# JoshFCooper415/differential_transformer_replication

Hardware: AMD Instinct MI355X
Metric: diff-attn fwd+bwd TFLOP/s (% MFMA peak); train tokens/sec at 1/2/4/8 GPUs (higher is better)
Workload: dtype bf16; 1 GPU; cfg2: fused N=2 diff-attention core fwd+bwd (BASELINE configs[1]); batch_per_gpu=8, global_batch=8, heads=16, head_size=64, dv=128, seq_len=4096, n_terms=2, causal=True, parallelism=batch-sharded replicas x1 (no data-path collective)

## Files before the change

### differential_transformer_replication_amd/_lib.py

```python
from __future__ import annotations

import ctypes
import os
import threading
from typing import Optional

import torch

_HERE = os.path.dirname(os.path.abspath(__file__))
LIB_PATH = os.environ.get("DTA_LIB", os.path.join(_HERE, "lib", "libdiffattn.so"))

DTA_BF16, DTA_F16, DTA_F32 = 0, 1, 2
_DTYPES = {torch.bfloat16: DTA_BF16, torch.float16: DTA_F16, torch.float32: DTA_F32}

ABI_VERSION = 9

EXPORTS = ("dta_attn_fwd", "dta_attn_bwd", "dta_attn_bwd_workspace_bytes", "dta_attn_bwd_dcoef_partial_bytes",
           "dta_ln_fwd", "dta_ln_bwd", "dta_ln_bwd_workspace_bytes",
           "dta_rope", "dta_cast_f32", "dta_error_string", "dta_abi_version", "dta_supported",
           "dta_attn_decode", "dta_attn_decode_workspace_bytes", "dta_swiglu_fwd", "dta_swiglu_bwd",
           "dta_accumulate_f32", "dta_swiglu_bwd_workspace_bytes", "dta_attn_bwd_dkdv_groups",
           "dta_attn_extend", "dta_extend_supported",
           "dta_attn_decode_ragged", "dta_attn_extend_ragged",
           "dta_attn_decode_paged", "dta_attn_extend_paged",
           "dta_attn_decode_paged_fp8", "dta_kv_quant_rows",
           "dta_attn_extend_paged_fp8", "dta_extend_fp8_supported")
FP8_EXPORTS = ("dta_attn_decode_paged_fp8", "dta_kv_quant_rows")
FP8_EXTEND_EXPORTS = ("dta_attn_extend_paged_fp8", "dta_extend_fp8_supported")


class DtaTensor(ctypes.Structure):
    _fields_ = [("ptr", ctypes.c_void_p), ("sb", ctypes.c_int64), ("st", ctypes.c_int64),
                ("sh", ctypes.c_int64), ("si", ctypes.c_int64)]


class SwigluArgs(ctypes.Structure):
    _fields_ = [("dtype", ctypes.c_int32), ("rows", ctypes.c_int64), ("n", ctypes.c_int64),
                ("a", ctypes.c_void_p), ("a_stride", ctypes.c_int64),
                ("b", ctypes.c_void_p), ("b_stride", ctypes.c_int64),
                ("out", ctypes.c_void_p), ("out_stride", ctypes.c_int64),
                ("dout", ctypes.c_void_p), ("dout_stride", ctypes.c_int64),
                ("da", ctypes.c_void_p), ("da_stride", ctypes.c_int64),
                ("db", ctypes.c_void_p), ("db_stride", ctypes.c_int64),
                ("dbias", ctypes.c_void_p), ("dbias_work", ctypes.c_void_p)]


class AttnFwdArgs(ctypes.Structure):
    _fields_ = [("dtype", ctypes.c_int32), ("B", ctypes.c_int32), ("T", ctypes.c_int32),
                ("H", ctypes.c_int32), ("n_terms", ctypes.c_int32), ("head_size", ctypes.c_int32),
                ("dv", ctypes.c_int32), ("scale", ctypes.c_float), ("dropout_p", ctypes.c_float),
                ("q", DtaTensor), ("k", DtaTensor), ("v", DtaTensor), ("o", DtaTensor),
                ("obr", DtaTensor), ("lse", ctypes.c_void_p), ("coef", ctypes.c_void_p),
                ("dropout_seed", ctypes.c_uint64), ("rope_freqs", ctypes.c_void_p), ("q_rot", DtaTensor),
                ("obr_dtype", ctypes.c_int32)]


class AttnBwdArgs(ctypes.Structure):
    _fields_ = [("dtype", ctypes.c_int32), ("B", ctypes.c_int32), ("T", ctypes.c_int32),
                ("H", ctypes.c_int32), ("n_terms", ctypes.c_int32), ("head_size", ctypes.c_int32),
                ("dv", ctypes.c_int32), ("scale", ctypes.c_float), ("dropout_p", ctypes.c_float),
                ("q", DtaTensor), ("k", DtaTensor), ("v", DtaTensor), ("obr", DtaTensor),
                ("lse", ctypes.c_void_p), ("coef", ctypes.c_void_p), ("dout", DtaTensor),
                ("dq", DtaTensor), ("dk", DtaTensor), ("dv_out", DtaTensor),
                ("dcoef", ctypes.c_void_p), ("delta", ctypes.c_void_p), ("dq_f32", ctypes.c_void_p),
                ("stages", ctypes.c_int32), ("rope_freqs", ctypes.c_void_p), ("dcoef_partial", ctypes.c_void_p),
                ("dropout_seed", ctypes.c_uint64), ("obr_dtype", ctypes.c_int32),
                ("group_max_dq", ctypes.c_int32), ("group_max_dkdv", ctypes.c_int32),
                ("dv_f32", ctypes.c_void_p), ("lse_c", ctypes.c_void_p)]


BWD_PRE, BWD_DQ, BWD_DKDV = 1, 2, 4


class LnArgs(ctypes.Structure):
    _fields_ = [("dtype", ctypes.c_int32), ("rows", ctypes.c_int64), ("C", ctypes.c_int64),
                ("eps", ctypes.c_float), ("out_scale", ctypes.c_float),
                ("x", ctypes.c_void_p), ("x_stride", ctypes.c_int64),
                ("y", ctypes.c_void_p), ("y_stride", ctypes.c_int64),
                ("w", ctypes.c_void_p), ("b", ctypes.c_void_p),
                ("mean", ctypes.c_void_p), ("rstd", ctypes.c_void_p),
                ("dy", ctypes.c_void_p), ("dy_stride", ctypes.c_int64),
                ("dx", ctypes.c_void_p), ("dx_stride", ctypes.c_int64),
                ("dw", ctypes.c_void_p), ("db", ctypes.c_void_p), ("partial", ctypes.c_void_p), ("io_dtype", ctypes.c_int32),
                ("res", ctypes.c_void_p), ("res_stride", ctypes.c_int64), ("xo", ctypes.c_void_p),
                ("xo_stride", ctypes.c_int64), ("dres", ctypes.c_void_p), ("dres_stride", ctypes.c_int64),
                ("dx16", ctypes.c_void_p), ("dx16_stride", ctypes.c_int64)]


class RopeArgs(ctypes.Structure):
    _fields_ = [("dtype", ctypes.c_int32), ("B", ctypes.c_int32), ("T", ctypes.c_int32),
                ("H", ctypes.c_int32), ("n_terms", ctypes.c_int32), ("head_size", ctypes.c_int32),
                ("inverse", ctypes.c_int32), ("src_f32", ctypes.c_int32),
                ("src", DtaTensor), ("dst", DtaTensor), ("freqs", ctypes.c_void_p)]


def _cache_op_fields(sizes, k: str, v: str, pointers):
    i32 = ("dtype", "B", "H", "n_terms", "head_size", "dv") + sizes
    return ([(n, ctypes.c_int32) for n in i32] + [("scale", ctypes.c_float)]
            + [(n, DtaTensor) for n in ("q", k, v, "o")]
            + [(n, ctypes.c_void_p) for n in ("coef",) + pointers])


_PAGED_FIELDS = [("page_size", ctypes.c_int32), ("max_pages", ctypes.c_int32), ("n_pages", ctypes.c_int32),
                 ("block_table_dev", ctypes.c_void_p)]
_DECODE_SIZES = ("length", "t_cap")


class DecodeArgs(ctypes.Structure):
    _fields_ = _cache_op_fields(_DECODE_SIZES, "k_cache", "v_cache", ("workspace", "length_dev"))


class ExtendArgs(ctypes.Structure):
    _fields_ = _cache_op_fields(("Tq", "pos", "t_cap"), "k_cache", "v_cache", ())


class DecodeRaggedArgs(ctypes.Structure):
    _fields_ = _cache_op_fields(_DECODE_SIZES, "k_cache", "v_cache", ("workspace", "lengths_dev"))


class ExtendRaggedArgs(ctypes.Structure):
    _fields_ = _cache_op_fields(("Tq", "t_cap"), "k_cache", "v_cache", ("pos_dev", "count_dev"))


class DecodePagedArgs(ctypes.Structure):
    _fields_ = _cache_op_fields(_DECODE_SIZES, "k_pool", "v_pool", ("workspace", "lengths_dev")) + _PAGED_FIELDS


class ExtendPagedArgs(ctypes.Structure):
    _fields_ = _cache_op_fields(("Tq", "t_cap"), "k_pool", "v_pool", ("pos_dev", "count_dev")) + _PAGED_FIELDS


class DecodePagedFp8Args(ctypes.Structure):
    _fields_ = DecodePagedArgs._fields_ + [("scale_pool_dev", ctypes.c_void_p), ("scale_page_stride", ctypes.c_int64)]


class ExtendPagedFp8Args(ctypes.Structure):
    _fields_ = ExtendPagedArgs._fields_ + [("scale_pool_dev", ctypes.c_void_p), ("scale_page_stride", ctypes.c_int64)]


class KvQuantRowsArgs(ctypes.Structure):
    _fields_ = [("dtype", ctypes.c_int32), ("B", ctypes.c_int32), ("Tn", ctypes.c_int32), ("H", ctypes.c_int32),
                ("n_terms", ctypes.c_int32), ("head_size", ctypes.c_int32), ("dv", ctypes.c_int32),
                ("page_size", ctypes.c_int32), ("n_pages", ctypes.c_int32),
                ("k_new", DtaTensor), ("v_new", DtaTensor), ("k_pool", DtaTensor), ("v_pool", DtaTensor),
                ("scale_pool_dev", ctypes.c_void_p), ("scale_page_stride", ctypes.c_int64),
                ("slot_dev", ctypes.c_void_p)]


_lock = threading.Lock()
_lib: Optional[ctypes.CDLL] = None


def load(path: str = LIB_PATH) -> ctypes.CDLL:
    global _lib
    with _lock:
        if _lib is not None:
            return _lib
        if not os.path.exists(path):
            raise RuntimeError(f"libdiffattn.so not found at {path}: run __graft_entry__.build() "
                               "(hipcc --offload-arch=gfx950); there is no CPU fallback")
        lib = ctypes.CDLL(path)
        P = ctypes.POINTER
        lib.dta_attn_fwd.argtypes = [P(AttnFwdArgs), ctypes.c_void_p]
        lib.dta_attn_bwd.argtypes = [P(AttnBwdArgs), ctypes.c_void_p]
        lib.dta_ln_fwd.argtypes = [P(LnArgs), ctypes.c_void_p]
        lib.dta_ln_bwd.argtypes = [P(LnArgs), ctypes.c_void_p]
        lib.dta_rope.argtypes = [P(RopeArgs), ctypes.c_void_p]
        lib.dta_swiglu_fwd.argtypes = [P(SwigluArgs), ctypes.c_void_p]
        lib.dta_swiglu_bwd.argtypes = [P(SwigluArgs), ctypes.c_void_p]
        lib.dta_cast_f32.argtypes = [ctypes.c_int32] * 6 + [ctypes.c_void_p, DtaTensor, ctypes.c_void_p]
        lib.dta_swiglu_bwd_workspace_bytes.argtypes = [ctypes.c_int64, ctypes.c_int64]
        lib.dta_swiglu_bwd_workspace_bytes.restype = ctypes.c_size_t
        lib.dta_accumulate_f32.argtypes = [ctypes.c_int32, ctypes.c_int64, ctypes.c_void_p, ctypes.c_void_p,
                                           ctypes.c_void_p]
        lib.dta_attn_decode.argtypes = [P(DecodeArgs), ctypes.c_void_p]
        lib.dta_attn_decode_workspace_bytes.argtypes = [ctypes.c_int32] * 6
        lib.dta_attn_extend.argtypes = [P(ExtendArgs), ctypes.c_void_p]
        lib.dta_extend_supported.argtypes = [ctypes.c_int32] * 4
        lib.dta_attn_decode_ragged.argtypes = [P(DecodeRaggedArgs), ctypes.c_void_p]
        lib.dta_attn_extend_ragged.argtypes = [P(ExtendRaggedArgs), ctypes.c_void_p]
        lib.dta_attn_decode_paged.argtypes = [P(DecodePagedArgs), ctypes.c_void_p]
        lib.dta_attn_extend_paged.argtypes = [P(ExtendPagedArgs), ctypes.c_void_p]
        lib.dta_attn_decode_workspace_bytes.restype = ctypes.c_size_t
        lib.dta_attn_bwd_workspace_bytes.argtypes = [ctypes.c_int32] * 5
        lib.dta_attn_bwd_workspace_bytes.restype = ctypes.c_size_t
        lib.dta_attn_bwd_dcoef_partial_bytes.argtypes = [ctypes.c_int32] * 4
        lib.dta_attn_bwd_dcoef_partial_bytes.restype = ctypes.c_size_t
        lib.dta_ln_bwd_workspace_bytes.argtypes = [ctypes.c_int64] * 2
        lib.dta_ln_bwd_workspace_bytes.restype = ctypes.c_size_t
        lib.dta_error_string.argtypes = [ctypes.c_int]
        lib.dta_error_string.restype = ctypes.c_char_p
        lib.dta_supported.argtypes = [ctypes.c_int32] * 4
        lib.dta_attn_bwd_dkdv_groups.argtypes = [ctypes.c_int32] * 5
        for fn in ("dta_attn_fwd", "dta_attn_bwd", "dta_attn_decode", "dta_ln_fwd", "dta_ln_bwd", "dta_rope", "dta_cast_f32",
                   "dta_abi_version", "dta_supported", "dta_swiglu_fwd", "dta_swiglu_bwd", "dta_accumulate_f32",
                   "dta_attn_bwd_dkdv_groups", "dta_attn_extend", "dta_extend_supported", "dta_attn_decode_ragged",
                   "dta_attn_extend_ragged", "dta_attn_decode_paged", "dta_attn_extend_paged"):
            getattr(lib, fn).restype = ctypes.c_int
        if fp8_symbols(lib):
            lib.dta_attn_decode_paged_fp8.argtypes = [P(DecodePagedFp8Args), ctypes.c_void_p]
            lib.dta_kv_quant_rows.argtypes = [P(KvQuantRowsArgs), ctypes.c_void_p]
            lib.dta_attn_decode_paged_fp8.restype = lib.dta_kv_quant_rows.restype = ctypes.c_int
        if fp8_extend_symbols(lib):
            lib.dta_attn_extend_paged_fp8.argtypes = [P(ExtendPagedFp8Args), ctypes.c_void_p]
            lib.dta_extend_fp8_supported.argtypes = [ctypes.c_int32] * 4
            lib.dta_attn_extend_paged_fp8.restype = lib.dta_extend_fp8_supported.restype = ctypes.c_int
        if lib.dta_abi_version() != ABI_VERSION:
            raise RuntimeError(f"libdiffattn ABI {lib.dta_abi_version()} != expected {ABI_VERSION}")
        _lib = lib
        return lib


def fp8_symbols(lib) -> bool:
    return all(hasattr(lib, name) for name in FP8_EXPORTS)


def fp8_extend_symbols(lib) -> bool:
    return all(hasattr(lib, name) for name in FP8_EXTEND_EXPORTS)


def check(rc: int) -> None:
    if rc != 0:
        msg = load().dta_error_string(rc).decode()
        raise RuntimeError(f"libdiffattn: {msg} (code {rc})")


def dtype_code(t: torch.dtype) -> int:
    try:
        return _DTYPES[t]
    except KeyError:
        raise RuntimeError(f"libdiffattn supports bf16, fp16 and fp32 activations, got {t}") from None


def stream_handle(device: torch.device) -> int:
    return torch.cuda.current_stream(device).cuda_stream


def ptr(t: Optional[torch.Tensor]) -> Optional[int]:
    return None if t is None else t.data_ptr()


def tensor5(t: torch.Tensor) -> DtaTensor:
    if t.dim() == 5:
        sb, st, sh, si, sd = t.stride()
    elif t.dim() == 4:
        sb, st, sh, sd = t.stride()
        si = 0
    else:
        raise ValueError("expected a 4-d or 5-d view")
    if sd != 1:
        raise RuntimeError("innermost dimension must be contiguous")
    return DtaTensor(t.data_ptr(), sb, st, sh, si)


def supported(dtype: torch.dtype, head_size: int, n_terms: int, dv: int) -> bool:
    return bool(load().dta_supported(dtype_code(dtype), head_size, n_terms, dv))
```

### differential_transformer_replication_amd/csrc/attn_bf16.hip

```cpp
#include "attn_kernels.h"

namespace dta {
int launch_attn_fwd_bf16(const FwdParams& p, hipStream_t st) { return dispatch_fwd<__bf16, false>(p, st); }
int launch_attn_dq_bf16(const BwdParams& p, hipStream_t st) { return dispatch_dq<__bf16, false>(p, st); }
int launch_attn_dkdv_bf16(const BwdParams& p, hipStream_t st) { return dispatch_dkdv<__bf16, false>(p, st); }
bool attn_native_bf16(int hs, int n, int dv) { return native_t<__bf16>(hs, n, dv); }
}
```

### differential_transformer_replication_amd/csrc/attn_f16.hip

```cpp
#include "attn_kernels.h"

namespace dta {
int launch_attn_fwd_f16(const FwdParams& p, hipStream_t st) { return dispatch_fwd<_Float16, false>(p, st); }
int launch_attn_dq_f16(const BwdParams& p, hipStream_t st) { return dispatch_dq<_Float16, false>(p, st); }
int launch_attn_dkdv_f16(const BwdParams& p, hipStream_t st) { return dispatch_dkdv<_Float16, false>(p, st); }
bool attn_native_f16(int hs, int n, int dv) { return native_t<_Float16>(hs, n, dv); }
}
```

### differential_transformer_replication_amd/csrc/attn_kernels.h

```cpp
#pragma once
#include "dta_common.h"
#include "dta_internal.h"
#include "layout_checks.h"

#include <type_traits>
#include <utility>

#ifndef DTA_STAMPS
#define DTA_STAMPS 0
#endif

namespace dta {

template <int NSEG_ = 8>
struct Stamps {
  static constexpr int NSEG = NSEG_;
  unsigned t = 0, s[NSEG] = {};
  __device__ __forceinline__ static unsigned now() {
    unsigned long long v;
    __builtin_amdgcn_sched_barrier(0);
    asm volatile("s_memtime %0\n\ts_waitcnt lgkmcnt(0)" : "=s"(v) : : "memory");
    __builtin_amdgcn_sched_barrier(0);
    return (unsigned)v;
  }
// ... 861 lines not shown
        const unsigned a0 = vb + (Lv ^ (64 * d)), a1 = vb + (Lv ^ (64 * d + 32));
        if constexpr (SPILLS) {
          sfor<NKB>([&](auto KB) { tr_load<VI::ROWB, 32 * decltype(KB)::value>(r[decltype(KB)::value], a0, a1); });
        } else {
          sfor<NKB>([&](auto KB) { tr_issue<VI::ROWB, 32 * decltype(KB)::value>(r[decltype(KB)::value], a0, a1); });
          lgkm_pin<NKB>(r);
        }
#pragma unroll
        for (int kb = 0; kb < NKB; ++kb)
#pragma unroll
          for (int s = 0; s < 2; ++s) {
            const frag va = tr_frag<E>(r[kb], s);
#pragma unroll
            for (int i = 0; i < N; ++i) acc[i][d] = O::mma(va, pf[i][kb * 2 + s], acc[i][d]);
          }
      });
    } else {
#pragma unroll
      for (int d = 0; d < NDB; ++d)
#pragma unroll
        for (int kb = 0; kb < NKB; ++kb)
#pragma unroll
          for (int s = 0; s < SPB; ++s) {
            const frag va = VI::tr_perm(Vc, kb * 32, s, hf, d * 32, lane);
#pragma unroll
            for (int i = 0; i < N; ++i) acc[i][d] = O::mma(va, pf[i][kb * SPB + s], acc[i][d]);
          }
    }
  };

  Stamps<> st;
  auto step = [&](int kt, auto MASKED, auto FASTT) {
    asm volatile("" : "+v"(lane));
    if constexpr (sizeof(E) == 2) asm volatile("" : "+v"(LrK), "+v"(LtV));
    tid = (wave << 6) + lane; hf = lane >> 5; c32 = lane & 31;
    qrow = qw0 + c32;
    const bool live = wave_live && kt * BN <= qw0 + 31;
    st.lap<7>();
    if (kt + NS - 1 < ntiles) stage_kv(kt + NS - 1, (kt + NS - 1) % NS);
    st.lap<0>();
    if (live) {
      frag pf[N][NKB * SPB];
      phase_a(kt, MASKED, pf, FASTT);
      st.lap<1>();
      phase_b(kt, pf);
      st.lap<2>();
    }
    wait_vm(tile_pieces * max(0, min(NS - 2, ntiles - 2 - kt)));
    st.lap<3>();
    lds_barrier();
    st.lap<4>();
  };
  auto attempt = [&](bool safe) {
    for (int j = 0; j < NS - 1; ++j)
      if (j < ntiles) stage_kv(j, j);
    wait_vm(tile_pieces * max(0, min(NS - 1, ntiles) - 1));
    lds_barrier();
    if (qrot_pending) {
#pragma unroll
      for (int i = NQR; i < N; ++i)
        rope_lds<E, HSP, BM, HS, NTHR>(Qs + (i - NQR) * BM * HSP, p.rope, q0, T, gqr + i * p.qrot.si, p.qrot.st,
                                       dc0 == 0, tid);
      lds_barrier();
      qrot_pending = false;
    }
#pragma unroll
    for (int i = 0; i < N; ++i) {
      m[i] = -INFINITY;
      l[i] = 0.f;
#pragma unroll
      for (int d = 0; d < NDB; ++d) acc[i][d] = f32x16{};
    }
    if constexpr (sizeof(E) == 2) { LrK = row_lane<KI::ROWB>(lane); LtV = tr_lane<VI::ROWB>(lane); }
    st.start();
    const int nfull = min(ntiles, min((q0 + 1) / BN, T / BN));
    const int kslow = (safe || !FAST) ? ntiles : min(1, ntiles);
    for (int kt = 0; kt < min(nfull, kslow); ++kt) step(kt, std::false_type{}, std::false_type{});
    for (int kt = nfull; kt < kslow; ++kt) step(kt, std::true_type{}, std::false_type{});
    if constexpr (FAST) {
      for (int kt = kslow; kt < nfull; ++kt) step(kt, std::false_type{}, std::true_type{});
      for (int kt = max(kslow, nfull); kt < ntiles; ++kt) step(kt, std::true_type{}, std::true_type{});
    }
  };
  for (int pass = 0; pass < (FAST ? 2 : 1); ++pass) {
    attempt(pass == 1);
    if constexpr (!FAST) break;
    if (pass == 1) break;
    int* flag = reinterpret_cast<int*>(Kb);
    const bool mine = __any(wave_live && qrow < T && bad != 0.f);
    if (lane == 0) flag[wave] = mine ? 1 : 0;
    lds_barrier();
    bool any = false;
#pragma unroll
    for (int w = 0; w < NW; ++w) any |= flag[w] != 0;
    lds_barrier();
    if (!any) break;
  }
  st.lap<5>();
  st.flush(p.stamps, lin * NW + wave, lane);

  if (!SEQ && !wave_live) return;
  if (bnc) {
    if (wave_live) {
      float inv[N];
#pragma unroll
      for (int i = 0; i < N; ++i) {
        const float lt = wave_sum_halves(l[i]);
        inv[i] = 1.f / lt;
        if (dc0 == 0 && hf == 0 && qrow < T)
          p.lse[(((int64_t)(brs + i) * p.B + b) * p.H + hh) * T + qrow] = -(m[i] + __builtin_log2f(lt));
      }
      float* reg = reinterpret_cast<float*>(Kb) + wave * 2048;
      const int nrows = min(32, T - qw0);
      float* gob0 = reinterpret_cast<float*>(p.obr.p) + b * p.obr.sb + (int64_t)qw0 * p.obr.st + hh * p.obr.sh +
                    brs * p.obr.si + dc0;
#pragma unroll
      for (int i = 0; i < N; ++i)
        bounce_store<float, NDB>(reg, lane, [&](int d, int g) {
          return f32x4{acc[i][d][4 * g] * inv[i], acc[i][d][4 * g + 1] * inv[i], acc[i][d][4 * g + 2] * inv[i],
                       acc[i][d][4 * g + 3] * inv[i]};
        }, gob0 + i * p.obr.si, p.obr.st, nrows);
      auto osum = [&](int d, int g) {
        f32x4 o = f32x4{};
#pragma unroll
        for (int i = 0; i < N; ++i)
#pragma unroll
          for (int j = 0; j < 4; ++j) o[j] = fmaf(coef[i], acc[i][d][4 * g + j] * inv[i], o[j]);
        return o;
      };
      if constexpr (SEQ) {
#pragma unroll
        for (int d = 0; d < NDB; ++d)
#pragma unroll
          for (int g = 0; g < 4; ++g) {
            const f32x4 o = osum(d, g);
#pragma unroll
            for (int j = 0; j < 4; ++j) oacc[d < NDBS ? d : 0][4 * g + j] += o[j];
          }
      } else if (nsp == 1) {
        E* go0 = reinterpret_cast<E*>(p.o.p) + b * p.o.sb + (int64_t)qw0 * p.o.st + hh * p.o.sh + dc0;
        bounce_store<E, NDB>(reg, lane, osum, go0, p.o.st, nrows);
      }
    }
    if constexpr (SEQ) lds_barrier();
  } else {
  if (!SEQ && qrow >= T) return;
  if (wave_live && qrow < T) {
  float inv[N];
#pragma unroll
  for (int i = 0; i < N; ++i) {
    const float lt = wave_sum_halves(l[i]);
    inv[i] = 1.f / lt;
    if (dc0 == 0 && hf == 0)
      p.lse[(((int64_t)(brs + i) * p.B + b) * p.H + hh) * T + qrow] = -(m[i] + __builtin_log2f(lt));
  }
  E* go = reinterpret_cast<E*>(p.o.p) + b * p.o.sb + (int64_t)qrow * p.o.st + hh * p.o.sh + dc0;
  const int64_t gob = b * p.obr.sb + (int64_t)qrow * p.obr.st + hh * p.obr.sh + brs * p.obr.si + dc0;
#pragma unroll
  for (int d = 0; d < NDB; ++d)
#pragma unroll
    for (int g = 0; g < 4; ++g) {
      const int e = d * 32 + 8 * g + 4 * hf;
      float o0 = 0.f, o1 = 0.f, o2 = 0.f, o3 = 0.f;
#pragma unroll
      for (int i = 0; i < N; ++i) {
        const float a0 = acc[i][d][4 * g + 0] * inv[i], a1 = acc[i][d][4 * g + 1] * inv[i];
        const float a2 = acc[i][d][4 * g + 2] * inv[i], a3 = acc[i][d][4 * g + 3] * inv[i];
        store_ob4(p.obr.p, gob + i * p.obr.si + e, p.ob16, a0, a1, a2, a3);
        o0 = fmaf(coef[i], a0, o0); o1 = fmaf(coef[i], a1, o1);
        o2 = fmaf(coef[i], a2, o2); o3 = fmaf(coef[i], a3, o3);
      }
      if constexpr (SEQ) {
        oacc[d < NDBS ? d : 0][4 * g + 0] += o0; oacc[d < NDBS ? d : 0][4 * g + 1] += o1;
        oacc[d < NDBS ? d : 0][4 * g + 2] += o2; oacc[d < NDBS ? d : 0][4 * g + 3] += o3;
      } else {
        if (nsp == 1) store4<E>(go + e, o0, o1, o2, o3);
      }
    }
  }
  }
  }
  if constexpr (SEQ) {
    if (qw0 >= T) return;
    if (bnc) {
      E* go0 = reinterpret_cast<E*>(p.o.p) + b * p.o.sb + (int64_t)qw0 * p.o.st + hh * p.o.sh + dc0;
      bounce_store<E, NDBS>(reinterpret_cast<float*>(Kb) + wave * 2048, lane, [&](int d, int g) {
        return f32x4{oacc[d][4 * g], oacc[d][4 * g + 1], oacc[d][4 * g + 2], oacc[d][4 * g + 3]};
      }, go0, p.o.st, min(32, T - qw0));
      return;
    }
    if (qrow >= T) return;
    E* go = reinterpret_cast<E*>(p.o.p) + b * p.o.sb + (int64_t)qrow * p.o.st + hh * p.o.sh + dc0;
#pragma unroll
    for (int d = 0; d < NDBS; ++d)
#pragma unroll
      for (int g = 0; g < 4; ++g)
        store4<E>(go + d * 32 + 8 * g + 4 * hf, oacc[d][4 * g], oacc[d][4 * g + 1], oacc[d][4 * g + 2], oacc[d][4 * g + 3]);
  }
}

template <class E, int HS, int N, int DV, int NW, bool QREG, int QRH = 0, bool BN32 = false>
struct DqCfg {
  static constexpr bool PAIR = NW == 4 && !QREG && sizeof(E) == 2;
  static constexpr int BN = (PAIR && QRH == 0) || BN32 ? 32 : FwdTile<E>::BN;
  static constexpr int BM = NW * 32;
  static constexpr int HSP = img_cols(HS < 32 ? 32 : HS), QP = img_cols(HS), DVP = img_cols(DV);
  static constexpr int nQ = QREG ? 0 : (N - QRH) * BM * QP;
  static constexpr int nK = N * BN * HSP;
  static constexpr int nV = BN * DVP;
  static constexpr int NS = ring_stages_lim(nQ * (int)sizeof(E), (nK + nV) * (int)sizeof(E),
                                            PAIR ? 80 * 1024 : 160 * 1024);
  static constexpr int bytes = (nQ + NS * nK + NS * nV) * (int)sizeof(E);
};

#ifndef DTA_DQ_EXPG
#define DTA_DQ_EXPG 4
#endif
static_assert(DTA_DQ_EXPG >= 1 && 16 % DTA_DQ_EXPG == 0, "DTA_DQ_EXPG: a divisor of the 16 rows a lane holds");
template <class E, int HS, int N, int DV = 2 * HS, bool NP = false>
struct DqPick {
  static constexpr int LIM = 160 * 1024;
  static constexpr bool q8 = sizeof(E) == 2 && DqCfg<E, HS, N, DV, 8, false>::bytes <= LIM;
  static constexpr int QRH = (q8 && DqCfg<E, HS, N, DV, 4, false, 1>::bytes <= 80 * 1024) ? 1 : 0;
  static constexpr bool pair64 = !NP && QRH == 1 && q8 && HS >= 64 &&
                                 DqCfg<E, HS, N, DV, 4, false, QRH>::bytes <= 80 * 1024;
  static constexpr bool pair32 = !NP && !pair64 && sizeof(E) == 2 && N >= 3 && HS == 64 &&
                                 DqCfg<E, HS, N, DV, 4, false, 1, true>::bytes <= 80 * 1024;
  static constexpr bool pair = pair64 || pair32;
  static constexpr int NW = pair ? 4 : (q8 ? 8 : (sizeof(E) == 2 ? 4 : 2));
  static constexpr bool QREG = pair ? false : !q8;
  static constexpr int QH = pair ? 1 : 0;
  static constexpr bool B32 = pair32 || DqCfg<E, HS, N, DV, NW, QREG, QH>::bytes > LIM;
  static constexpr bool ok = DqCfg<E, HS, N, DV, NW, QREG, QH, B32>::bytes <= LIM;
};

template <class E, int HS, int N, int DV, int NW, bool QREG, bool OUTF32, bool SRD, bool DROP, int QRH, bool B32>
__global__ __launch_bounds__(NW * 64, simd_waves(NW, DqCfg<E, HS, N, DV, NW, QREG, QRH, B32>::bytes))
void attn_dq_kernel(BwdParams p) {
  using O = Ops<E>;
  using frag = typename O::frag;
  using CF = DqCfg<E, HS, N, DV, NW, QREG, QRH, B32>;
  constexpr int NQR = QREG ? N : QRH;
  constexpr int HSP = CF::HSP, QP = CF::QP, DVP = CF::DVP;
  using QI = Img<E, QP>;
  using KI = Img<E, HSP>;
  using VI = Img<E, DVP>;
  constexpr int BN = CF::BN, BM = CF::BM, NTHR = NW * 64;
  constexpr int KS = O::KSTEP;
  constexpr int NSQ = HS / KS, NSV = DV / KS;
  constexpr int NKB = BN / 32, SPB = 32 / KS, NHB = (HS + 31) / 32;

  extern __shared__ __attribute__((aligned(16))) char smem[];
  E* Qs = reinterpret_cast<E*>(smem);
  constexpr int NS = CF::NS;
  E* Kb = Qs + CF::nQ;
  E* Vb = Kb + NS * CF::nK;

  const int wave = __builtin_amdgcn_readfirstlane(threadIdx.x >> 6);
  int tid = threadIdx.x, lane = tid & 63;
  int hf = lane >> 5, c32 = lane & 31;
  int bx, by, bz, lin;
  lpt_order(bx, by, bz, lin);
  const int qt = gridDim.x - 1 - bx;
  const int hh = by, b = bz;
  const int T = p.T;
  const int q0 = qt * BM, qw0 = q0 + wave * 32;
  int qrow = qw0 + c32;
  const bool rowok = qrow < T;

  const E* gq = reinterpret_cast<const E*>(p.q.p) + b * p.q.sb + hh * p.q.sh;
  const E* gk = reinterpret_cast<const E*>(p.k.p) + b * p.k.sb + hh * p.k.sh;
  const E* gv = reinterpret_cast<const E*>(p.v.p) + b * p.v.sb + hh * p.v.sh;
  const E* gdo = reinterpret_cast<const E*>(p.dout.p) + b * p.dout.sb + hh * p.dout.sh;
  const int64_t gob = b * p.obr.sb + hh * p.obr.sh;

  const int kend = min(T, q0 + BM);
  const int ntiles = (kend + BN - 1) / BN;
  using KR = KvRing<E, HS, N, DV, BN, NW>;
  static_assert(!SRD || (HSP == KR::HSP && DVP == KR::DVP), "descriptor staging fills the kernel's images");
  constexpr bool PRE = SRD && !DROP;
  uint32_t doff[PRE ? KR::MYP : 1];
  if constexpr (PRE) KR::offsets(p.k.st, p.k.si, p.v.st, wave, lane, doff);
  auto stage_kv = [&](int kt, int buf) {
    const int k0 = kt * BN;
    if constexpr (PRE) {
      KR::issue_pre(gk, p.k.st, gv, p.v.st, k0, T, Kb + buf * CF::nK, Vb + buf * CF::nV, wave, doff);
    } else if constexpr (SRD) {
      KR::issue(gk, p.k.st, p.k.si, gv, p.v.st, k0, T, Kb + buf * CF::nK, Vb + buf * CF::nV, wave, lane);
    } else {
#pragma unroll
      for (int i = 0; i < N; ++i)
        stage<E, HSP, BN, HS, NTHR>(Kb + (buf * N + i) * BN * HSP, gk + i * p.k.si, p.k.st, k0, T - 1, tid);
      stage<E, DVP, BN, DV, NTHR>(Vb + buf * CF::nV, gv, p.v.st, k0, T - 1, tid);
    }
  };

  constexpr bool SEED = std::is_same<E, __bf16>::value && !DROP && SRD && !(HS >= 128 && N >= 3);
  constexpr bool SPILLS = sizeof(E) == 2 && (DROP || (HS >= 128 && N >= 3) || (HS >= 192 && N >= 2));
  frag qf[NQR > 0 ? NQR : 1][NQR > 0 ? NSQ : 1], df[NSV];
  float coef[N], lse[N], del[N];
  float dhead = 0.f;
  const int64_t rs = (((int64_t)0 * p.B + b) * p.H + hh) * T + qrow;
  const int64_t bstride = (int64_t)p.B * p.H * T;
#pragma unroll
  for (int s = 0; s < NSV; ++s)
    df[s] = rowok ? O::load_global(gdo + (int64_t)qrow * p.dout.st + s * KS + hf * O::KH) : O::zero();
#pragma unroll
  for (int i = 0; i < N; ++i) {
    coef[i] = p.coef[hh * p.cst + i];
    if (i < NQR) {
#pragma unroll
      for (int s = 0; s < NSQ; ++s)
        qf[i < NQR ? i : 0][s] = rowok ? O::load_global(gq + (int64_t)qrow * p.q.st + i * p.q.si + s * KS + hf * O::KH)
                                       : O::zero();
      if constexpr (SEED) {
#pragma unroll
        for (int s = 0; s < NSQ; ++s)
#pragma unroll
          for (int j = 0; j < 8; ++j) qf[i < NQR ? i : 0][s][j] = (E)((float)qf[i < NQR ? i : 0][s][j] * p.sl2);
      }
    }
    lse[i] = rowok ? p.lse[rs + i * bstride] : 0.f;
    if (p.lsec && rowok && hf == 0) p.lsec[rs + i * bstride] = lse[i] + __builtin_log2f(fabsf(coef[i]));
    float d = 0.f;
    if (rowok) {
#pragma unroll
      for (int s = 0; s < NSV; ++s) {
        const int64_t o = gob + (int64_t)qrow * p.obr.st + i * p.obr.si + s * KS + hf * O::KH;
        if constexpr (sizeof(E) == 2) {
          float ov[8];
          load_ob8(p.obr.p, o, p.ob16, ov);
#pragma unroll
          for (int j = 0; j < 8; ++j) d = fmaf((float)df[s][j], ov[j], d);
        } else {
          d = fmaf(df[s], reinterpret_cast<const float*>(p.obr.p)[o], d);
        }
      }
    }
    d = wave_sum_halves(d);
    del[i] = d;
    const bool kstart = i == 0 || ((p.kstarts >> i) & 1);
    if (kstart) dhead = d;
    if (rowok && hf == 0) p.delta[rs + i * bstride] = DROP ? d : (kstart ? -d : dhead - d);
    float w = (rowok && hf == 0) ? d : 0.f;
#pragma unroll
    for (int o = 32; o > 0; o >>= 1) w += __shfl_xor(w, o, 64);
    if (p.dcoef_part) {
      if (lane == 0 && qw0 < T) p.dcoef_part[(((int64_t)hh * p.cst + i) * p.B + b) * ((T + 31) / 32) + qw0 / 32] = w;
    } else if (lane == 0 && qw0 < T) {
      atomicAdd(p.dcoef + hh * p.cst + i, w);
    }
  }

  if constexpr (!QREG) {
#pragma unroll
    for (int i = NQR; i < N; ++i)
      stage<E, QP, BM, HS, NTHR>(Qs + (i - NQR) * BM * QP, gq + i * p.q.si, p.q.st, q0, T - 1, tid);
  }
  const int tile_pieces = SRD ? KR::pieces(wave)
                              : N * stage_pieces<E, HSP, BN, HS, NW>(wave) + stage_pieces<E, DVP, BN, DV, NW>(wave);
  for (int j = 0; j < NS - 1; ++j)
    if (j < ntiles) stage_kv(j, j);
  wait_vm(tile_pieces * max(0, min(NS - 1, ntiles) - 1));
  lds_barrier();
  frag f_one = O::zero(), f_lse[SEED ? N : 1], f_dp = O::zero();
  float ddel[N];
  if constexpr (SEED) {
    if constexpr (!QREG && N > NQR) {
      scale_lds<E, NTHR>(Qs, CF::nQ, p.sl2, tid);
      lds_barrier();
    }
    if (hf == 0) { f_one[0] = (E)1.f; f_one[1] = (E)1.f; }
#pragma unroll
    for (int i = 0; i < N; ++i) {
      f_lse[i] = seed_frag<E>(lse[i], hf);
      ddel[i] = del[0] - del[i];
    }
    f_dp = seed_frag<E>(-del[0], hf);
  }

  f32x16 dq[N][NHB];
#pragma unroll
  for (int i = 0; i < N; ++i)
#pragma unroll
    for (int d = 0; d < NHB; ++d) dq[i][d] = f32x16{};
  const bool wave_live = qw0 < T;

  int LrV = 0, LrK = 0, LrQ = 0, LtK = 0;
  constexpr int XMAX = 32 * ((NSV > NSQ ? NSV : NSQ) - 1) + 64 * (NHB - 1) + 32;
  constexpr int XM = XMAX < 256 ? 256 : (XMAX < 512 ? 512 : 1024);
  constexpr bool XA = !DROP && SRD && sizeof(E) == 2 && (CF::nQ * (int)sizeof(E)) % XM == 0 &&
                      (CF::nK * (int)sizeof(E)) % XM == 0 && (CF::nV * (int)sizeof(E)) % XM == 0;
  if constexpr (sizeof(E) == 2) {
    LrV = row_lane<VI::ROWB>(lane); LrK = row_lane<KI::ROWB>(lane); LrQ = row_lane<QI::ROWB>(lane);
    LtK = tr_lane<KI::ROWB>(lane);
  }
  Stamps<5> st;
  auto step = [&](int kt, auto MASKED) {
    constexpr bool MASK = decltype(MASKED)::value;
    asm volatile("" : "+v"(lane));
    if constexpr (!DROP && sizeof(E) == 2) {
      asm volatile("" : "+v"(LrV), "+v"(LrK), "+v"(LtK));
      if constexpr (QI::ROWB == KI::ROWB) LrQ = LrK;
      else asm volatile("" : "+v"(LrQ));
    } else if constexpr (sizeof(E) == 2) {
      LrV = row_lane<VI::ROWB>(lane); LrK = row_lane<KI::ROWB>(lane); LrQ = row_lane<QI::ROWB>(lane);
      LtK = tr_lane<KI::ROWB>(lane);
    }
    tid = (wave << 6) + lane; hf = lane >> 5; c32 = lane & 31;
    qrow = qw0 + c32;
    const int buf = kt % NS;
    if (kt + NS - 1 < ntiles) stage_kv(kt + NS - 1, (kt + NS - 1) % NS);
    st.lap<0>();
    const int k0 = kt * BN;
    if (wave_live && k0 <= qw0 + 31) {
      const E* Kc = Kb + buf * CF::nK;
      const E* Vc = Vb + buf * CF::nV;
      unsigned bV = 0, bK = 0, tK = 0;
      if constexpr (XA) {
        bV = LrV + lds_addr(Vc); bK = LrK + lds_addr(Kc); tK = LtK + lds_addr(Kc);
      }
      {
        f32x16 dp[NKB];
        if constexpr (sizeof(E) == 2) {
          const int Lv = LrV;
          const char* vbase = reinterpret_cast<const char*>(Vc);
#pragma unroll
          for (int kb = 0; kb < NKB; ++kb) dp[kb] = SEED ? O::mma(f_one, f_dp, f32x16{}) : f32x16{};
          if constexpr (XA && !SPILLS) {
            constexpr int NIT = NSV * NKB, D = DTA_DQ_PIPE;
            i32x4 vb[D + 1];
            auto issue = [&](auto J) {
              constexpr int j = decltype(J)::value;
              ds128<(j % NKB) * 32 * VI::ROWB>(vb[j % (D + 1)], bV ^ (32 * (j / NKB)));
            };
            sfor<(D < NIT ? D : NIT)>([&](auto J) { issue(J); });
            sfor<NIT>([&](auto J) {
              constexpr int j = decltype(J)::value;
              if constexpr (j + D < NIT) issue(std::integral_constant<int, j + D>{});
              lgkm_wait<(j + D < NIT ? D : NIT - 1 - j)>();
              asm volatile("" : "+v"(vb[j % (D + 1)]));
              dp[j % NKB] = O::mma(__builtin_bit_cast(frag, vb[j % (D + 1)]), df[j / NKB], dp[j % NKB]);
            });
          } else
#pragma unroll
          for (int s = 0; s < NSV; ++s) {
            const int o = Lv ^ (32 * s);
#pragma unroll
            for (int kb = 0; kb < NKB; ++kb) {
              if constexpr (XA) dp[kb] = O::mma(lds_at<frag>(bV ^ (32 * s), kb * 32 * VI::ROWB), df[s], dp[kb]);
              else dp[kb] = O::mma(*reinterpret_cast<const frag*>(vbase + kb * 32 * VI::ROWB + o), df[s], dp[kb]);
            }
          }

        } else {
#pragma unroll
          for (int kb = 0; kb < NKB; ++kb) {
            dp[kb] = f32x16{};
#pragma unroll
            for (int s = 0; s < NSV; ++s) dp[kb] = O::mma(VI::row(Vc, kb * 32 + c32, s, hf), df[s], dp[kb]);
          }
        }
        st.lap<1>();
        sfor<N>([&](auto I_) {
          constexpr int i = decltype(I_)::value;
          const E* Ki = Kc + i * BN * HSP;
          f32x16 sa[NKB];
          if constexpr (XA && !SPILLS) {
            constexpr int QL = i >= NQR ? 1 : 0;
            constexpr int KOFF = i * BN * HSP * (int)sizeof(E), QOFF = (i >= NQR ? i - NQR : 0) * BM * QP * (int)sizeof(E);
#pragma unroll
            for (int kb = 0; kb < NKB; ++kb) sa[kb] = SEED ? O::mma(f_one, f_lse[SEED ? i : 0], f32x16{}) : f32x16{};
            s_chain_pipe<E, NSQ, NKB, QL, DTA_DQ_PIPE, KOFF, QOFF, KI::ROWB>(
                sa, bK, lds_addr(Qs) + wave * 32 * QI::ROWB + LrQ, qf[i < NQR ? i : 0]);
          } else if constexpr (sizeof(E) == 2) {
            const int Lr = LrK;
            const char* kbase = reinterpret_cast<const char*>(Ki);
            const char* qbase = reinterpret_cast<const char*>(Qs + (i >= NQR ? i - NQR : 0) * BM * QP) +
                                wave * 32 * QI::ROWB;
            const int Lq = LrQ;
#pragma unroll
            for (int kb = 0; kb < NKB; ++kb) sa[kb] = SEED ? O::mma(f_one, f_lse[SEED ? i : 0], f32x16{}) : f32x16{};
#pragma unroll
            for (int s = 0; s < NSQ; ++s) {
              frag qb;
              if (i < NQR) qb = qf[i < NQR ? i : 0][s];
              else qb = *reinterpret_cast<const frag*>(qbase + (Lq ^ (32 * s)));
#pragma unroll
              for (int kb = 0; kb < NKB; ++kb) {
                if constexpr (XA)
                  sa[kb] = O::mma(lds_at<frag>(bK ^ (32 * s), (i * BN * HSP) * (int)sizeof(E) + kb * 32 * KI::ROWB), qb,
                                  sa[kb]);
                else
                  sa[kb] = O::mma(*reinterpret_cast<const frag*>(kbase + kb * 32 * KI::ROWB + (Lr ^ (32 * s))), qb, sa[kb]);
              }
            }
          } else {
#pragma unroll
            for (int kb = 0; kb < NKB; ++kb) {
              sa[kb] = f32x16{};
#pragma unroll
              for (int s = 0; s < NSQ; ++s) {
                frag qb;
                if (i < NQR) qb = qf[i < NQR ? i : 0][s];
                else qb = QI::row(Qs + (i >= NQR ? i - NQR : 0) * BM * QP, wave * 32 + c32, s, hf);
                sa[kb] = O::mma(KI::row(Ki, kb * 32 + c32, s, hf), qb, sa[kb]);
              }
            }
          }
          const float li = lse[i], ci = coef[i], cdi = coef[i] * del[i];
          const int lim = min(qrow, T - 1) - k0 - 4 * hf;
          if constexpr (SEED) {
            const float dd = ddel[i];
#pragma unroll
            for (int kb = 0; kb < NKB; ++kb)
#pragma unroll
              for (int r0 = 0; r0 < 16; r0 += DTA_DQ_EXPG) {
                float pr[DTA_DQ_EXPG];
#pragma unroll
                for (int u = 0; u < DTA_DQ_EXPG; ++u) {
                  const int r = r0 + u;
                  float arg = sa[kb][r];
                  if constexpr (MASK) arg = (kb * 32 + (r & 3) + 8 * (r >> 2) > lim) ? -INFINITY : arg;
                  pr[u] = exp2_fast(arg);
                }
#pragma unroll
                for (int u = 0; u < DTA_DQ_EXPG; ++u) {
                  const int r = r0 + u;
                  sa[kb][r] = i == 0 ? pr[u] * dp[kb][r] : pr[u] * (dp[kb][r] + dd);
                }
              }
          } else {
          uint32_t dkey = 0;
          if constexpr (DROP) dkey = drop_key(p.drop_seed_lo, p.drop_seed_hi, b, hh, p.br0 + i, p.H, p.cst);
#pragma unroll
          for (int kb = 0; kb < NKB; ++kb)
#pragma unroll
            for (int r = 0; r < 16; ++r) {
              float arg = fmaf(sa[kb][r], p.sl2, li);
              if constexpr (MASK) arg = (kb * 32 + (r & 3) + 8 * (r >> 2) > lim) ? -INFINITY : arg;
              float cm = ci;
              if constexpr (DROP)
                cm *= drop_mul(dkey, qrow, k0 + kb * 32 + (r & 3) + 8 * (r >> 2) + 4 * hf, p.drop_thr, p.drop_scale);
              sa[kb][r] = exp2_fast(arg) * fmaf(cm, dp[kb][r], -cdi);
            }
          }
          if constexpr (sizeof(E) == 2) {
            const unsigned kbse = lds_addr(Ki);
            const int Lk = LtK;
            sfor<NHB>([&](auto D) {
              constexpr int d = decltype(D)::value;
              lds64 r[NKB][4];
              const unsigned a0 = XA ? (tK ^ (64 * d)) + (unsigned)(i * BN * HSP * (int)sizeof(E)) : kbse + (Lk ^ (64 * d));
              const unsigned a1 = XA ? (tK ^ (64 * d + 32)) + (unsigned)(i * BN * HSP * (int)sizeof(E))
                                     : kbse + (Lk ^ (64 * d + 32));
              if constexpr (SPILLS) {
                sfor<NKB>([&](auto KB) { tr_load<KI::ROWB, 32 * decltype(KB)::value>(r[decltype(KB)::value], a0, a1); });
              } else {
                sfor<NKB>([&](auto KB) { tr_issue<KI::ROWB, 32 * decltype(KB)::value>(r[decltype(KB)::value], a0, a1); });
                lgkm_pin<NKB>(r);
              }
#pragma unroll
              for (int kb = 0; kb < NKB; ++kb) {
                dq[i][d] = O::mma(tr_frag<E>(r[kb], 0), O::template pack<0>(sa[kb]), dq[i][d]);
                dq[i][d] = O::mma(tr_frag<E>(r[kb], 1), O::template pack<1>(sa[kb]), dq[i][d]);
              }
            });
          } else {
#pragma unroll
            for (int d = 0; d < NHB; ++d)
#pragma unroll
              for (int kb = 0; kb < NKB; ++kb)
#pragma unroll
                for (int s = 0; s < SPB; ++s)
                  dq[i][d] = O::mma(KI::tr_perm(Ki, kb * 32, s, hf, d * 32, lane), sa[kb][s], dq[i][d]);
          }
        });
      }
    }
    st.lap<2>();
    wait_vm(tile_pieces * max(0, min(NS - 2, ntiles - 2 - kt)));
    st.lap<3>();
    lds_barrier();
    st.lap<4>();
  };
  st.start();
  const int nfull = min(ntiles, min((q0 + 1) / BN, T / BN));
  for (int kt = 0; kt < nfull; ++kt) step(kt, std::false_type{});
  for (int kt = nfull; kt < ntiles; ++kt) step(kt, std::true_type{});
  st.flush(p.stamps, lin * NW + wave, lane);

  if (qw0 >= T) return;
  constexpr bool BNC = sizeof(E) == 2 && NHB % 2 == 0 && CF::bytes >= NW * 8192;
  if constexpr (BNC) {
    if (OUTF32 || t5_aligned16(p.dq, sizeof(E))) {
      float* reg = reinterpret_cast<float*>(smem) + wave * 2048;
      const int nrows = min(32, T - qw0);
      const int rrow = min(qrow, T - 1);
#pragma unroll
      for (int i = 0; i < N; ++i) {
        const float sc = SEED ? p.scale * coef[i] : p.scale;
        auto val = [&](int d, int g) {
          float a0 = dq[i][d][4 * g] * sc, a1 = dq[i][d][4 * g + 1] * sc;
          float a2 = dq[i][d][4 * g + 2] * sc, a3 = dq[i][d][4 * g + 3] * sc;
          if (p.rope) rope_inv4(p.rope, rrow, HS, d * 32 + 8 * g + 4 * hf, a0, a1, a2, a3);
          return f32x4{a0, a1, a2, a3};
        };
        if constexpr (OUTF32)
          bounce_store<float, NHB>(reg, lane, val, p.dq32 + ((((int64_t)b * T + qw0) * p.H + hh) * p.cst + i) * HS,
                                   (int64_t)p.H * p.cst * HS, nrows);
        else
          bounce_store<E, NHB>(reg, lane, val, reinterpret_cast<E*>(p.dq.p) + b * p.dq.sb + (int64_t)qw0 * p.dq.st +
                                                   hh * p.dq.sh + i * p.dq.si, p.dq.st, nrows);
      }
      return;
    }
  }
  if (!rowok) return;
#pragma unroll
  for (int i = 0; i < N; ++i)
#pragma unroll
    for (int d = 0; d < NHB; ++d)
#pragma unroll
      for (int g = 0; g < 4; ++g) {
        const int e = d * 32 + 8 * g + 4 * hf;
        if (e >= HS) continue;
        const float sc = SEED ? p.scale * coef[i] : p.scale;
        float a0 = dq[i][d][4 * g] * sc, a1 = dq[i][d][4 * g + 1] * sc;
        float a2 = dq[i][d][4 * g + 2] * sc, a3 = dq[i][d][4 * g + 3] * sc;
        if (p.rope) rope_inv4(p.rope, qrow, HS, e, a0, a1, a2, a3);
        if constexpr (OUTF32) {
          store4<float>(p.dq32 + ((((int64_t)b * T + qrow) * p.H + hh) * p.cst + i) * HS + e, a0, a1, a2, a3);
        } else {
          E* gdq = reinterpret_cast<E*>(p.dq.p) + b * p.dq.sb + (int64_t)qrow * p.dq.st + hh * p.dq.sh + i * p.dq.si;
          store4<E>(gdq + e, a0, a1, a2, a3);
        }
      }
}

template <class E, int HS, int N, int DV, int NW, bool DELTA, int BQ_ = 32, bool ROWS = true>
struct TileRing {
  static constexpr int ES = (int)sizeof(E), BQ = BQ_;
  static constexpr int NP = (N * BQ + 63) / 64 * 64;
  static constexpr int HSP = img_cols(HS), DVP = img_cols(DV);
  static constexpr int QB = BQ * HSP * ES, DB = BQ * DVP * ES;
  static constexpr int OFF_D = N * QB, OFF_L = OFF_D + DB, OFF_G = OFF_L + NP * 4;
  static constexpr int SB = ROWS ? OFF_G + NP * 4 : OFF_L;
  static constexpr int PQ = N * QB / 1024, PD = DB / 1024, PL = NP / 64;
  static constexpr int NPC = PQ + PD + (ROWS ? (DELTA ? 2 : 1) * PL : 0);
  static constexpr int MYP = (NPC + NW - 1) / NW;
  static constexpr bool ok = ES == 2 && HS >= 32 && QB % 1024 == 0 && DB % 1024 == 0;

  __device__ static int pieces(int wave) { return NPC / NW + (wave < NPC % NW ? 1 : 0); }

  __device__ static uint32_t offq(const BwdParams& p, int j, int lane) {
    using QI = Img<E, HSP>;
    const int i = j / (QB / 1024), pb = (j % (QB / 1024)) * 1024 + lane * 16;
    const int r = pb / QI::ROWB;
    int c = ((pb % QI::ROWB) >> 4) ^ swz<QI::ROWB>(r);
    if constexpr (HSP != HS) c = c * 16 < HS * ES ? c : 0;
    return (uint32_t)(r * (uint32_t)(p.q.st * ES) + (uint32_t)(i * p.q.si * ES) + c * 16);
  }
  __device__ static uint32_t offd(const BwdParams& p, int j, int lane) {
    using DI = Img<E, DVP>;
    const int pb = (j - PQ) * 1024 + lane * 16;
    const int r = pb / DI::ROWB;
    int c = ((pb % DI::ROWB) >> 4) ^ swz<DI::ROWB>(r);
    if constexpr (DVP != DV) c = c * 16 < DV * ES ? c : 0;
    return (uint32_t)(r * (uint32_t)(p.dout.st * ES) + c * 16);
  }
  __device__ static uint32_t offr(int j, int lane, int64_t bstride) {
    const int e = ((j - PQ - PD) % PL) * 64 + lane;
    const int i = min(e / BQ, N - 1), r = e % BQ;
    return (uint32_t)((i * (uint32_t)bstride + r) * 4);
  }
  __device__ static void offsets(const BwdParams& p, int64_t bstride, int wave, int lane, uint32_t (&off)[MYP]) {
    sfor<MYP>([&](auto U) {
      constexpr int u = decltype(U)::value;
      const int j = u * NW + wave;
      if constexpr ((u + 1) * NW <= PQ) off[u] = offq(p, j, lane);
      else if constexpr (u * NW >= PQ && (u + 1) * NW <= PQ + PD) off[u] = offd(p, j, lane);
      else off[u] = j < PQ ? offq(p, j, lane) : (j < PQ + PD ? offd(p, j, lane) : (j < NPC ? offr(j, lane, bstride) : 0u));
    });
  }
  __device__ static void issue_pre(const BwdParams& p, const E* gq, const E* gdo, const float* lse, const float* delta,
                                   int64_t bstride, int q0, int T, char* st0, int wave, const uint32_t (&off)[MYP]) {
    const int rows = T - q0;
    const E* bq = gq + (int64_t)q0 * p.q.st;
    const E* bd = gdo + (int64_t)q0 * p.dout.st;
    const uint32_t nq = (uint32_t)rows * (uint32_t)(p.q.st * ES), nd = (uint32_t)rows * (uint32_t)(p.dout.st * ES);
    const uint32_t nl = (uint32_t)(((N - 1) * bstride + rows) * 4);
    sfor<MYP>([&](auto U) {
      constexpr int u = decltype(U)::value;
      const int j = u * NW + wave;
      if constexpr ((u + 1) * NW <= PQ) {
        buf_lds16(bq, nq, st0 + j * 1024, off[u]);
      } else if constexpr (u * NW >= PQ && (u + 1) * NW <= PQ + PD) {
        buf_lds16(bd, nd, st0 + OFF_D + (j - PQ) * 1024, off[u]);
      } else {
        if (j < PQ) buf_lds16(bq, nq, st0 + j * 1024, off[u]);
        else if (j < PQ + PD) buf_lds16(bd, nd, st0 + OFF_D + (j - PQ) * 1024, off[u]);
        else if (j < PQ + PD + PL) buf_lds4(lse + q0, nl, st0 + OFF_L + (j - PQ - PD) * 256, off[u]);
        else if (j < NPC) buf_lds4(delta + q0, nl, st0 + OFF_G + (j - PQ - PD - PL) * 256, off[u]);
      }
    });
  }
};

inline bool ring_layout_ok(const BwdParams& p, int es) {
  return dma_rows_ok(p.T, p.q.st, p.q.si, p.N, p.HS, es) && dma_rows_ok(p.T, p.dout.st, 0, 1, p.DV, es) &&
         dma_rowvecs_ok(p.N, p.B, p.H, p.T);
}


template <class E, int HS, int N, int DV, int NW, bool PR = false, bool GRX = false>
struct DkdvCfg {
  static constexpr int LIMB = PR ? 80 * 1024 : 160 * 1024;
  static constexpr int BK = NW * 32;
  static constexpr int HSP = img_cols(HS < 32 ? 32 : HS), KP = img_cols(HS), DVP = img_cols(DV);
  static constexpr int BQ = 32;
  static constexpr int NP = (N * BQ + 63) / 64 * 64;
  static constexpr int nQ = N * BQ * HSP;
  static constexpr int nD = BQ * DVP;
  static constexpr int nK = N * BK * KP;
  static constexpr int RB = 2 * NP * 4;
  static constexpr bool GR = GRX;
  static constexpr int NS = ring_stages_lim(nK * (int)sizeof(E), (nQ + nD) * (int)sizeof(E) + (GR ? 0 : RB), LIMB);
  static constexpr int bytes = (nK + NS * nQ + NS * nD) * (int)sizeof(E) + (GR ? 0 : NS * RB);
};

template <int HS, int N, int DV>
struct DkdvSplit {
  static constexpr int HSB = (HS < 32 ? 32 : HS + 31) / 32 * 32;
  static constexpr bool fused = (N * HSB / 2 + DV / 2) <= 160;
};

template <class E, int HS, int N, int DV, bool NP = false>
struct DkdvWaves {
  static constexpr int LIM = 160 * 1024;
  static constexpr int HSB = DkdvSplit<HS, N, DV>::HSB;
  static constexpr int regs8 = DkdvSplit<HS, N, DV>::fused ? N * HSB / 2 + DV / 2 + DV / 4 + 88
                             : (N * HSB / 2 + DV / 4 > DV / 2 ? N * HSB / 2 + DV / 4 : DV / 2) + 88;
  static constexpr int v8 = (sizeof(E) == 2 && DkdvCfg<E, HS, N, DV, 8>::bytes <= LIM && regs8 <= 256) ? 8
                          : DkdvCfg<E, HS, N, DV, 4>::bytes <= LIM ? 4 : 2;
  static constexpr bool pair = !NP && std::is_same<E, __bf16>::value && v8 == 8 &&
                               DkdvCfg<E, HS, N, DV, 4, true>::bytes <= 80 * 1024;
  static constexpr int v0 = pair ? 4 : v8;
  static constexpr bool gr = DkdvCfg<E, HS, N, DV, v0, pair>::bytes > LIM;
  static constexpr int v = !gr ? v0 : (DkdvCfg<E, HS, N, DV, 2, false, true>::bytes <= LIM ? 2 : 1);
};

template <class E, int HS, int N, int DV, int NW, bool DK, bool DVV, bool SRD, bool DROP, bool PR, bool GRX,
          bool CFOLD = false>
__global__ __launch_bounds__(NW * 64, (NW >= 8 || PR ? 2 : 1))
void attn_dkdv_kernel(BwdParams p) {
  using O = Ops<E>;
  using frag = typename O::frag;
  using CF = DkdvCfg<E, HS, N, DV, NW, PR, GRX>;
  constexpr int HSP = CF::HSP, KP = CF::KP, DVP = CF::DVP, BQ = CF::BQ, BK = CF::BK, NP = CF::NP;
  constexpr int NTHR = NW * 64;
  using QI = Img<E, HSP>;
  using DI = Img<E, DVP>;
  constexpr int KS = O::KSTEP;
  constexpr int NSQ = HS / KS, NSV = DV / KS, SPB = 32 / KS;
  constexpr int NHB = (HS + 31) / 32, NVB = DV / 32;
  constexpr bool SPILLS = sizeof(E) == 2 && (DROP || (HS >= 128 && N >= 3) || (HS >= 192 && N >= 2));

  using KI = Img<E, KP>;
  extern __shared__ __attribute__((aligned(16))) char smem[];
  E* Ks = reinterpret_cast<E*>(smem);
  E* Qb = Ks + CF::nK;
  constexpr int NS = CF::NS;
  E* Db = Qb + NS * CF::nQ;
  float* Lb = reinterpret_cast<float*>(Db + NS * CF::nD);
  float* Gb = Lb + NS * NP;
  constexpr bool GR = CF::GR;
  using RG = TileRing<E, HS, N, DV, NW, DK, BQ, !GR>;
  char* ringb = reinterpret_cast<char*>(Qb);
  static_assert(!SRD || (RG::ok && RG::SB * NS <= CF::bytes - CF::nK * (int)sizeof(E) && RG::HSP == HSP &&
                          RG::DVP == DVP), "ring layout");

  const int wave = __builtin_amdgcn_readfirstlane(threadIdx.x >> 6);
  int tid = threadIdx.x, lane = tid & 63;
  int hf = lane >> 5, c32 = lane & 31;
  int bx, by, bz, lin;
  lpt_order(bx, by, bz, lin);
  const int kblk = bx;
  const int hh = by, b = bz;
  const int T = p.T;
  const int kb0 = kblk * BK, kw0 = kb0 + wave * 32;
  int krow = kw0 + c32;

  const E* gq = reinterpret_cast<const E*>(p.q.p) + b * p.q.sb + hh * p.q.sh;
  const E* gk = reinterpret_cast<const E*>(p.k.p) + b * p.k.sb + hh * p.k.sh;
  const E* gv = reinterpret_cast<const E*>(p.v.p) + b * p.v.sb + hh * p.v.sh;
  const E* gdo = reinterpret_cast<const E*>(p.dout.p) + b * p.dout.sb + hh * p.dout.sh;
  const int64_t rowvec = ((int64_t)b * p.H + hh) * T;
  const int64_t bstride = (int64_t)p.B * p.H * T;

  float coef[N];
  uint32_t dkey[N];
#pragma unroll
  for (int i = 0; i < N; ++i) {
    coef[i] = p.coef[hh * p.cst + i];
    dkey[i] = DROP ? drop_key(p.drop_seed_lo, p.drop_seed_hi, b, hh, p.br0 + i, p.H, p.cst) : 0u;
  }
  static_assert(!CFOLD || (!DROP && sizeof(E) == 2 && !GRX), "CFOLD: 16-bit plans without dropout");
  auto sgn = [](float c) { return c < 0.f ? -1.f : 1.f; };
  float wv[N];
#pragma unroll
  for (int i = 0; i < N; ++i) wv[i] = CFOLD ? sgn(coef[0]) * sgn(coef[i]) : coef[i];
  const float dvsc = CFOLD ? sgn(coef[0]) : 1.f;
  const float* lsep = CFOLD ? p.lsec : p.lse;
  frag vf[DK ? NSV : 1];
  if constexpr (DK) {
#pragma unroll
    for (int s = 0; s < NSV; ++s)
      vf[s] = krow < T ? O::load_global(gv + (int64_t)krow * p.v.st + s * KS + hf * O::KH) : O::zero();
  }

  uint32_t roff[SRD ? RG::MYP : 1];
  if constexpr (SRD) RG::offsets(p, bstride, wave, lane, roff);
  auto stage_q = [&](int q0, int buf) {
    if constexpr (SRD) {
      RG::issue_pre(p, gq, gdo, lsep + rowvec, p.delta + rowvec, bstride, q0, T, ringb + buf * RG::SB, wave, roff);
    } else {
#pragma unroll
      for (int i = 0; i < N; ++i)
        stage<E, HSP, BQ, HS, NTHR>(Qb + (buf * N + i) * BQ * HSP, gq + i * p.q.si, p.q.st, q0, T - 1, tid);
      stage<E, DVP, BQ, DV, NTHR>(Db + buf * CF::nD, gdo, p.dout.st, q0, T - 1, tid);
      if constexpr (!GR) {
        stage_rows<N, BQ, NTHR>(Lb + buf * NP, lsep + rowvec, bstride, q0, T - 1, tid);
        if constexpr (DK) stage_rows<N, BQ, NTHR>(Gb + buf * NP, p.delta + rowvec, bstride, q0, T - 1, tid);
      }
    }
  };

  f32x16 dk[DK ? N : 1][NHB];
  f32x16 dv[DVV ? NVB : 1];
#pragma unroll
  for (int i = 0; i < (DK ? N : 1); ++i)
#pragma unroll
    for (int d = 0; d < NHB; ++d) dk[i][d] = f32x16{};
#pragma unroll
  for (int d = 0; d < (DVV ? NVB : 1); ++d) dv[d] = f32x16{};

  const int ntiles = kb0 < T ? (T - kb0 + BQ - 1) / BQ : 0;
#pragma unroll
  for (int i = 0; i < N; ++i) stage<E, KP, BK, HS, NTHR>(Ks + i * BK * KP, gk + i * p.k.si, p.k.st, kb0, T - 1, tid);
  const int tile_pieces = SRD ? RG::pieces(wave)
                              : N * stage_pieces<E, HSP, BQ, HS, NW>(wave) + stage_pieces<E, DVP, BQ, DV, NW>(wave) +
                                    rows_pieces<N, BQ, NW>(wave) * (DK ? 2 : 1);
  for (int j = 0; j < NS - 1; ++j)
    if (j < ntiles) stage_q(kb0 + j * BQ, j);
  wait_vm(tile_pieces * max(0, min(NS - 1, ntiles) - 1));
  lds_barrier();
  scale_lds<E, NTHR>(Ks, CF::nK, p.sl2, tid);
  lds_barrier();
  const bool wave_keys = kw0 < T;

  Stamps<4> st;
  int LrD = 0, LrQ = 0, LrK = 0, LtQ = 0, LtD = 0;
  constexpr int XMAX = 64 * ((NVB > NHB ? NVB : NHB) - 1) + 32 + 32 * ((NSV > NSQ ? NSV : NSQ) - 1);
  constexpr int XM = XMAX < 256 ? 256 : (XMAX < 512 ? 512 : 1024);
  constexpr bool XA = SRD && sizeof(E) == 2 && (CF::nK * (int)sizeof(E)) % XM == 0 && RG::SB % XM == 0 &&
                      QI::ROWB == KI::ROWB;
  if constexpr (sizeof(E) == 2) {
    LrD = row_lane<DI::ROWB>(lane); LrQ = row_lane<QI::ROWB>(lane); LrK = row_lane<KI::ROWB>(lane);
    LtQ = tr_lane<QI::ROWB>(lane); LtD = tr_lane<DI::ROWB>(lane);
  }
  auto step = [&](int t, auto MASKED) {
    constexpr bool MASK = decltype(MASKED)::value;
    asm volatile("" : "+v"(lane));
    if constexpr (sizeof(E) == 2) {
      asm volatile("" : "+v"(LrD), "+v"(LrQ), "+v"(LtQ), "+v"(LtD));
      if constexpr (QI::ROWB == KI::ROWB) LrK = LrQ;
      else asm volatile("" : "+v"(LrK));
    }
    tid = (wave << 6) + lane; hf = lane >> 5; c32 = lane & 31;
    krow = kw0 + c32;
    const int buf = t % NS;
    const int q0 = kb0 + t * BQ;
    if (t + NS - 1 < ntiles) stage_q(q0 + (NS - 1) * BQ, (t + NS - 1) % NS);
    st.lap<0>();
    if (wave_keys && q0 + 31 >= kw0) {
      const char* sg = ringb + buf * RG::SB;
      const E* Qc = SRD ? reinterpret_cast<const E*>(sg) : Qb + buf * N * BQ * HSP;
      const E* Dc = SRD ? reinterpret_cast<const E*>(sg + RG::OFF_D) : Db + buf * CF::nD;
      const float* Lc = SRD ? reinterpret_cast<const float*>(sg + RG::OFF_L) : Lb + buf * NP;
      const float* Gc = SRD ? reinterpret_cast<const float*>(sg + RG::OFF_G) : Gb + buf * NP;
      auto rows4 = [&](const float* ring, const float* glb, int i, int g) -> f32x4 {
        if constexpr (GR) {
          const float* v = glb + rowvec + i * bstride;
          const int r0 = q0 + 8 * g + 4 * hf;
          return f32x4{v[min(r0, T - 1)], v[min(r0 + 1, T - 1)], v[min(r0 + 2, T - 1)], v[min(r0 + 3, T - 1)]};
        } else {
          return *reinterpret_cast<const f32x4*>(ring + i * BQ + 8 * g + 4 * hf);
        }
      };
      unsigned bQ = 0, bD = 0, tQ = 0, tD = 0;
      if constexpr (XA) {
        const unsigned sb = lds_addr(sg);
        bQ = LrQ + sb; bD = LrD + sb; tQ = LtQ + sb; tD = LtD + sb;
      }
      {
      f32x16 dpa = f32x16{};
      if constexpr (DK && !DROP) {
#pragma unroll
        for (int g = 0; g < 4; ++g) {
          const f32x4 g4 = rows4(Gc, p.delta, 0, g);
#pragma unroll
          for (int j = 0; j < 4; ++j) dpa[4 * g + j] = g4[j];
        }
      }
      if constexpr (DK) {
        if constexpr (sizeof(E) == 2) {
          const int Ld = LrD;
          const char* dbase = reinterpret_cast<const char*>(Dc);
#pragma unroll
          for (int s = 0; s < NSV; ++s) {
            if constexpr (XA) dpa = O::mma(lds_at<frag>(bD ^ (32 * s), RG::OFF_D), vf[s], dpa);
            else dpa = O::mma(*reinterpret_cast<const frag*>(dbase + (Ld ^ (32 * s))), vf[s], dpa);
          }
        } else {
#pragma unroll
          for (int s = 0; s < NSV; ++s) dpa = O::mma(DI::row(Dc, c32, s, hf), vf[s], dpa);
        }
      }
      f32x16 pc = f32x16{};
      const int lim_lo = krow - q0 - 4 * hf;
      const int lim_hi = T - 1 - q0 - 4 * hf;
#pragma unroll
      for (int i = 0; i < N; ++i) {
        if constexpr (CFOLD) if (i > 0) __builtin_amdgcn_sched_barrier(0);
        f32x16 sa;
#pragma unroll
        for (int g = 0; g < 4; ++g) {
          const f32x4 l4 = rows4(Lc, lsep, i, g);
#pragma unroll
          for (int j = 0; j < 4; ++j) sa[4 * g + j] = l4[j];
        }
        const E* Qi = Qc + i * BQ * HSP;
        if constexpr (sizeof(E) == 2) {
          const int Lq = LrQ, Lk = LrK;
          const char* qbase = reinterpret_cast<const char*>(Qi);
          const char* kbase = reinterpret_cast<const char*>(Ks + i * BK * KP) + wave * 32 * KI::ROWB;
          frag qfr[NSQ], kfr[NSQ];
#pragma unroll
          for (int s = 0; s < NSQ; ++s) {
            if constexpr (XA) qfr[s] = lds_at<frag>(bQ ^ (32 * s), i * RG::QB);
            else qfr[s] = *reinterpret_cast<const frag*>(qbase + (Lq ^ (32 * s)));
            kfr[s] = *reinterpret_cast<const frag*>(kbase + (Lk ^ (32 * s)));
          }
#pragma unroll
          for (int s = 0; s < NSQ; ++s) sa = O::mma(qfr[s], kfr[s], sa);
          __builtin_amdgcn_sched_group_barrier(0x100, 2 * NSQ, 0);
          __builtin_amdgcn_sched_group_barrier(0x008, NSQ, 0);
        } else {
#pragma unroll
          for (int s = 0; s < NSQ; ++s)
            sa = O::mma(QI::row(Qi, c32, s, hf), KI::row(Ks + i * BK * KP, wave * 32 + c32, s, hf), sa);
        }
#pragma unroll
        for (int g = 0; g < 4; ++g) {
          f32x4 d4 = f32x4{};
          if constexpr (DK) if (DROP || i > 0) d4 = rows4(Gc, p.delta, i, g);
#pragma unroll
          for (int j = 0; j < 4; ++j) {
            const int r = 4 * g + j;
            float arg = sa[r];
            if constexpr (MASK) {
              const int rc = (r & 3) + 8 * (r >> 2);
              arg = (rc < lim_lo || rc > lim_hi) ? -INFINITY : arg;
            }
            const float pr = exp2_fast(arg);
            if constexpr (DROP) {
              const float mk = drop_mul(dkey[i], q0 + (r & 3) + 8 * (r >> 2) + 4 * hf, krow, p.drop_thr, p.drop_scale);
              if constexpr (DVV) pc[r] = fmaf(coef[i] * mk, pr, pc[r]);
              if constexpr (DK) sa[r] = pr * fmaf(mk, dpa[r], -d4[j]);
            } else {
              if constexpr (DVV) pc[r] = i == 0 ? (CFOLD ? pr : wv[0] * pr) : fmaf(wv[i], pr, pc[r]);
              if constexpr (DK) sa[r] = i == 0 ? pr * dpa[r] : pr * (dpa[r] + d4[j]);
            }
          }
        }
        if constexpr (DK) {
          if constexpr (sizeof(E) == 2) {
            const unsigned qb = lds_addr(Qi);
            const int Lq = LtQ;
            lds64 r[NHB][4];
            sfor<NHB>([&](auto D) {
              constexpr int d = decltype(D)::value;
              if constexpr (SPILLS) {
                if constexpr (XA) tr_load<QI::ROWB, 0>(r[d], (tQ ^ (64 * d)) + i * RG::QB, (tQ ^ (64 * d + 32)) + i * RG::QB);
                else tr_load<QI::ROWB, 0>(r[d], qb + (Lq ^ (64 * d)), qb + (Lq ^ (64 * d + 32)));
              } else {
                if constexpr (XA) tr_issue<QI::ROWB, 0>(r[d], (tQ ^ (64 * d)) + i * RG::QB, (tQ ^ (64 * d + 32)) + i * RG::QB);
                else tr_issue<QI::ROWB, 0>(r[d], qb + (Lq ^ (64 * d)), qb + (Lq ^ (64 * d + 32)));
              }
            });
            if constexpr (!SPILLS) lgkm_pin<NHB>(r);
            const frag p0 = O::template pack<0>(sa), p1 = O::template pack<1>(sa);
#pragma unroll
            for (int d = 0; d < NHB; ++d) {
              dk[i][d] = O::mma(tr_frag<E>(r[d], 0), p0, dk[i][d]);
              dk[i][d] = O::mma(tr_frag<E>(r[d], 1), p1, dk[i][d]);
            }
          } else {
#pragma unroll
            for (int d = 0; d < NHB; ++d)
#pragma unroll
              for (int s = 0; s < SPB; ++s) dk[i][d] = O::mma(QI::tr_perm(Qi, 0, s, hf, d * 32, lane), sa[s], dk[i][d]);
          }
        }
      }
      if constexpr (DVV) {
        if constexpr (sizeof(E) == 2) {
          const unsigned db = lds_addr(Dc);
          const int Ld = LtD;
          const frag p0 = O::template pack<0>(pc), p1 = O::template pack<1>(pc);
          constexpr int NP2 = NVB >= 2 ? 2 : 1;
          auto dv_blocks = [&](auto D0, auto NB) {
            constexpr int d0 = decltype(D0)::value, nb = decltype(NB)::value;
            lds64 r[nb][4];
            sfor<nb>([&](auto E2) {
              constexpr int d = d0 + decltype(E2)::value;
              if constexpr (SPILLS) {
                if constexpr (XA) tr_load<DI::ROWB, 0, RG::OFF_D>(r[decltype(E2)::value], tD ^ (64 * d), tD ^ (64 * d + 32));
                else tr_load<DI::ROWB, 0>(r[decltype(E2)::value], db + (Ld ^ (64 * d)), db + (Ld ^ (64 * d + 32)));
              } else {
                if constexpr (XA) tr_issue<DI::ROWB, 0, RG::OFF_D>(r[decltype(E2)::value], tD ^ (64 * d), tD ^ (64 * d + 32));
                else tr_issue<DI::ROWB, 0>(r[decltype(E2)::value], db + (Ld ^ (64 * d)), db + (Ld ^ (64 * d + 32)));
              }
            });
            if constexpr (!SPILLS) lgkm_pin<nb>(r);
#pragma unroll
            for (int e = 0; e < nb; ++e) {
              dv[d0 + e] = O::mma(tr_frag<E>(r[e], 0), p0, dv[d0 + e]);
              dv[d0 + e] = O::mma(tr_frag<E>(r[e], 1), p1, dv[d0 + e]);
            }
          };
          sfor<NVB / NP2>([&](auto D2) {
            dv_blocks(std::integral_constant<int, NP2 * decltype(D2)::value>{}, std::integral_constant<int, NP2>{});
          });
          if constexpr (NVB % NP2) dv_blocks(std::integral_constant<int, NVB - 1>{}, std::integral_constant<int, 1>{});
        } else {
#pragma unroll
          for (int d = 0; d < NVB; ++d)
#pragma unroll
            for (int s = 0; s < SPB; ++s) dv[d] = O::mma(DI::tr_perm(Dc, 0, s, hf, d * 32, lane), pc[s], dv[d]);
        }
      }
      }
    }
    st.lap<1>();
    wait_vm(tile_pieces * max(0, min(NS - 2, ntiles - 2 - t)));
    st.lap<2>();
    lds_barrier();
    st.lap<3>();
  };
  st.start();
  const int thead = min(ntiles, (BK - 2) / BQ + 1);
  const int ttail = max(thead, ntiles - ((T - kb0) % BQ != 0 ? 1 : 0));
  for (int t = 0; t < thead; ++t) step(t, std::true_type{});
  for (int t = thead; t < ttail; ++t) step(t, std::false_type{});
  for (int t = ttail; t < ntiles; ++t) step(t, std::true_type{});
  st.flush(p.stamps, lin * NW + wave, lane);

  if (!wave_keys) return;
  constexpr bool BNC = sizeof(E) == 2 && (!DK || NHB % 2 == 0) && (!DVV || NVB % 2 == 0) &&
                       CF::bytes >= NW * 8192;
  if constexpr (BNC) {
    float* g32 = p.dv32 ? p.dv32 + (((int64_t)b * p.T + kw0) * p.H + hh) * p.DV : nullptr;
    const bool to32 = g32 != nullptr && !p.dv_last;
    if ((!DK || t5_aligned16(p.dk, sizeof(E))) && (!DVV || p.dv_acc || to32 || t5_aligned16(p.dv, sizeof(E)))) {
      float* reg = reinterpret_cast<float*>(smem) + wave * 2048;
      const int nrows = min(32, T - kw0);
      const int rrow = min(krow, T - 1);
      if constexpr (DK) {
#pragma unroll
        for (int i = 0; i < N; ++i) {
          const float sc = p.scale * (CFOLD ? sgn(coef[i]) : coef[i]);
          bounce_store<E, NHB>(reg, lane, [&](int d, int g) {
            float a0 = dk[i][d][4 * g] * sc, a1 = dk[i][d][4 * g + 1] * sc;
            float a2 = dk[i][d][4 * g + 2] * sc, a3 = dk[i][d][4 * g + 3] * sc;
            if (p.rope) rope_inv4(p.rope, rrow, HS, d * 32 + 8 * g + 4 * hf, a0, a1, a2, a3);
            return f32x4{a0, a1, a2, a3};
          }, reinterpret_cast<E*>(p.dk.p) + b * p.dk.sb + (int64_t)kw0 * p.dk.st + hh * p.dk.sh + i * p.dk.si,
             p.dk.st, nrows);
        }
      }
      if constexpr (DVV) {
        if (!p.dv_acc) {
          auto val = [&](int d, int g) {
            return f32x4{dv[d][4 * g] * dvsc, dv[d][4 * g + 1] * dvsc, dv[d][4 * g + 2] * dvsc, dv[d][4 * g + 3] * dvsc};
          };
          if (to32) bounce_store<float, NVB>(reg, lane, val, g32, (int64_t)p.H * p.DV, nrows);
          else bounce_store<E, NVB>(reg, lane, val, reinterpret_cast<E*>(p.dv.p) + b * p.dv.sb + (int64_t)kw0 * p.dv.st +
                                                       hh * p.dv.sh, p.dv.st, nrows);
          return;
        }
      } else {
        return;
      }
      if (krow >= T) return;
      float* g32r = p.dv32 ? p.dv32 + (((int64_t)b * p.T + krow) * p.H + hh) * p.DV : nullptr;
      E* gdv = reinterpret_cast<E*>(p.dv.p) + b * p.dv.sb + (int64_t)krow * p.dv.st + hh * p.dv.sh;
#pragma unroll
      for (int d = 0; d < (DVV ? NVB : 1); ++d)
#pragma unroll
        for (int g = 0; g < 4; ++g) {
          const int e = d * 32 + 8 * g + 4 * hf;
          float a0 = dv[d][4 * g] * dvsc, a1 = dv[d][4 * g + 1] * dvsc, a2 = dv[d][4 * g + 2] * dvsc,
                a3 = dv[d][4 * g + 3] * dvsc;
          if (g32r) {
            const f32x4 v = *reinterpret_cast<const f32x4*>(g32r + e);
            a0 += v[0]; a1 += v[1]; a2 += v[2]; a3 += v[3];
          } else {
            a0 += (float)gdv[e]; a1 += (float)gdv[e + 1]; a2 += (float)gdv[e + 2]; a3 += (float)gdv[e + 3];
          }
          if (to32) store4<float>(g32r + e, a0, a1, a2, a3);
          else store4<E>(gdv + e, a0, a1, a2, a3);
        }
      return;
    }
  }
  if (krow >= T) return;
  if constexpr (DK) {
    E* gdk = reinterpret_cast<E*>(p.dk.p) + b * p.dk.sb + (int64_t)krow * p.dk.st + hh * p.dk.sh;
#pragma unroll
    for (int i = 0; i < N; ++i) {
      const float sc = p.scale * (CFOLD ? sgn(coef[i]) : coef[i]);
#pragma unroll
      for (int d = 0; d < NHB; ++d)
#pragma unroll
        for (int g = 0; g < 4; ++g) {
          const int e = d * 32 + 8 * g + 4 * hf;
          if (e < HS) {
            float a0 = dk[i][d][4 * g] * sc, a1 = dk[i][d][4 * g + 1] * sc;
            float a2 = dk[i][d][4 * g + 2] * sc, a3 = dk[i][d][4 * g + 3] * sc;
            if (p.rope) rope_inv4(p.rope, krow, HS, e, a0, a1, a2, a3);
            store4<E>(gdk + i * p.dk.si + e, a0, a1, a2, a3);
          }
        }
    }
  }
  if constexpr (DVV) {
    E* gdv = reinterpret_cast<E*>(p.dv.p) + b * p.dv.sb + (int64_t)krow * p.dv.st + hh * p.dv.sh;
    float* g32 = p.dv32 ? p.dv32 + (((int64_t)b * p.T + krow) * p.H + hh) * p.DV : nullptr;
    const bool to32 = g32 != nullptr && !p.dv_last;
#pragma unroll
    for (int d = 0; d < NVB; ++d)
#pragma unroll
      for (int g = 0; g < 4; ++g) {
        const int e = d * 32 + 8 * g + 4 * hf;
        float a0 = dv[d][4 * g] * dvsc, a1 = dv[d][4 * g + 1] * dvsc, a2 = dv[d][4 * g + 2] * dvsc,
              a3 = dv[d][4 * g + 3] * dvsc;
        if (p.dv_acc) {
          if (g32) {
            const f32x4 v = *reinterpret_cast<const f32x4*>(g32 + e);
            a0 += v[0]; a1 += v[1]; a2 += v[2]; a3 += v[3];
          } else {
            a0 += (float)gdv[e]; a1 += (float)gdv[e + 1]; a2 += (float)gdv[e + 2]; a3 += (float)gdv[e + 3];
          }
        }
        if (to32) store4<float>(g32 + e, a0, a1, a2, a3);
        else store4<E>(gdv + e, a0, a1, a2, a3);
      }
  }
}

template <class K>
static inline int set_smem(K kernel, int bytes) {
  if (bytes > 65536)
    return (int)hipFuncSetAttribute((const void*)kernel, hipFuncAttributeMaxDynamicSharedMemorySize, bytes);
  return 0;
}

struct CombineDiv {
  FastDiv vpr, H, T;
};
inline CombineDiv combine_div(const FwdParams& p, int esize) {
  return CombineDiv{FastDiv((uint32_t)(p.DV / (16 / esize))), FastDiv((uint32_t)p.H), FastDiv((uint32_t)p.T)};
}
template <class E, int NC>
__global__ __launch_bounds__(256) void branch_combine_kernel(FwdParams p, CombineDiv dv) {
  const int N = NC > 0 ? NC : p.N;
  constexpr int V = 16 / (int)sizeof(E);
  typedef float f32xv __attribute__((ext_vector_type(V)));
  typedef E ev __attribute__((ext_vector_type(V)));
  const uint32_t idx = blockIdx.x * 256 + threadIdx.x;
  const uint32_t total = (uint32_t)p.B * p.T * p.H * dv.vpr.d;
  if (idx >= total) return;
  const uint32_t row = dv.vpr.div(idx);
  const int e = (int)(idx - row * dv.vpr.d) * V;
  const uint32_t bt = dv.H.div(row);
  const int hh = (int)(row - bt * p.H);
  const uint32_t b = dv.T.div(bt);
  const int t = (int)(bt - b * p.T);
  const int64_t src = b * p.obr.sb + (int64_t)t * p.obr.st + hh * p.obr.sh + e;
  f32xv acc = f32xv{};
#pragma unroll
  for (int i = 0; i < N; ++i) {
    const float c = p.coef[hh * p.cst + i];
    if constexpr (V == 8) {
      if (p.ob16) {
        float x[8];
        load_ob8(p.obr.p, src + i * p.obr.si, true, x);
#pragma unroll
        for (int j = 0; j < V; ++j) acc[j] = fmaf(c, x[j], acc[j]);
        continue;
      }
    }
    const f32xv x = *reinterpret_cast<const f32xv*>(reinterpret_cast<const float*>(p.obr.p) + src + i * p.obr.si);
#pragma unroll
    for (int j = 0; j < V; ++j) acc[j] = fmaf(c, x[j], acc[j]);
  }
  ev y;
#pragma unroll
  for (int j = 0; j < V; ++j) y[j] = (E)acc[j];
  __builtin_nontemporal_store(y, reinterpret_cast<ev*>(reinterpret_cast<E*>(p.o.p) + b * p.o.sb + (int64_t)t * p.o.st +
                                                       hh * p.o.sh + e));
}

template <class E, int HS, int DV, bool DROP>
constexpr bool fwd_seq_ok() {
  return !DROP && sizeof(E) == 2 && DV == 2 * HS && FwdPick<E, HS, 1, DV, DROP>::pair &&
         FwdPick<E, HS, 1, DV, DROP>::DVC == DV;
}

template <class E, int HS, int N, int DV_ = 2 * HS>
struct Plan {
  static constexpr int DV = DV_;
  using FP = FwdPick<E, HS, N, DV>;
  using DP = DqPick<E, HS, N, DV>;
  static constexpr int KVW = DkdvWaves<E, HS, N, DV>::v;
  static constexpr bool KPR = DkdvWaves<E, HS, N, DV>::pair && !DkdvWaves<E, HS, N, DV>::gr;
  static constexpr bool ok = FP::ok && DP::ok &&
                             DkdvCfg<E, HS, N, DV, KVW, KPR, DkdvWaves<E, HS, N, DV>::gr>::bytes <= 160 * 1024;
};

template <class E, int HS, int N, int DV_, bool DROP>
int launch_fwd_t(const FwdParams& p, hipStream_t st) {
  using PL = Plan<E, HS, N, DV_>;
  using FP = FwdPick<E, HS, N, PL::DV, DROP>;
  constexpr int DVC = FP::DVC, NW = FP::NW;
  constexpr int QH = FP::QH;
  constexpr int bytes = FwdCfg<E, HS, N, DVC, NW, FP::QREG, QH>::bytes;
  constexpr bool SPLIT = N >= 2 && Plan<E, HS, 1, PL::DV>::ok &&
                         (DVC < PL::DV || (sizeof(E) == 2 && HS >= 64 && !FwdPick<E, HS, N, PL::DV>::pair));
  if constexpr (SPLIT) {
    FwdParams q = p;
    if constexpr (fwd_seq_ok<E, HS, PL::DV, DROP>()) {
      q.bseq = N;
      return launch_fwd_t<E, HS, 1, DV_, DROP>(q, st);
    }
    q.bsplit = N;
    if (int e = launch_fwd_t<E, HS, 1, DV_, DROP>(q, st)) return e;
    const int64_t n = (int64_t)p.B * p.T * p.H * (PL::DV / (16 / (int)sizeof(E)));
    if (n >= (1ll << 31)) return -2;
    hipLaunchKernelGGL((branch_combine_kernel<E, N>), dim3((unsigned)((n + 255) / 256)), dim3(256), 0, st, p,
                       combine_div(p, (int)sizeof(E)));
    return (int)hipGetLastError();
  } else {
    const int nsp = (N == 1 && p.bsplit > 1) ? p.bsplit : 1;
    dim3 grid((p.T + NW * 32 - 1) / (NW * 32), p.H * nsp * (PL::DV / DVC), p.B);
    auto run = [&](auto SRDV) -> int {
      auto go = [&](auto K) -> int {
        if (int e = set_smem(K, bytes)) return e;
        hipLaunchKernelGGL(K, grid, dim3(NW * 64), bytes, st, p);
        return 0;
      };
      if constexpr (N == 1 && fwd_seq_ok<E, HS, PL::DV, DROP>())
        if (p.bseq > 1) return go(attn_fwd_kernel<E, HS, N, DVC, NW, FP::QREG, decltype(SRDV)::value, DROP, QH, true>);
      return go(attn_fwd_kernel<E, HS, N, DVC, NW, FP::QREG, decltype(SRDV)::value, DROP, QH>);
    };
    int e = 0;
    if constexpr (KvRing<E, HS, N, DVC, FwdCfg<E, HS, N, DVC, NW, FP::QREG, QH>::BN, NW>::ok)
      e = kv_layout_ok(p, (int)sizeof(E)) ? run(std::true_type{}) : run(std::false_type{});
    else
      e = run(std::false_type{});
    if (e) return e;
    return (int)hipGetLastError();
  }
}

template <class E, int HS, int N, int DV_, bool DROP>
int launch_dq_t(const BwdParams& p, hipStream_t st) {
  using PL = Plan<E, HS, N, DV_>;
  using DP = DqPick<E, HS, N, PL::DV, DROP>;
  constexpr int NW = DP::NW, DV = PL::DV;
  constexpr bool QR = DP::QREG;
  constexpr int QH = DP::QH;
  constexpr bool B32 = DP::B32;
  using CF = DqCfg<E, HS, N, DV, NW, QR, QH, B32>;
  constexpr int bytes = CF::bytes;
  dim3 grid((p.T + NW * 32 - 1) / (NW * 32), p.H, p.B);
  auto run = [&](auto F32, auto SRDV) -> int {
    auto kern = attn_dq_kernel<E, HS, N, DV, NW, QR, decltype(F32)::value, decltype(SRDV)::value, DROP, QH, B32>;
    if (int e = set_smem(kern, bytes)) return e;
    hipLaunchKernelGGL(kern, grid, dim3(NW * 64), bytes, st, p);
    return 0;
  };
  auto go = [&](auto SRDV) -> int { return p.dq32 ? run(std::true_type{}, SRDV) : run(std::false_type{}, SRDV); };
  int e = 0;
  if constexpr (KvRing<E, HS, N, DV, CF::BN, NW>::ok && CF::HSP == img_cols(HS))
    e = kv_layout_ok(p, (int)sizeof(E)) ? go(std::true_type{}) : go(std::false_type{});
  else
    e = go(std::false_type{});
  if (e) return e;
  return (int)hipGetLastError();
}

template <class E, int HS, int N, int DV_, bool DROP>
int launch_dkdv_t(const BwdParams& p, hipStream_t st) {
  using PL = Plan<E, HS, N, DV_>;
  using KW = DkdvWaves<E, HS, N, PL::DV, DROP>;
  constexpr int NW = KW::v, DV = PL::DV;
  constexpr bool GR = KW::gr;
  constexpr bool PR = KW::pair && !GR;
  using CF = DkdvCfg<E, HS, N, DV, NW, PR, GR>;
  constexpr int bytes = CF::bytes;
  dim3 grid((p.T + NW * 32 - 1) / (NW * 32), p.H, p.B);
  dim3 block(NW * 64);
  constexpr int HSB = DkdvSplit<HS, N, DV>::HSB;
  constexpr bool FUSED = DkdvSplit<HS, N, DV>::fused ||
                         (sizeof(E) == 2 && NW == 4 && !PR && N * HSB / 2 + DV / 2 <= 288);
  constexpr bool CAN_FOLD = sizeof(E) == 2 && !DROP && !GR;
  auto run = [&](auto DKV, auto DVVV, auto SRDV) -> int {
    auto launch = [&](auto CFV) -> int {
      auto kern = attn_dkdv_kernel<E, HS, N, DV, NW, decltype(DKV)::value, decltype(DVVV)::value,
                                   decltype(SRDV)::value, DROP, PR, GR, decltype(CFV)::value>;
      if (int e = set_smem(kern, bytes)) return e;
      hipLaunchKernelGGL(kern, grid, block, bytes, st, p);
      return 0;
    };
    if constexpr (CAN_FOLD)
      if (p.lsec) return launch(std::true_type{});
    return launch(std::false_type{});
  };
  auto go = [&](auto SRDV) -> int {
    if constexpr (FUSED) {
      return run(std::true_type{}, std::true_type{}, SRDV);
    } else {
      if (int e = run(std::true_type{}, std::false_type{}, SRDV)) return e;
      return run(std::false_type{}, std::true_type{}, SRDV);
    }
  };
  int e = 0;
  if constexpr (TileRing<E, HS, N, DV, NW, true, CF::BQ, !GR>::ok) {
    e = ring_layout_ok(p, (int)sizeof(E)) ? go(std::true_type{}) : go(std::false_type{});
  } else {
    e = go(std::false_type{});
  }
  if (e) return e;
  return (int)hipGetLastError();
}

#ifndef DTA_FOR_CONFIGS
#define DTA_FOR_CONFIGS(X) \
  X(16, 1, 32) X(16, 2, 32) X(16, 3, 32) X(16, 4, 32) X(32, 1, 64) X(32, 2, 64) X(32, 3, 64) X(32, 4, 64) \
  X(64, 1, 128) X(64, 2, 128) X(64, 3, 128) X(64, 4, 128) X(128, 1, 256) X(128, 2, 256) X(128, 3, 256) \
  X(128, 4, 256) X(64, 1, 64) X(128, 1, 128) X(32, 1, 32) \
  X(96, 1, 192) X(96, 2, 192) X(96, 3, 192) X(96, 4, 192) X(96, 1, 96) \
  X(256, 1, 512) X(256, 2, 512) X(256, 1, 256)
#endif

template <class E>
bool native_t(int hs, int n, int dv) {
#define DTA_S(HS_, N_, DV_) if (hs == HS_ && n == N_ && dv == DV_) return Plan<E, HS_, N_, DV_>::ok;
  DTA_FOR_CONFIGS(DTA_S)
#undef DTA_S
  return false;
}

template <class E, bool DROP>
int fwd_branch_split_any(const FwdParams& p, hipStream_t st) {
  FwdParams q = p;
  q.bsplit = p.N;
  int e = -2;
  bool seq = false;
#define DTA_F1(HS_, N_, DV_) \
  if (N_ == 1 && p.HS == HS_ && p.DV == DV_) { \
    if constexpr (N_ == 1 && Plan<E, HS_, 1, DV_>::ok) { \
      if constexpr (fwd_seq_ok<E, HS_, DV_, DROP>()) { q.bsplit = 0; q.bseq = p.N; seq = true; } \
      e = launch_fwd_t<E, HS_, 1, DV_, DROP>(q, st); } }
  DTA_FOR_CONFIGS(DTA_F1)
#undef DTA_F1
  if (e || seq) return e;
  const int64_t n = (int64_t)p.B * p.T * p.H * (p.DV / (16 / (int)sizeof(E)));
  if (n >= (1ll << 31)) return -2;
  hipLaunchKernelGGL((branch_combine_kernel<E, 0>), dim3((unsigned)((n + 255) / 256)), dim3(256), 0, st, p,
                     combine_div(p, (int)sizeof(E)));
  return (int)hipGetLastError();
}

template <class E, bool DROP>
int dispatch_fwd(const FwdParams& p, hipStream_t st) {
#define DTA_F(HS_, N_, DV_) \
  if (p.HS == HS_ && p.N == N_ && p.DV == DV_) { \
    if constexpr (Plan<E, HS_, N_, DV_>::ok) return launch_fwd_t<E, HS_, N_, DV_, DROP>(p, st); }
  DTA_FOR_CONFIGS(DTA_F)
#undef DTA_F
  if (p.N >= 2) return fwd_branch_split_any<E, DROP>(p, st);
  return -2;
}

template <class E, bool DROP>
int dispatch_dq(const BwdParams& p, hipStream_t st) {
#define DTA_Q(HS_, N_, DV_) \
  if (p.HS == HS_ && p.N == N_ && p.DV == DV_) { \
    if constexpr (Plan<E, HS_, N_, DV_>::ok) return launch_dq_t<E, HS_, N_, DV_, DROP>(p, st); else return -2; }
  DTA_FOR_CONFIGS(DTA_Q)
#undef DTA_Q
  return -2;
}

template <class E, bool DROP>
int dispatch_dkdv(const BwdParams& p, hipStream_t st) {
#define DTA_K(HS_, N_, DV_) \
  if (p.HS == HS_ && p.N == N_ && p.DV == DV_) { \
    if constexpr (Plan<E, HS_, N_, DV_>::ok) return launch_dkdv_t<E, HS_, N_, DV_, DROP>(p, st); else return -2; }
  DTA_FOR_CONFIGS(DTA_K)
#undef DTA_K
  return -2;
}

}
```

### differential_transformer_replication_amd/csrc/capi.hip

```cpp
#include "../../include/diffattn.h"
#include "dta_internal.h"

namespace dta {
int launch_attn_fwd_bf16(const FwdParams&, hipStream_t);
int launch_attn_fwd_f16(const FwdParams&, hipStream_t);
int launch_attn_fwd_f32(const FwdParams&, hipStream_t);
int launch_attn_dq_bf16(const BwdParams&, hipStream_t);
int launch_attn_dq_f16(const BwdParams&, hipStream_t);
int launch_attn_dq_f32(const BwdParams&, hipStream_t);
int launch_attn_dkdv_bf16(const BwdParams&, hipStream_t);
int launch_attn_dkdv_f16(const BwdParams&, hipStream_t);
int launch_attn_dkdv_f32(const BwdParams&, hipStream_t);
int launch_attn_fwd_bf16_drop(const FwdParams&, hipStream_t);
int launch_attn_fwd_f16_drop(const FwdParams&, hipStream_t);
int launch_attn_fwd_f32_drop(const FwdParams&, hipStream_t);
int launch_attn_dq_bf16_drop(const BwdParams&, hipStream_t);
int launch_attn_dq_f16_drop(const BwdParams&, hipStream_t);
int launch_attn_dq_f32_drop(const BwdParams&, hipStream_t);
int launch_attn_dkdv_bf16_drop(const BwdParams&, hipStream_t);
int launch_attn_dkdv_f16_drop(const BwdParams&, hipStream_t);
int launch_attn_dkdv_f32_drop(const BwdParams&, hipStream_t);
bool attn_native_bf16(int, int, int);
bool attn_native_f16(int, int, int);
bool attn_native_f32(int, int, int);

int launch_attn_fwd(int dtype, const FwdParams& p, hipStream_t st) {
  if (p.drop_thr) switch (dtype) {
    case DTA_BF16: return launch_attn_fwd_bf16_drop(p, st);
    case DTA_F16: return launch_attn_fwd_f16_drop(p, st);
    case DTA_F32: return launch_attn_fwd_f32_drop(p, st);
  }
  switch (dtype) {
    case DTA_BF16: return launch_attn_fwd_bf16(p, st);
    case DTA_F16: return launch_attn_fwd_f16(p, st);
    case DTA_F32: return launch_attn_fwd_f32(p, st);
  }
  return -2;
}
int launch_attn_dq(int dtype, const BwdParams& p, hipStream_t st) {
  if (p.drop_thr) switch (dtype) {
    case DTA_BF16: return launch_attn_dq_bf16_drop(p, st);
    case DTA_F16: return launch_attn_dq_f16_drop(p, st);
    case DTA_F32: return launch_attn_dq_f32_drop(p, st);
  }
  switch (dtype) {
    case DTA_BF16: return launch_attn_dq_bf16(p, st);
    case DTA_F16: return launch_attn_dq_f16(p, st);
    case DTA_F32: return launch_attn_dq_f32(p, st);
  }
  return -2;
}
int launch_attn_dkdv(int dtype, const BwdParams& p, hipStream_t st) {
  if (p.drop_thr) switch (dtype) {
    case DTA_BF16: return launch_attn_dkdv_bf16_drop(p, st);
    case DTA_F16: return launch_attn_dkdv_f16_drop(p, st);
    case DTA_F32: return launch_attn_dkdv_f32_drop(p, st);
  }
  switch (dtype) {
    case DTA_BF16: return launch_attn_dkdv_bf16(p, st);
    case DTA_F16: return launch_attn_dkdv_f16(p, st);
    case DTA_F32: return launch_attn_dkdv_f32(p, st);
  }
  return -2;
}
bool attn_native(int dtype, int hs, int n, int dv) {
  if (dv != 2 * hs && !(n == 1 && dv == hs)) return false;
  switch (dtype) {
    case DTA_BF16: return attn_native_bf16(hs, n, dv);
    case DTA_F16: return attn_native_f16(hs, n, dv);
    case DTA_F32: return attn_native_f32(hs, n, dv);
  }
  return false;
}
bool attn_supported(int dtype, int hs, int n, int dv) {
  if (n < 1) return false;
  return attn_native(dtype, hs, n, dv) || (n >= 2 && dv == 2 * hs && attn_native(dtype, hs, 1, dv));
}
int branch_group(int dtype, int hs, int left, int dv, int cap) {
  for (int g = left < cap ? left : cap; g > 1; --g)
    if (attn_native(dtype, hs, g, dv)) return g;
  return 1;
}
int bwd_group_cap(int dtype, int hs, int n, bool dkdv) {
  if (dtype == DTA_F32) return 4;
  if (hs >= 192) return 1;
  if (dkdv) return hs >= 64 ? 2 : 4;
  return (hs >= 128 || (hs >= 64 && hs < 96 && n >= 4)) ? 2 : 4;
}
uint64_t group_starts(int dtype, int hs, int n, int dv, int cap) {
  uint64_t m = 0;
  for (int g0 = 0, ng; g0 < n; g0 += ng) {
    ng = branch_group(dtype, hs, n - g0, dv, cap);
    m |= 1ull << g0;
  }
  return m;
}
}

using namespace dta;

namespace {

constexpr float kLog2e = 1.4426950408889634f;

int esize(int dtype) { return dtype == DTA_F32 ? 4 : 2; }

bool drop_params(float p, uint64_t seed, uint32_t& thr, float& scale, uint32_t& lo, uint32_t& hi) {
  if (!(p >= 0.f && p < 1.f)) return false;
  const double t = (double)p * 4294967296.0;
  thr = p > 0.f ? (uint32_t)(t < 1.0 ? 1.0 : (t > 4294967295.0 ? 4294967295.0 : t)) : 0u;
  scale = p > 0.f ? (float)(1.0 / (1.0 - (double)p)) : 1.f;
  lo = (uint32_t)seed;
  hi = (uint32_t)(seed >> 32);
  return true;
}

int vec_elems(int dtype) { return 16 / esize(dtype); }

bool aligned_ptr(const void* p) { return p && (reinterpret_cast<uintptr_t>(p) % 16) == 0; }

bool ok_tensor(const dta_tensor& t, int dtype, bool with_i) {
  const int64_t v = vec_elems(dtype);
  if (!aligned_ptr(t.ptr)) return false;
  if (t.sb % v || t.st % v || t.sh % v) return false;
  if (with_i && t.si % v) return false;
  return t.sb >= 0 && t.st >= 0 && t.sh >= 0 && t.si >= 0;
}

T5 t5(const dta_tensor& t) { return T5{t.ptr, t.sb, t.st, t.sh, t.si}; }

bool ok_obr(const dta_tensor& t, int obr_dtype, int dtype) {
  if (obr_dtype == DTA_F16) return dtype != DTA_F32 && ok_tensor(t, DTA_F16, true);
  return (obr_dtype == 0 || obr_dtype == DTA_F32) && ok_tensor(t, DTA_F32, true);
}

int status(int e) {
  if (e == 0) return DTA_OK;
  if (e == -2) return DTA_ERR_UNSUPPORTED;
  return DTA_ERR_LAUNCH;
}

bool ok_dims(int dtype, int B, int T, int H, int N, int hs, int dv) {
  if (dtype < DTA_BF16 || dtype > DTA_F32) return false;
  return B >= 0 && T >= 0 && H > 0 && N > 0 && hs > 0 && dv > 0;
}

}

#ifndef DTA_STAMPS
#define DTA_STAMPS 0
#endif
#if DTA_STAMPS
static unsigned long long* stamp_buf() {
  static unsigned long long* b = [] {
    void* p = nullptr;
    if (hipMalloc(&p, 64 << 20) || hipMemset(p, 0, 64 << 20)) p = nullptr;
    return (unsigned long long*)p;
  }();
  return b;
}
#else
static unsigned long long* stamp_buf() { return nullptr; }
#endif

extern "C" {

#if DTA_STAMPS
int dta_debug_stamps(void* dst, size_t bytes) {
  if (!stamp_buf() || bytes > (64u << 20)) return DTA_ERR_INVALID;
  return hipMemcpy(dst, stamp_buf(), bytes, hipMemcpyDeviceToHost) ? DTA_ERR_LAUNCH : DTA_OK;
}
#endif

int dta_abi_version(void) { return DTA_ABI_VERSION; }

const char* dta_error_string(int code) {
  switch (code) {
    case DTA_OK: return "ok";
    case DTA_ERR_INVALID: return "invalid argument (shape, null/misaligned pointer or stride)";
    case DTA_ERR_UNSUPPORTED: return "unsupported configuration (head_size/n_terms/dtype not built for gfx950)";
    case DTA_ERR_LAUNCH: return "HIP launch failed";
    case DTA_ERR_DROPOUT: return "attention dropout p must lie in [0, 1)";
  }
  return "unknown error";
}

int dta_supported(int32_t dtype, int32_t head_size, int32_t n_terms, int32_t dv) {
  return attn_supported(dtype, head_size, n_terms, dv) ? 1 : 0;
}

int dta_attn_fwd(const dta_attn_fwd_args* a, void* stream) {
  if (!a) return DTA_ERR_INVALID;
  if (!ok_dims(a->dtype, a->B, a->T, a->H, a->n_terms, a->head_size, a->dv)) return DTA_ERR_INVALID;
  FwdParams p{};
  if (!drop_params(a->dropout_p, a->dropout_seed, p.drop_thr, p.drop_scale, p.drop_seed_lo, p.drop_seed_hi))
    return DTA_ERR_DROPOUT;
  if (!attn_supported(a->dtype, a->head_size, a->n_terms, a->dv)) return DTA_ERR_UNSUPPORTED;
  if ((int64_t)a->B * a->T == 0) return DTA_OK;
  if (!ok_tensor(a->q, a->dtype, true) || !ok_tensor(a->k, a->dtype, true) || !ok_tensor(a->v, a->dtype, false) ||
      !ok_tensor(a->o, a->dtype, false) || !ok_obr(a->obr, a->obr_dtype, a->dtype) || !a->lse || !a->coef)
    return DTA_ERR_INVALID;
  p.ob16 = a->obr_dtype == DTA_F16;
  p.q = t5(a->q); p.k = t5(a->k); p.v = t5(a->v); p.o = t5(a->o); p.obr = t5(a->obr);
  p.lse = a->lse; p.coef = a->coef;
  p.B = a->B; p.T = a->T; p.H = a->H; p.N = a->n_terms; p.HS = a->head_size; p.DV = a->dv;
  p.sl2 = a->scale * kLog2e;
  p.cst = a->n_terms;
  if (a->rope_freqs) {
    if (a->head_size % 2 || ((uintptr_t)a->rope_freqs & 15) || !ok_tensor(a->q_rot, a->dtype, true)) return DTA_ERR_INVALID;
    p.rope = a->rope_freqs;
    p.qrot = t5(a->q_rot);
  }
  p.stamps = stamp_buf();
  return status(launch_attn_fwd(a->dtype, p, (hipStream_t)stream));
}

int dta_attn_bwd_dkdv_groups(int32_t dtype, int32_t head_size, int32_t n_terms, int32_t dv, int32_t group_max_dkdv) {
  if (!attn_supported(dtype, head_size, n_terms, dv) || group_max_dkdv < 0) return 0;
  const int cap = group_max_dkdv > 0 ? group_max_dkdv : bwd_group_cap(dtype, head_size, n_terms, true);
  int n = 0;
  for (int g0 = 0, ng; g0 < n_terms; g0 += ng, ++n) ng = branch_group(dtype, head_size, n_terms - g0, dv, cap);
  return n;
}

size_t dta_attn_bwd_dcoef_partial_bytes(int32_t B, int32_t T, int32_t H, int32_t n_terms) {
  return (size_t)H * n_terms * B * ((T + 31) / 32) * 4;
}

size_t dta_attn_bwd_workspace_bytes(int32_t B, int32_t T, int32_t H, int32_t n_terms, int32_t head_size) {
  const size_t delta = (size_t)n_terms * B * H * T * 4;
  const size_t dq = (size_t)B * T * H * n_terms * head_size * 4;
  return delta + dq;
}

int dta_attn_bwd(const dta_attn_bwd_args* a, void* stream) {
  if (!a) return DTA_ERR_INVALID;
  if (!ok_dims(a->dtype, a->B, a->T, a->H, a->n_terms, a->head_size, a->dv)) return DTA_ERR_INVALID;
  BwdParams p{};
  if (!drop_params(a->dropout_p, a->dropout_seed, p.drop_thr, p.drop_scale, p.drop_seed_lo, p.drop_seed_hi))
    return DTA_ERR_DROPOUT;
  if (!attn_supported(a->dtype, a->head_size, a->n_terms, a->dv)) return DTA_ERR_UNSUPPORTED;
  if (!a->dcoef) return DTA_ERR_INVALID;
  hipStream_t st = (hipStream_t)stream;
  const int stages = a->stages ? a->stages : (DTA_BWD_PRE | DTA_BWD_DQ | DTA_BWD_DKDV);
  const bool empty = (int64_t)a->B * a->T == 0;
  if (((stages & DTA_BWD_PRE) && !a->dcoef_partial) || (empty && (stages & DTA_BWD_DQ))) {
    if (hipMemsetAsync(a->dcoef, 0, sizeof(float) * a->H * a->n_terms, st)) return DTA_ERR_LAUNCH;
  }
  if (empty) return DTA_OK;
  if (!ok_tensor(a->q, a->dtype, true) || !ok_tensor(a->k, a->dtype, true) || !ok_tensor(a->v, a->dtype, false) ||
      !ok_obr(a->obr, a->obr_dtype, a->dtype) || !ok_tensor(a->dout, a->dtype, false) ||
      !ok_tensor(a->dk, a->dtype, true) || !ok_tensor(a->dv_out, a->dtype, false) ||
      !a->lse || !a->coef || !a->delta)
    return DTA_ERR_INVALID;
  if (a->dq.ptr ? !ok_tensor(a->dq, a->dtype, true) : !aligned_ptr(a->dq_f32)) return DTA_ERR_INVALID;
  p.q = t5(a->q); p.k = t5(a->k); p.v = t5(a->v); p.obr = t5(a->obr); p.dout = t5(a->dout);
  p.ob16 = a->obr_dtype == DTA_F16;
  p.dq = t5(a->dq); p.dk = t5(a->dk); p.dv = t5(a->dv_out);
  p.lse = a->lse; p.delta = a->delta; p.coef = a->coef; p.dcoef = a->dcoef;
  p.dq32 = a->dq.ptr ? nullptr : a->dq_f32;
  if (a->rope_freqs && (a->head_size % 4 || reinterpret_cast<uintptr_t>(a->rope_freqs) % 16)) return DTA_ERR_INVALID;
  p.rope = a->rope_freqs;
  if (a->dcoef_partial && !aligned_ptr(a->dcoef_partial)) return DTA_ERR_INVALID;
  if (a->dv_f32 && !aligned_ptr(a->dv_f32)) return DTA_ERR_INVALID;
  if (a->lse_c && !aligned_ptr(a->lse_c)) return DTA_ERR_INVALID;
  p.lsec = (a->lse_c && a->dtype != DTA_F32 && !p.drop_thr) ? a->lse_c : nullptr;
  p.dcoef_part = a->dcoef_partial;
  p.B = a->B; p.T = a->T; p.H = a->H; p.N = a->n_terms; p.HS = a->head_size; p.DV = a->dv;
  p.scale = a->scale; p.sl2 = a->scale * kLog2e;
  p.cst = a->n_terms; p.br0 = 0; p.dv_acc = 0;
  p.stamps = stamp_buf();
  const int es = esize(a->dtype);
  const int64_t rowvec = (int64_t)p.B * p.H * p.T, nblk = (p.T + 31) / 32;
  auto group = [&](int g0, int ng) {
    BwdParams q = p;
    auto off = [&](T5& t) { t.p = (char*)t.p + (int64_t)g0 * t.si * es; };
    off(q.q); off(q.k); off(q.dk);
    q.obr.p = (char*)q.obr.p + (int64_t)g0 * q.obr.si * (p.ob16 ? 2 : 4);
    if (q.dq.p) off(q.dq);
    if (q.dq32) q.dq32 += (int64_t)g0 * p.HS;
    q.lse += g0 * rowvec; q.delta += g0 * rowvec; q.coef += g0; q.dcoef += g0;
    if (q.lsec) q.lsec += g0 * rowvec;
    if (q.dcoef_part) q.dcoef_part += g0 * (int64_t)p.B * nblk;
    q.N = ng; q.br0 = g0; q.dv_acc = g0 > 0; q.dv_last = g0 + ng == p.N;
    return q;
  };
  int e = 0;
  if (a->group_max_dq < 0 || a->group_max_dkdv < 0) return DTA_ERR_INVALID;
  const int kcap = a->group_max_dkdv ? a->group_max_dkdv : bwd_group_cap(a->dtype, p.HS, p.N, true);
  int qcap = a->group_max_dq ? a->group_max_dq : bwd_group_cap(a->dtype, p.HS, p.N, false);
  if (p.N > 64) qcap = kcap;
  const bool rebase = qcap != kcap && !p.drop_thr;
  const uint64_t qstarts = rebase ? group_starts(a->dtype, p.HS, p.N, p.DV, qcap) : 0;
  const uint64_t kstarts = rebase ? group_starts(a->dtype, p.HS, p.N, p.DV, kcap) : 0;
  if (stages & DTA_BWD_DQ) {
    const bool direct = qstarts != kstarts && branch_group(a->dtype, p.HS, p.N, p.DV, qcap) == p.N;
    for (int g0 = 0, ng; g0 < p.N; g0 += ng) {
      ng = branch_group(a->dtype, p.HS, p.N - g0, p.DV, qcap);
      BwdParams q = group(g0, ng);
      q.kstarts = direct ? kstarts : 0;
      if ((e = launch_attn_dq(a->dtype, q, st))) return status(e);
    }
    if (p.dcoef_part &&
        (e = launch_dcoef_reduce(p.dcoef_part, p.dcoef, p.H, p.N, (int64_t)p.B * nblk, st)))
      return status(e);
    if (!direct && qstarts != kstarts && (e = launch_delta_rebase(p.delta, rowvec, p.N, qstarts, kstarts, st)))
      return status(e);
  }
  if (stages & DTA_BWD_DKDV) {
    const bool multi = branch_group(a->dtype, p.HS, p.N, p.DV, kcap) < p.N;
    for (int g0 = 0, ng; g0 < p.N; g0 += ng) {
      ng = branch_group(a->dtype, p.HS, p.N - g0, p.DV, kcap);
      BwdParams q = group(g0, ng);
      q.dv32 = multi ? a->dv_f32 : nullptr;
      if ((e = launch_attn_dkdv(a->dtype, q, st))) return status(e);
    }
  }
  return DTA_OK;
}

static int ln_common(const dta_ln_args* a, bool bwd) {
  if (!a || a->dtype < DTA_BF16 || a->dtype > DTA_F32 || a->rows < 0 || a->C <= 0) return DTA_ERR_INVALID;
  if (a->io_dtype != 0 && (a->dtype != DTA_F32 || (a->io_dtype - 1 != DTA_BF16 && a->io_dtype - 1 != DTA_F16)))
    return DTA_ERR_UNSUPPORTED;
  const int64_t v = 8;
  if (a->C % v || a->C > 8192) return DTA_ERR_UNSUPPORTED;
  if (a->rows == 0) return DTA_OK;
  if (!aligned_ptr(a->x) || a->x_stride % v || !a->w || !a->mean || !a->rstd) return DTA_ERR_INVALID;
  if (!bwd && (!aligned_ptr(a->y) || a->y_stride % v || !a->b)) return DTA_ERR_INVALID;
  if (bwd && (!aligned_ptr(a->dy) || !aligned_ptr(a->dx) || a->dy_stride % v || a->dx_stride % v || !a->dw || !a->db))
    return DTA_ERR_INVALID;
  const bool fused = bwd ? (a->dres || a->dx16) : (a->res || a->xo);
  if (fused && a->io_dtype == 0) return DTA_ERR_UNSUPPORTED;
  if (!bwd && fused && (!aligned_ptr(a->res) || !aligned_ptr(a->xo) || a->res_stride % v || a->xo_stride % v))
    return DTA_ERR_INVALID;
  if (bwd && a->partial && !aligned_ptr(a->partial)) return DTA_ERR_INVALID;
  if (bwd && a->dres && (!aligned_ptr(a->dres) || a->dres_stride % v)) return DTA_ERR_INVALID;
  if (bwd && a->dx16 && (!aligned_ptr(a->dx16) || a->dx16_stride % v)) return DTA_ERR_INVALID;
  return DTA_OK;
}

static LnParams ln_params(const dta_ln_args* a) {
  LnParams p{};
  p.rows = a->rows; p.C = a->C; p.eps = a->eps; p.out_scale = a->out_scale;
  p.x = a->x; p.xs = a->x_stride; p.y = a->y; p.ys = a->y_stride;
  p.w = a->w; p.b = a->b; p.mean = a->mean; p.rstd = a->rstd;
  p.dy = a->dy; p.dys = a->dy_stride; p.dx = a->dx; p.dxs = a->dx_stride;
  p.dw = a->dw; p.db = a->db;
  p.partial = a->partial;
  p.res = a->res; p.ress = a->res_stride; p.xo = a->xo; p.xos = a->xo_stride;
  p.dres = a->dres; p.dress = a->dres_stride; p.dx16 = a->dx16; p.dx16s = a->dx16_stride;
  return p;
}

int dta_ln_fwd(const dta_ln_args* a, void* stream) {
  if (int e = ln_common(a, false)) return e;
  if (a->io_dtype) return status(launch_ln_mixed(a->io_dtype - 1, ln_params(a), false, (hipStream_t)stream));
  return status(launch_ln(a->dtype, ln_params(a), false, (hipStream_t)stream));
}

size_t dta_ln_bwd_workspace_bytes(int64_t rows, int64_t C) { return (size_t)ln_bwd_workspace_floats(rows, C) * 4; }

int dta_ln_bwd(const dta_ln_args* a, void* stream) {
  if (int e = ln_common(a, true)) return e;
  if (a->io_dtype) return status(launch_ln_mixed(a->io_dtype - 1, ln_params(a), true, (hipStream_t)stream));
  return status(launch_ln(a->dtype, ln_params(a), true, (hipStream_t)stream));
}

int dta_rope(const dta_rope_args* a, void* stream) {
  if (!a || !ok_dims(a->dtype, a->B, a->T, a->H, a->n_terms, a->head_size, 1)) return DTA_ERR_INVALID;
  if (a->head_size % 8) return DTA_ERR_UNSUPPORTED;
  if ((int64_t)a->B * a->T == 0) return DTA_OK;
  const int src_dtype = a->src_f32 ? DTA_F32 : a->dtype;
  if (!ok_tensor(a->src, src_dtype, true) || !ok_tensor(a->dst, a->dtype, true) || !aligned_ptr(a->freqs))
    return DTA_ERR_INVALID;
  RopeParams p{};
  p.src = t5(a->src); p.dst = t5(a->dst); p.freqs = a->freqs;
  p.B = a->B; p.T = a->T; p.H = a->H; p.N = a->n_terms; p.HS = a->head_size; p.inverse = a->inverse ? 1 : 0;
  return status(launch_rope(a->dtype, a->src_f32 != 0, p, (hipStream_t)stream));
}

static int swiglu_common(const dta_swiglu_args* a, bool bwd, SwigluParams& p) {
  if (!a || a->dtype < DTA_BF16 || a->dtype > DTA_F32 || a->rows < 0 || a->n < 0) return DTA_ERR_INVALID;
  if (a->n % 8) return DTA_ERR_UNSUPPORTED;
  const bool none = a->rows == 0 || a->n == 0;
  auto ok = [none](const void* q, int64_t st) { return (none || aligned_ptr(q)) && st % 8 == 0 && st >= 0; };
  if (!ok(a->a, a->a_stride) || !ok(a->b, a->b_stride)) return DTA_ERR_INVALID;
  if (!bwd && !ok(a->out, a->out_stride)) return DTA_ERR_INVALID;
  if (bwd && (!ok(a->dout, a->dout_stride) || !ok(a->da, a->da_stride) || !ok(a->db, a->db_stride)))
    return DTA_ERR_INVALID;
  p = SwigluParams{a->rows, a->n, a->a, a->a_stride, a->b, a->b_stride, a->out, a->out_stride,
                   a->dout, a->dout_stride, a->da, a->da_stride, a->db, a->db_stride};
  return DTA_OK;
}

int dta_swiglu_fwd(const dta_swiglu_args* a, void* stream) {
  SwigluParams p;
  if (int e = swiglu_common(a, false, p)) return e;
  return status(launch_swiglu(a->dtype, p, false, (hipStream_t)stream));
}

int dta_swiglu_bwd(const dta_swiglu_args* a, void* stream) {
  SwigluParams p;
  if (int e = swiglu_common(a, true, p)) return e;
  if (a->dbias) {
    if (!aligned_ptr(a->dbias) || !aligned_ptr(a->dbias_work)) return DTA_ERR_INVALID;
    if (a->rows == 0 || a->n == 0) return status(hipMemsetAsync(a->dbias, 0, sizeof(float) * 2 * a->n, (hipStream_t)stream));
    return status(launch_swiglu_bias(a->dtype, p, a->dbias, a->dbias_work, (hipStream_t)stream));
  }
  return status(launch_swiglu(a->dtype, p, true, (hipStream_t)stream));
}

size_t dta_swiglu_bwd_workspace_bytes(int64_t rows, int64_t n) {
  return rows < 0 || n < 0 ? 0 : (size_t)swiglu_bias_work_floats(rows, n) * 4;
}

int dta_accumulate_f32(int32_t dtype, int64_t n, const void* src, float* dst, void* stream) {
  if (dtype < DTA_BF16 || dtype > DTA_F32 || n < 0) return DTA_ERR_INVALID;
  if (n == 0) return DTA_OK;
  if (!aligned_ptr(src) || !aligned_ptr(dst)) return DTA_ERR_INVALID;
  return status(launch_accumulate(dtype, n, src, dst, (hipStream_t)stream));
}

int dta_cast_f32(int32_t dtype, int32_t B, int32_t T, int32_t H, int32_t n_terms, int32_t head_size,
                 const float* src, dta_tensor dst, void* stream) {
  if (!ok_dims(dtype, B, T, H, n_terms, head_size, 1) || head_size % 8) return DTA_ERR_INVALID;
  if ((int64_t)B * T == 0) return DTA_OK;
  if (!aligned_ptr(src) || !ok_tensor(dst, dtype, true)) return DTA_ERR_INVALID;
  return status(launch_cast(dtype, src, t5(dst), B, T, H, n_terms, head_size, (hipStream_t)stream));
}

static int64_t decode_splits(int32_t t_cap) { return (t_cap + DTA_DECODE_CHUNK - 1) / DTA_DECODE_CHUNK; }

size_t dta_attn_decode_workspace_bytes(int32_t B, int32_t H, int32_t n_terms, int32_t head_size, int32_t dv,
                                       int32_t t_cap) {
  const size_t single = (size_t)B * H * n_terms * t_cap * 4;
  const size_t split = (size_t)B * H * decode_splits(t_cap) * n_terms * (dv + 2) * 4;
  return single > split ? single : split;
}

static int page_shift(int page_size) {
  switch (page_size) {
    case 32: return 5;
    case 64: return 6;
    case 128: return 7;
    case 256: return 8;
    default: return 0;
  }
}

extern "C++" template <class A>
static bool page_table(const A* a, PageTable& g) {
  if (!a->block_table_dev || (uintptr_t)a->block_table_dev % 4) return false;
  const int shift = page_shift(a->page_size);
  if (!shift) return false;
  if (a->n_pages < 1 || a->max_pages < 1 || (int64_t)a->max_pages * a->page_size != a->t_cap) return false;
  g = PageTable{a->block_table_dev, a->max_pages, shift, a->n_pages};
  return true;
}

static bool ok_byte_pool(const dta_tensor& t, int width, bool with_i) {
  const int64_t v = width % 16 ? 8 : 16;
  if (!aligned_ptr(t.ptr) || t.sb % 16 || t.st % 16 || t.sh % v || (with_i && t.si % v)) return false;
  return t.sb >= 0 && t.st >= 0 && t.sh >= 0 && t.si >= 0;
}

extern "C++" template <class A>
static int decode_call(const A* a, const dta_tensor& kc, const dta_tensor& vc, const int32_t* ldev, int lsb,
                       const PageTable& pg, void* stream, const float* scales = nullptr, int64_t scales_sb = 0) {
  if (!ok_dims(a->dtype, a->B, 1, a->H, a->n_terms, a->head_size, a->dv)) return DTA_ERR_INVALID;
  if (a->head_size % 8 || a->head_size > 128 || a->n_terms > 4 || a->dv > 256) return DTA_ERR_UNSUPPORTED;
  if (a->length < 1 || a->t_cap < a->length) return DTA_ERR_INVALID;
  if ((int64_t)a->B * a->H == 0) return DTA_OK;
  if (!ok_tensor(a->q, a->dtype, true) || !ok_tensor(a->o, a->dtype, false) || !a->coef || !aligned_ptr(a->workspace))
    return DTA_ERR_INVALID;
  if (scales ? !ok_byte_pool(kc, a->head_size, true) || !ok_byte_pool(vc, a->dv, false)
             : !ok_tensor(kc, a->dtype, true) || !ok_tensor(vc, a->dtype, false))
    return DTA_ERR_INVALID;
  DecodeParams p{};
  p.q = t5(a->q); p.k = t5(kc); p.v = t5(vc); p.o = t5(a->o); p.pg = pg;
  p.coef = a->coef; p.ws = a->workspace;
  p.B = a->B; p.H = a->H; p.N = a->n_terms; p.HS = a->head_size; p.DV = a->dv;
  p.L = a->length; p.ldw = a->t_cap; p.scale = a->scale; p.Ldev = ldev; p.Lsb = lsb;
  p.S = (int)decode_splits(a->length);
  p.ml = a->workspace + (int64_t)a->B * a->H * p.S * a->n_terms * a->dv;
  if (scales) {
    p.kvs = scales; p.kvs_sb = scales_sb;
    return status(launch_decode_f8(a->dtype, p, (hipStream_t)stream));
  }
  return status(launch_decode(a->dtype, p, (hipStream_t)stream));
}

int dta_attn_decode(const dta_attn_decode_args* a, void* stream) {
  if (!a) return DTA_ERR_INVALID;
  return decode_call(a, a->k_cache, a->v_cache, a->length_dev, 0, PageTable{}, stream);
}

int dta_attn_decode_ragged(const dta_attn_decode_ragged_args* a, void* stream) {
  if (!a || !a->lengths_dev || (uintptr_t)a->lengths_dev % 4) return DTA_ERR_INVALID;
  return decode_call(a, a->k_cache, a->v_cache, a->lengths_dev, 1, PageTable{}, stream);
}

int dta_attn_decode_paged(const dta_attn_decode_paged_args* a, void* stream) {
  PageTable pg{};
  if (!a || !a->lengths_dev || (uintptr_t)a->lengths_dev % 4 || !page_table(a, pg)) return DTA_ERR_INVALID;
  return decode_call(a, a->k_pool, a->v_pool, a->lengths_dev, 1, pg, stream);
}

int dta_attn_decode_paged_fp8(const dta_attn_decode_paged_fp8_args* a, void* stream) {
  PageTable pg{};
  if (!a || !a->lengths_dev || (uintptr_t)a->lengths_dev % 4 || !page_table(a, pg)) return DTA_ERR_INVALID;
  if (!a->scale_pool_dev || (uintptr_t)a->scale_pool_dev % 4) return DTA_ERR_INVALID;
  if (a->H > 0 && a->n_terms > 0 && a->scale_page_stride < (int64_t)a->page_size * a->H * (a->n_terms + 1))
    return DTA_ERR_INVALID;
  if (a->k_pool.sb % 16 || a->k_pool.st % 16 || a->v_pool.sb % 16 || a->v_pool.st % 16) return DTA_ERR_INVALID;
  return decode_call(a, a->k_pool, a->v_pool, a->lengths_dev, 1, pg, stream, a->scale_pool_dev, a->scale_page_stride);
}

int dta_kv_quant_rows(const dta_kv_quant_rows_args* a, void* stream) {
  if (!a || !ok_dims(a->dtype, a->B, a->Tn, a->H, a->n_terms, a->head_size, a->dv)) return DTA_ERR_INVALID;
  if (a->head_size % 16 || a->dv % 16 || a->head_size > 128 || a->dv > 256 || a->n_terms > 4)
    return DTA_ERR_UNSUPPORTED;
  const int shift = page_shift(a->page_size);
  if (!shift) return DTA_ERR_INVALID;
  if (a->n_pages < 1 || ((int64_t)a->n_pages + 1) * a->page_size > INT32_MAX) return DTA_ERR_INVALID;
  if (!a->slot_dev || (uintptr_t)a->slot_dev % 4 || !a->scale_pool_dev || (uintptr_t)a->scale_pool_dev % 4 ||
      a->scale_page_stride < (int64_t)a->page_size * a->H * (a->n_terms + 1))
    return DTA_ERR_INVALID;
  if ((int64_t)a->B * a->Tn == 0) return DTA_OK;
  if (!ok_tensor(a->k_new, a->dtype, true) || !ok_tensor(a->v_new, a->dtype, false) ||
      !ok_byte_pool(a->k_pool, a->head_size, true) || !ok_byte_pool(a->v_pool, a->dv, false))
    return DTA_ERR_INVALID;
  KvQuantParams p{};
  p.ksrc = t5(a->k_new); p.vsrc = t5(a->v_new); p.kdst = t5(a->k_pool); p.vdst = t5(a->v_pool);
  p.kvs = a->scale_pool_dev; p.kvs_sb = a->scale_page_stride; p.slot = a->slot_dev;
  p.B = a->B; p.Tn = a->Tn; p.H = a->H; p.N = a->n_terms; p.HS = a->head_size; p.DV = a->dv;
  p.shift = shift; p.slots = (a->n_pages + 1) * a->page_size;
  return status(launch_kv_quant(a->dtype, p, (hipStream_t)stream));
}

int dta_extend_supported(int32_t dtype, int32_t head_size, int32_t n_terms, int32_t dv) {
  return extend_supported(dtype, head_size, n_terms, dv) ? 1 : 0;
}

int dta_extend_fp8_supported(int32_t dtype, int32_t head_size, int32_t n_terms, int32_t dv) {
  return extend_f8_supported(dtype, head_size, n_terms, dv) ? 1 : 0;
}

extern "C++" template <class A>
static int extend_call(const A* a, const dta_tensor& kc, const dta_tensor& vc, int pos, const int32_t* pos_dev,
                       const int32_t* cnt_dev, const PageTable& pg, void* stream, const float* scales = nullptr,
                       int64_t scales_sb = 0) {
  if (!ok_dims(a->dtype, a->B, a->Tq, a->H, a->n_terms, a->head_size, a->dv)) return DTA_ERR_INVALID;
  if (scales ? !extend_f8_supported(a->dtype, a->head_size, a->n_terms, a->dv)
             : !extend_supported(a->dtype, a->head_size, a->n_terms, a->dv))
    return DTA_ERR_UNSUPPORTED;
  if (pos < 0 || a->t_cap < 0 || (int64_t)pos + a->Tq > a->t_cap) return DTA_ERR_INVALID;
  if (a->Tq == 0 || (int64_t)a->B * a->H == 0) return DTA_OK;
  if (!ok_tensor(a->q, a->dtype, true) || !ok_tensor(a->o, a->dtype, false) || !a->coef) return DTA_ERR_INVALID;
  if (scales ? !ok_byte_pool(kc, a->head_size, true) || !ok_byte_pool(vc, a->dv, false)
             : !ok_tensor(kc, a->dtype, true) || !ok_tensor(vc, a->dtype, false))
    return DTA_ERR_INVALID;
  ExtendParams p{};
  p.q = t5(a->q); p.k = t5(kc); p.v = t5(vc); p.o = t5(a->o); p.pg = pg;
  p.coef = a->coef;
  p.B = a->B; p.H = a->H; p.N = a->n_terms; p.HS = a->head_size; p.DV = a->dv;
  p.Tq = a->Tq; p.pos = pos; p.sl2 = a->scale * kLog2e;
  p.pos_dev = pos_dev; p.cnt_dev = cnt_dev; p.cap = a->t_cap;
  if (scales) {
    p.kvs = scales; p.kvs_sb = scales_sb;
    return status(launch_extend_f8(a->dtype, p, (hipStream_t)stream));
  }
  return status(launch_extend(a->dtype, p, (hipStream_t)stream));
}

int dta_attn_extend(const dta_attn_extend_args* a, void* stream) {
  if (!a) return DTA_ERR_INVALID;
  return extend_call(a, a->k_cache, a->v_cache, a->pos, nullptr, nullptr, PageTable{}, stream);
}

int dta_attn_extend_ragged(const dta_attn_extend_ragged_args* a, void* stream) {
  if (!a || !a->pos_dev || (uintptr_t)a->pos_dev % 4 || (uintptr_t)a->count_dev % 4) return DTA_ERR_INVALID;
  return extend_call(a, a->k_cache, a->v_cache, 0, a->pos_dev, a->count_dev, PageTable{}, stream);
}

int dta_attn_extend_paged(const dta_attn_extend_paged_args* a, void* stream) {
  PageTable pg{};
  if (!a || !a->pos_dev || (uintptr_t)a->pos_dev % 4 || (uintptr_t)a->count_dev % 4 || !page_table(a, pg))
    return DTA_ERR_INVALID;
  return extend_call(a, a->k_pool, a->v_pool, 0, a->pos_dev, a->count_dev, pg, stream);
}

int dta_attn_extend_paged_fp8(const dta_attn_extend_paged_fp8_args* a, void* stream) {
  PageTable pg{};
  if (!a || !a->pos_dev || (uintptr_t)a->pos_dev % 4 || (uintptr_t)a->count_dev % 4 || !page_table(a, pg))
    return DTA_ERR_INVALID;
  if (!a->scale_pool_dev || (uintptr_t)a->scale_pool_dev % 4) return DTA_ERR_INVALID;
// ... 9 lines not shown
```

### differential_transformer_replication_amd/csrc/dta_internal.h

```cpp
#pragma once
#include <hip/hip_runtime.h>
#include <stdint.h>

namespace dta {

struct T5 {
  void* p;
  int64_t sb, st, sh, si;
};

struct FwdParams {
  T5 q, k, v, o, obr;
  float* lse;
  const float* coef;
  int B, T, H, N, HS, DV;
  float sl2;
  unsigned long long* stamps;
  uint32_t drop_thr;
  float drop_scale;
  uint32_t drop_seed_lo, drop_seed_hi;
  int bsplit;
  int bseq;
  int cst;
  const float* rope;
  T5 qrot;
  int ob16;
};

struct BwdParams {
  T5 q, k, v, obr, dout, dq, dk, dv;
  const float* lse;
  float* delta;
  const float* coef;
  float* dcoef;
  float* dq32;
  const float* rope;
  float* dcoef_part;
  int B, T, H, N, HS, DV;
  float sl2, scale;
  unsigned long long* stamps;
  uint32_t drop_thr;
  float drop_scale;
  uint32_t drop_seed_lo, drop_seed_hi;
  int cst;
  int br0;
  int dv_acc;
  float* dv32;
  int dv_last;
  int ob16;
  float* lsec;
  uint64_t kstarts;
};

int launch_attn_fwd(int dtype, const FwdParams& p, hipStream_t st);
int launch_attn_fwd_drop(int dtype, const FwdParams& p, hipStream_t st);
int launch_attn_dq_drop(int dtype, const BwdParams& p, hipStream_t st);
int launch_attn_dkdv_drop(int dtype, const BwdParams& p, hipStream_t st);
int launch_attn_dq(int dtype, const BwdParams& p, hipStream_t st);
int launch_attn_dkdv(int dtype, const BwdParams& p, hipStream_t st);
bool attn_supported(int dtype, int hs, int n, int dv);
bool attn_native(int dtype, int hs, int n, int dv);

struct LnParams {
  int64_t rows, C;
  float eps, out_scale;
  const void* x; int64_t xs;
  void* y; int64_t ys;
  const float* w; const float* b;
  float* mean; float* rstd;
  const void* dy; int64_t dys;
  void* dx; int64_t dxs;
  float* dw; float* db;
  float* partial;
  const void* res; int64_t ress;
  float* xo; int64_t xos;
  const float* dres; int64_t dress;
  void* dx16; int64_t dx16s;
};
int launch_ln_mixed(int y_dtype, const LnParams& p, bool bwd, hipStream_t st);
int ln_bwd_blocks(int64_t rows);
int64_t ln_bwd_workspace_floats(int64_t rows, int64_t C);

struct RopeParams {
  T5 src, dst;
  const float* freqs;
  int B, T, H, N, HS;
  int inverse;
};

#ifndef DTA_DECODE_CHUNK
#define DTA_DECODE_CHUNK 256
#endif

struct PageTable {
  const int* tbl;
  int max_pages;
  int shift;
  int n_pages;
};
__device__ __forceinline__ int page_of(const PageTable& g, int b, int j) {
  return min(max(g.tbl[(int64_t)b * g.max_pages + (j >> g.shift)], 0), g.n_pages - 1);
}

struct DecodeParams {
  T5 q, k, v, o;
  const float* coef;
  float* ws;
  float* ml;
  int B, H, N, HS, DV, L, ldw, S;
  float scale;
  const int* Ldev;
  int Lsb;
  PageTable pg;
  const float* kvs;
  int64_t kvs_sb;
};

int launch_decode(int dtype, const DecodeParams& p, hipStream_t st);
int launch_decode_f8(int dtype, const DecodeParams& p, hipStream_t st);

struct KvQuantParams {
  T5 ksrc, vsrc;
  T5 kdst, vdst;
  float* kvs;
  int64_t kvs_sb;
  const int* slot;
  int B, Tn, H, N, HS, DV;
  int shift;
  int slots;
};
int launch_kv_quant(int dtype, const KvQuantParams& p, hipStream_t st);

struct ExtendParams {
  T5 q, k, v, o;
  const float* coef;
  int B, H, N, HS, DV;
  int Tq, pos;
  float sl2;
  const int* pos_dev;
  const int* cnt_dev;
  int cap;
  PageTable pg;
  const float* kvs;
  int64_t kvs_sb;
};

int launch_extend(int dtype, const ExtendParams& p, hipStream_t st);
bool extend_supported(int dtype, int hs, int n, int dv);
int launch_extend_f8(int dtype, const ExtendParams& p, hipStream_t st);
bool extend_f8_supported(int dtype, int hs, int n, int dv);
int launch_ln(int dtype, const LnParams& p, bool bwd, hipStream_t st);
int launch_rope(int dtype, bool src_f32, const RopeParams& p, hipStream_t st);
int launch_dcoef_reduce(const float* part, float* dcoef, int H, int N, int64_t per, hipStream_t st);
int launch_delta_rebase(float* delta, int64_t rows, int N, uint64_t from, uint64_t to, hipStream_t st);
int launch_cast(int dtype, const float* src, const T5& dst, int B, int T, int H, int N, int HS, hipStream_t st);

struct SwigluParams {
  int64_t rows, n;
  const void* a; int64_t as;
  const void* b; int64_t bs;
  void* out; int64_t os;
  const void* dout; int64_t dos;
  void* da; int64_t das;
  void* db; int64_t dbs;
};
int launch_swiglu(int dtype, const SwigluParams& p, bool bwd, hipStream_t st);
int launch_accumulate(int dtype, int64_t n, const void* src, float* dst, hipStream_t st);
int launch_swiglu_bias(int dtype, const SwigluParams& p, float* dbias, float* work, hipStream_t st);
int64_t swiglu_bias_work_floats(int64_t rows, int64_t n);

}
```

### differential_transformer_replication_amd/csrc/layout_checks.h

```cpp
#pragma once
#include <stdint.h>

namespace dta {

inline bool dma_rows_ok(int64_t T, int64_t st, int64_t si, int n, int width, int es) {
  if (T <= 0) return true;
  if (st <= 0 || si < 0 || width > st) return false;
  if (n > 1 && si > (st - width) / (n - 1)) return false;
  return st <= ((1ll << 31) - 1) / (T * es);
}

inline bool dma_rowvecs_ok(int64_t n, int64_t B, int64_t H, int64_t T) {
  const int64_t lim = ((1ll << 31) - 1) / 4;
  if (n <= 0 || B <= 0 || H <= 0 || T <= 0) return true;
  if (n > lim || B > lim || H > lim || T > lim) return false;
  if (n * B > lim || n * B * H > lim) return false;
  return n * B * H * T <= lim;
}

}
```

### differential_transformer_replication_amd/ops.py

```python
from __future__ import annotations

import contextlib
import math
import os
from typing import Dict, List, Optional, Tuple

import torch
from torch.nn import functional as F

from . import _lib, packing

Tensor = torch.Tensor


def _require_gpu(*ts: Tensor) -> None:
    for t in ts:
        if t is not None and t.device.type != "cuda":
            raise RuntimeError("differential_transformer_replication_amd ops run only on the MI355X "
                               "HIP path (libdiffattn.so); got a tensor on " + str(t.device))


class KernelTimer:

    def __init__(self):
        self.active = False
        self._pairs: Dict[str, List[Tuple[torch.cuda.Event, torch.cuda.Event]]] = {}

    def start(self):
        self._pairs = {}
        self.active = True

    def stop(self):
        self.active = False

    @contextlib.contextmanager
    def region(self, name: str):
        if not self.active:
            yield
            return
        e0, e1 = torch.cuda.Event(enable_timing=True), torch.cuda.Event(enable_timing=True)
        e0.record()
        yield
        e1.record()
        self._pairs.setdefault(name, []).append((e0, e1))

    def mean_ms(self) -> Dict[str, Tuple[float, int]]:
        torch.cuda.synchronize()
        return {k: (sum(a.elapsed_time(b) for a, b in v) / len(v), len(v)) for k, v in self._pairs.items()}


TIMER = KernelTimer()


def supported(dtype: torch.dtype, hs: int, N: int, dv: int) -> bool:
    return bool(_lib.load().dta_supported(_lib.dtype_code(dtype), hs, N, dv))


def padded_head(dtype: torch.dtype, hs: int, N: int, dv: int) -> Optional[int]:
    if N < 1 or hs < 1 or dv not in (hs, 2 * hs) or (dv == hs and N != 1):
        return None
    for hp in (hs,) + tuple(h for h in (16, 32, 64, 96, 128, 256) if h > hs):
        if supported(dtype, hp, N, hp if dv == hs else 2 * hp):
            return hp
    return None


def attention_supported(dtype: torch.dtype, hs: int, N: int, dv: int) -> bool:
    return padded_head(dtype, hs, N, dv) is not None


def packed_width(H: int, N: int, hs: int, dv: int) -> int:
    return 2 * H * N * hs + H * dv


def split_packed(qkv: Tensor, H: int, N: int, hs: int, dv: int):
    B, T, W = qkv.shape
    nq = H * N * hs
    q = qkv[..., :nq].unflatten(-1, (H, N, hs))
    k = qkv[..., nq:2 * nq].unflatten(-1, (H, N, hs))
    v = qkv[..., 2 * nq:].unflatten(-1, (H, dv))
    return q, k, v


def _obr_dtype(dtype: torch.dtype) -> torch.dtype:
    if dtype != torch.float32 and os.environ.get("DTA_OBR_F16", "0") == "1":
        return torch.float16
    return torch.float32


_DV_F32_WORKSPACE = [True]
_LSE_C_WORKSPACE = [True]

_BWD_GROUP_MAX = [0, 0]


@contextlib.contextmanager
def bwd_group_caps(dq: int, dkdv: int):
    old = list(_BWD_GROUP_MAX)
    _BWD_GROUP_MAX[:] = [int(dq), int(dkdv)]
    try:
        yield
    finally:
        _BWD_GROUP_MAX[:] = old


class _DiffAttention(torch.autograd.Function):
    @staticmethod
    def forward(ctx, qkv: Tensor, coef: Tensor, H: int, N: int, hs: int, freqs: Optional[Tensor], dv: int,
                dropout_p: float, seed: int, scale: float):
        lib = _lib.load()
        _require_gpu(qkv, coef)
        if qkv.dim() != 3:
            raise RuntimeError("qkv must be (B, T, W)")
        qkv = qkv.contiguous()
        B, T, W = qkv.shape
        if W != packed_width(H, N, hs, dv):
            raise RuntimeError(f"packed width {W} != 2*H*N*hs + H*dv = {packed_width(H, N, hs, dv)}")
        dt = _lib.dtype_code(qkv.dtype)
        if not lib.dta_supported(dt, hs, N, dv):
            raise RuntimeError(f"no gfx950 kernel for head_size={hs}, n_terms={N}, dv={dv}, dtype={qkv.dtype}")
        coef = coef.detach().to(torch.float32).contiguous()
        dev = qkv.device
        stream = _lib.stream_handle(dev)
        q, k, v = split_packed(qkv, H, N, hs, dv)
        qk_rot = None
        rope_args = (None, _lib.DtaTensor())
        if freqs is not None:
            qk_rot = torch.empty(B, T, 2 * H, N, hs, device=dev, dtype=qkv.dtype)
            src = k
            ra = _lib.RopeArgs(dt, B, T, H, N, hs, 0, 0, _lib.tensor5(src), _lib.tensor5(qk_rot[:, :, H:]),
                               freqs.data_ptr())
            _lib.check(lib.dta_rope(ra, stream))
            k = qk_rot[:, :, H:]
            rope_args = (freqs.data_ptr(), _lib.tensor5(qk_rot[:, :, :H]))
        o = torch.empty(B, T, H, dv, device=dev, dtype=qkv.dtype)
        obr = torch.empty(N, B, T, H, dv, device=dev, dtype=_obr_dtype(qkv.dtype))
        lse = torch.empty(N, B, H, T, device=dev, dtype=torch.float32)
        obr_t = _lib.DtaTensor(obr.data_ptr(), *obr.stride()[1:4], obr.stride(0))
        a = _lib.AttnFwdArgs(dt, B, T, H, N, hs, dv, scale, dropout_p,
                             _lib.tensor5(q), _lib.tensor5(k), _lib.tensor5(v), _lib.tensor5(o), obr_t,
                             lse.data_ptr(), coef.data_ptr(), seed, *rope_args, _lib.dtype_code(obr.dtype))
        with TIMER.region("attn_fwd"):
            _lib.check(lib.dta_attn_fwd(a, stream))
        ctx.save_for_backward(qkv, qk_rot, obr, lse, coef, freqs)
        ctx.dims = (H, N, hs, dv, scale)
        ctx.drop = (dropout_p, seed)
        ctx.caps = tuple(_BWD_GROUP_MAX)
        return o.view(B, T, H * dv)

    @staticmethod
    def backward(ctx, do: Tensor):
        lib = _lib.load()
        qkv, qk_rot, obr, lse, coef, freqs = ctx.saved_tensors
        H, N, hs, dv, scale = ctx.dims
        B, T, W = qkv.shape
        dev = qkv.device
        stream = _lib.stream_handle(dev)
        dt = _lib.dtype_code(qkv.dtype)
        do = do.to(qkv.dtype).contiguous().view(B, T, H, dv)
        q, k, v = split_packed(qkv, H, N, hs, dv)
        if qk_rot is not None:
            q, k = qk_rot[:, :, :H], qk_rot[:, :, H:]
        dqkv = torch.empty_like(qkv)
        dq, dk, dvv = split_packed(dqkv, H, N, hs, dv)
        dcoef = torch.empty(H, N, device=dev, dtype=torch.float32)
        delta = torch.empty(N, B, H, T, device=dev, dtype=torch.float32)
        dcp = torch.empty(lib.dta_attn_bwd_dcoef_partial_bytes(B, T, H, N) // 4, device=dev, dtype=torch.float32)
        dv32 = None
        caps = ctx.caps
        if dt != _lib.DTA_F32 and _DV_F32_WORKSPACE[0] and lib.dta_attn_bwd_dkdv_groups(dt, hs, N, dv, caps[1]) > 1:
            dv32 = torch.empty(B, T, H, dv, device=dev, dtype=torch.float32)
        lsec = (torch.empty(N, B, H, T, device=dev, dtype=torch.float32)
                if dt != _lib.DTA_F32 and ctx.drop[0] == 0.0 and _LSE_C_WORKSPACE[0] else None)
        obr_t = _lib.DtaTensor(obr.data_ptr(), *obr.stride()[1:4], obr.stride(0))
        a = _lib.AttnBwdArgs(dt, B, T, H, N, hs, dv, scale, ctx.drop[0],
                             _lib.tensor5(q), _lib.tensor5(k), _lib.tensor5(v), obr_t,
                             lse.data_ptr(), coef.data_ptr(), _lib.tensor5(do),
                             _lib.tensor5(dq), _lib.tensor5(dk), _lib.tensor5(dvv),
                             dcoef.data_ptr(), delta.data_ptr(), None, _lib.BWD_PRE,
                             freqs.data_ptr() if freqs is not None else None, dcp.data_ptr(), ctx.drop[1],
                             _lib.dtype_code(obr.dtype), *caps,
                             dv32.data_ptr() if dv32 is not None else None,
                             lsec.data_ptr() if lsec is not None else None)
        a.stages = _lib.BWD_DQ
        with TIMER.region("attn_bwd_dq"):
            _lib.check(lib.dta_attn_bwd(a, stream))
        a.stages = _lib.BWD_DKDV
        with TIMER.region("attn_bwd_dkdv"):
            _lib.check(lib.dta_attn_bwd(a, stream))
        return dqkv, dcoef, None, None, None, None, None, None, None, None


def diff_attention(qkv: Tensor, coef: Tensor, H: int, N: int, hs: int,
                   freqs: Optional[Tensor] = None, dv: Optional[int] = None, dropout_p: float = 0.0,
                   seed: Optional[int] = None) -> Tensor:
    if freqs is not None:
        freqs = freqs.to(device=qkv.device, dtype=torch.float32).contiguous()
    dropout_p = float(dropout_p)
    if not 0.0 <= dropout_p < 1.0:
        raise ValueError(f"dropout probability has to be in [0, 1), got {dropout_p}")
    if seed is None:
        seed = int(torch.randint(0, 2 ** 62, (1,)).item()) if dropout_p > 0 else 0
    dv = 2 * hs if dv is None else dv
    scale = 1.0 / math.sqrt(hs)
    hp = padded_head(qkv.dtype, hs, N, dv) if qkv.is_cuda else hs
    if hp is None:
        raise RuntimeError(f"no gfx950 kernel for head_size={hs}, n_terms={N}, dv={dv}, dtype={qkv.dtype} "
                           "(head sizes up to 256 are served; 129-256 in 16-bit for the differential models)")
    if hp == hs:
        return _DiffAttention.apply(qkv, coef, H, N, hs, freqs, dv, dropout_p, int(seed), scale)
    dvp = hp if dv == hs else 2 * hp
    B, T, _ = qkv.shape
    q, k, v = split_packed(qkv, H, N, hs, dv)
    qkv_p = torch.cat([F.pad(q, (0, hp - hs)).flatten(2), F.pad(k, (0, hp - hs)).flatten(2),
                       F.pad(v, (0, dvp - dv)).flatten(2)], dim=-1)
    if freqs is not None:
        pad = torch.zeros(freqs.shape[0], (hp - hs) // 2, 2, device=freqs.device, dtype=freqs.dtype)
        pad[..., 0] = 1.0
        freqs = torch.cat([freqs, pad], dim=1).contiguous()
    out = _DiffAttention.apply(qkv_p, coef, H, N, hp, freqs, dvp, dropout_p, int(seed), scale)
    return out.view(B, T, H, dvp)[..., :dv].reshape(B, T, H * dv)


class _GroupLNScale(torch.autograd.Function):
    @staticmethod
    def forward(ctx, x: Tensor, w: Tensor, b: Tensor, eps: float, out_scale: float, holder=None,
                y_dtype: Optional[torch.dtype] = None):
        lib = _lib.load()
        _require_gpu(x, w, b)
        ctx.bound = (holder, (w, b)) if holder is not None and "grad" in holder else None
        C = x.shape[-1]
        x2 = x.contiguous().view(-1, C)
        rows = x2.shape[0]
        w32 = w.detach().to(torch.float32).contiguous().view(-1)
        b32 = b.detach().to(torch.float32).contiguous().view(-1)
        if w32.numel() != C or b32.numel() != C:
            raise RuntimeError("GroupLayerNorm weight/bias size must equal the normalised width")
        io = 0
        if y_dtype is not None and y_dtype != x.dtype:
            if x.dtype != torch.float32 or y_dtype not in (torch.bfloat16, torch.float16):
                raise RuntimeError("LayerNorm output dtype may differ only for fp32 input and 16-bit output")
            io = 1 + _lib.dtype_code(y_dtype)
        y = torch.empty(x2.shape, device=x.device, dtype=y_dtype if io else x.dtype)
        mean = torch.empty(rows, device=x.device, dtype=torch.float32)
        rstd = torch.empty_like(mean)
        a = _lib.LnArgs(_lib.dtype_code(x.dtype), rows, C, eps, out_scale, x2.data_ptr(), C, y.data_ptr(), C,
                        w32.data_ptr(), b32.data_ptr(), mean.data_ptr(), rstd.data_ptr(), None, 0, None, 0,
                        None, None, None, io)
        ctx.io = (io, y.dtype)
        _lib.check(lib.dta_ln_fwd(a, _lib.stream_handle(x.device)))
        ctx.save_for_backward(x2, w32, mean, rstd)
        ctx.meta = (eps, out_scale, x.shape, w.dtype, w.shape, b.dtype, b.shape)
        return y.view(x.shape)

    @staticmethod
    def backward(ctx, dy: Tensor):
        lib = _lib.load()
        x2, w32, mean, rstd = ctx.saved_tensors
        eps, out_scale, xshape, wdt, wshape, bdt, bshape = ctx.meta
        C = x2.shape[1]
        io, ydt = ctx.io
        dy2 = dy.to(ydt).contiguous().view(-1, C)
        dx = torch.empty_like(x2)
        g = None
        if ctx.bound is not None and ctx.needs_input_grad[1] and ctx.needs_input_grad[2]:
            holder, params = ctx.bound
            g = packing._grad_target(holder, params)
            if g is not None and g.numel() != 2 * C:
                g = None
        if g is not None:
            dw, db = g[:C], g[C:]
        else:
            dw = torch.zeros(C, device=x2.device, dtype=torch.float32)
            db = torch.zeros(C, device=x2.device, dtype=torch.float32)
        part = torch.empty(lib.dta_ln_bwd_workspace_bytes(x2.shape[0], C) // 4, device=x2.device, dtype=torch.float32)
        a = _lib.LnArgs(_lib.dtype_code(x2.dtype), x2.shape[0], C, eps, out_scale, x2.data_ptr(), C, None, 0,
                        w32.data_ptr(), None, mean.data_ptr(), rstd.data_ptr(), dy2.data_ptr(), C,
                        dx.data_ptr(), C, dw.data_ptr(), db.data_ptr(), part.data_ptr(), io)
        _lib.check(lib.dta_ln_bwd(a, _lib.stream_handle(x2.device)))
        if g is not None:
            hook = ctx.bound[0]["on_ready"]
            for p in ctx.bound[1]:
                hook(p)
            return dx.view(xshape), None, None, None, None, None, None
        return dx.view(xshape), dw.to(wdt).view(wshape), db.to(bdt).view(bshape), None, None, None, None


class _AddLN(torch.autograd.Function):

    @staticmethod
    def forward(ctx, x: Tensor, a: Tensor, w: Tensor, b: Tensor, eps: float, holder, ydt: torch.dtype):
        lib = _lib.load()
        _require_gpu(x, a, w, b)
        C = x.shape[-1]
        x2 = x.contiguous().view(-1, C)
        a2 = a.to(ydt).contiguous().view(-1, C)
        rows = x2.shape[0]
        w32 = w.detach().to(torch.float32).contiguous().view(-1)
        b32 = b.detach().to(torch.float32).contiguous().view(-1)
        xo = torch.empty_like(x2)
        y = torch.empty(x2.shape, device=x.device, dtype=ydt)
        mean = torch.empty(rows, device=x.device, dtype=torch.float32)
        rstd = torch.empty_like(mean)
        io = 1 + _lib.dtype_code(ydt)
        args = _lib.LnArgs(_lib.DTA_F32, rows, C, eps, 1.0, x2.data_ptr(), C, y.data_ptr(), C,
                           w32.data_ptr(), b32.data_ptr(), mean.data_ptr(), rstd.data_ptr(), None, 0, None, 0,
                           None, None, None, io, a2.data_ptr(), C, xo.data_ptr(), C)
        _lib.check(lib.dta_ln_fwd(args, _lib.stream_handle(x.device)))
        ctx.bound = (holder, (w, b)) if holder is not None and "grad" in holder else None
        ctx.save_for_backward(xo, w32, mean, rstd)
        ctx.meta = (eps, x.shape, a.dtype, ydt, w.dtype, w.shape, b.dtype, b.shape, io)
        return xo.view(x.shape), y.view(x.shape)

    @staticmethod
    def backward(ctx, dxo: Optional[Tensor], dy: Optional[Tensor]):
        lib = _lib.load()
        xo, w32, mean, rstd = ctx.saved_tensors
        eps, xshape, adt, ydt, wdt, wshape, bdt, bshape, io = ctx.meta
        C = xo.shape[1]
        dy2 = (dy.to(ydt).contiguous().view(-1, C) if dy is not None
               else torch.zeros(xo.shape, device=xo.device, dtype=ydt))
        dres = dxo.to(torch.float32).contiguous().view(-1, C) if dxo is not None else None
        dx = torch.empty_like(xo)
        da = torch.empty(xo.shape, device=xo.device, dtype=ydt)
        g = None
        if ctx.bound is not None and ctx.needs_input_grad[2] and ctx.needs_input_grad[3]:
            holder, params = ctx.bound
            g = packing._grad_target(holder, params)
            if g is not None and g.numel() != 2 * C:
                g = None
        if g is not None:
            dw, db = g[:C], g[C:]
        else:
            dw = torch.zeros(C, device=xo.device, dtype=torch.float32)
            db = torch.zeros(C, device=xo.device, dtype=torch.float32)
        part = torch.empty(lib.dta_ln_bwd_workspace_bytes(xo.shape[0], C) // 4, device=xo.device, dtype=torch.float32)
        args = _lib.LnArgs(_lib.DTA_F32, xo.shape[0], C, eps, 1.0, xo.data_ptr(), C, None, 0, w32.data_ptr(), None,
                           mean.data_ptr(), rstd.data_ptr(), dy2.data_ptr(), C, dx.data_ptr(), C, dw.data_ptr(),
                           db.data_ptr(), part.data_ptr(), io, None, 0, None, 0,
                           dres.data_ptr() if dres is not None else None, C, da.data_ptr(), C)
        _lib.check(lib.dta_ln_bwd(args, _lib.stream_handle(xo.device)))
        da_out = da.view(xshape).to(adt)
        if g is not None:
            hook = ctx.bound[0]["on_ready"]
            for p in ctx.bound[1]:
                hook(p)
            return dx.view(xshape), da_out, None, None, None, None, None
        return dx.view(xshape), da_out, dw.to(wdt).view(wshape), db.to(bdt).view(bshape), None, None, None


def add_layer_norm(x: Tensor, a: Tensor, ln: "LayerNorm"):
    C = x.shape[-1]
    if (x.is_cuda and x.dtype == torch.float32 and isinstance(ln, LayerNorm) and ln.autocast_out
            and torch.is_autocast_enabled("cuda") and ln.weight is not None and ln.bias is not None
            and len(ln.normalized_shape) == 1 and C % 8 == 0 and C <= 8192 and a.shape == x.shape
            and a.dtype in (torch.bfloat16, torch.float16)):
        ydt = torch.get_autocast_dtype("cuda")
        with torch.autocast("cuda", enabled=False):
            return _AddLN.apply(x, a, ln.weight, ln.bias, ln.eps, ln._gpack, ydt)
    xo = x + a
    return xo, ln(xo)


def group_ln_scale(x: Tensor, w: Tensor, b: Tensor, eps: float = 1e-5, out_scale: float = 1.0,
                   holder: Optional[Dict] = None) -> Tensor:
    return _GroupLNScale.apply(x, w, b, eps, out_scale, holder, None)


class LayerNorm(torch.nn.LayerNorm):

    def __init__(self, *args, autocast_out: bool = False, **kwargs):
        super().__init__(*args, **kwargs)
        self._gpack = {}
        self.autocast_out = autocast_out

    def param_packs(self):
        return [(self._gpack, [self.weight, self.bias])] if self.weight is not None and self.bias is not None else []

    def forward(self, x: Tensor) -> Tensor:
        C = x.shape[-1]
        if (not x.is_cuda or len(self.normalized_shape) != 1 or self.weight is None or self.bias is None
                or C % 8 or C > 8192):
            return super().forward(x)
        ydt = None
        if torch.is_autocast_enabled("cuda"):
            if x.dtype != torch.float32:
                x = x.float()
            if self.autocast_out:
                ydt = torch.get_autocast_dtype("cuda")
        with torch.autocast("cuda", enabled=False):
            return _GroupLNScale.apply(x, self.weight, self.bias, self.eps, 1.0, self._gpack, ydt)


class _SwiGLU(torch.autograd.Function):
    @staticmethod
    def forward(ctx, a: Tensor, b: Tensor):
        lib = _lib.load()
        _require_gpu(a, b)
        if a.shape != b.shape:
            raise RuntimeError("SwiGLU branches must have one shape")
        dt = torch.promote_types(a.dtype, b.dtype)
        a2 = a.to(dt).contiguous().view(-1, a.shape[-1])
        b2 = b.to(dt).contiguous().view(-1, a.shape[-1])
        out = torch.empty_like(a2)
        n = a2.shape[1]
        sa = _lib.SwigluArgs(_lib.dtype_code(dt), a2.shape[0], n, a2.data_ptr(), n, b2.data_ptr(), n,
                             out.data_ptr(), n, None, 0, None, 0, None, 0)
        _lib.check(lib.dta_swiglu_fwd(sa, _lib.stream_handle(a.device)))
        ctx.save_for_backward(a2, b2)
        ctx.meta = (a.shape, a.dtype, b.dtype)
        return out.view(a.shape)

    @staticmethod
    def backward(ctx, dout: Tensor):
        lib = _lib.load()
        a2, b2 = ctx.saved_tensors
        shape, adt, bdt = ctx.meta
        n = a2.shape[1]
        d2 = dout.to(a2.dtype).contiguous().view(-1, n)
        da, db = torch.empty_like(a2), torch.empty_like(b2)
        sa = _lib.SwigluArgs(_lib.dtype_code(a2.dtype), a2.shape[0], n, a2.data_ptr(), n, b2.data_ptr(), n,
                             None, 0, d2.data_ptr(), n, da.data_ptr(), n, db.data_ptr(), n)
        _lib.check(lib.dta_swiglu_bwd(sa, _lib.stream_handle(a2.device)))
        return da.view(shape).to(adt), db.view(shape).to(bdt)


def swiglu(a: Tensor, b: Tensor) -> Tensor:
    if not a.is_cuda or a.shape[-1] % 8 or a.shape != b.shape:
        return F.silu(a) * b
    return _SwiGLU.apply(a, b)


def _swiglu_launch(y2: Tensor, n: int, out: Optional[Tensor], dout: Optional[Tensor], dy: Optional[Tensor],
                   dbias: Optional[Tensor] = None):
    lib = _lib.load()
    es, rows, w = y2.element_size(), y2.shape[0], 2 * n
    a, b = y2.data_ptr(), y2.data_ptr() + n * es
    if dy is None:
        sa = _lib.SwigluArgs(_lib.dtype_code(y2.dtype), rows, n, a, w, b, w, out.data_ptr(), n,
                             None, 0, None, 0, None, 0)
        _lib.check(lib.dta_swiglu_fwd(sa, _lib.stream_handle(y2.device)))
    else:
        work = None
        if dbias is not None:
            work = torch.empty(lib.dta_swiglu_bwd_workspace_bytes(rows, n) // 4 + 4, device=y2.device,
                               dtype=torch.float32)
        sa = _lib.SwigluArgs(_lib.dtype_code(y2.dtype), rows, n, a, w, b, w, None, 0, dout.data_ptr(), n,
                             dy.data_ptr(), w, dy.data_ptr() + n * es, w,
                             dbias.data_ptr() if dbias is not None else None,
                             work.data_ptr() if work is not None else None)
        _lib.check(lib.dta_swiglu_bwd(sa, _lib.stream_handle(y2.device)))


class _PackedSwiGLU(torch.autograd.Function):

    @staticmethod
    @torch.amp.custom_fwd(device_type="cuda")
    def forward(ctx, x, wbase, bbase, wholder, bholder, *params):
        dt = torch.get_autocast_dtype("cuda") if torch.is_autocast_enabled("cuda") else x.dtype
        xc = x.to(dt)
        wc, bc = wbase.to(dt), bbase.view(-1).to(dt)
        with torch.autocast("cuda", enabled=False):
            y = F.linear(xc, wc, bc)
        n = wc.shape[0] // 2
        y2 = y.view(-1, 2 * n)
        out = torch.empty(y2.shape[0], n, device=y.device, dtype=y.dtype)
        _swiglu_launch(y2, n, out, None, None)
        ctx.save_for_backward(xc, wc, y2)
        ctx.x_dtype, ctx.w_dtype, ctx.n = x.dtype, wbase.dtype, n
        ctx.wrows = [params[0].shape[0], params[1].shape[0]]
        bound = (wholder is not None and "grad" in wholder and bholder is not None and "grad" in bholder)
        ctx.holders = (wholder, bholder) if bound else None
        ctx.params = params if bound else None
        return out.view(*x.shape[:-1], n)

    @staticmethod
    @torch.amp.custom_bwd(device_type="cuda")
    def backward(ctx, dout):
        xc, wc, y2 = ctx.saved_tensors
        n = ctx.n
        d2 = dout.to(y2.dtype).contiguous().view(-1, n)
        dy = torch.empty_like(y2)
        db = torch.empty(2 * n, device=y2.device, dtype=torch.float32)
        _swiglu_launch(y2, n, None, d2, dy, db)
        with torch.autocast("cuda", enabled=False):
            dx = (dy @ wc).view(*xc.shape[:-1], xc.shape[-1]).to(ctx.x_dtype) if ctx.needs_input_grad[0] else None
            dw = packing.weight_grad(dy, xc.reshape(-1, xc.shape[-1]))
        if ctx.holders is not None and all(ctx.needs_input_grad[5:]):
            wh, bh = ctx.holders
            gw = packing._grad_target(wh, ctx.params[:2])
            gb = packing._grad_target(bh, ctx.params[2:])
            if gw is not None and gb is not None:
# ... 408 lines not shown
```

### include/diffattn.h

```cpp
#ifndef DIFFATTN_H_
#define DIFFATTN_H_

#include <stddef.h>
#include <stdint.h>

#ifdef __cplusplus
extern "C" {
#endif

#define DTA_ABI_VERSION 9

enum dta_dtype { DTA_BF16 = 0, DTA_F16 = 1, DTA_F32 = 2 };

enum dta_status {
  DTA_OK = 0,
  DTA_ERR_INVALID = -1,
  DTA_ERR_UNSUPPORTED = -2,
  DTA_ERR_LAUNCH = -3,
  DTA_ERR_DROPOUT = -4
};

typedef struct dta_tensor {
  void* ptr;
  int64_t sb, st, sh, si;
} dta_tensor;

typedef struct dta_attn_fwd_args {
  int32_t dtype;
  int32_t B, T, H, n_terms, head_size, dv;
  float scale;
  float dropout_p;
  dta_tensor q, k, v;
  dta_tensor o;
  dta_tensor obr;
  float* lse;
  const float* coef;
  uint64_t dropout_seed;
  const float* rope_freqs;
  dta_tensor q_rot;
  int32_t obr_dtype;
} dta_attn_fwd_args;

int dta_attn_fwd(const dta_attn_fwd_args* a, void* stream);

typedef struct dta_attn_bwd_args {
  int32_t dtype;
  int32_t B, T, H, n_terms, head_size, dv;
  float scale;
  float dropout_p;
  dta_tensor q, k, v, obr;
  const float* lse;
  const float* coef;
  dta_tensor dout;
  dta_tensor dq, dk, dv_out;
  float* dcoef;
  float* delta;
  float* dq_f32;
  int32_t stages;
  const float* rope_freqs;
  float* dcoef_partial;
  uint64_t dropout_seed;
  int32_t obr_dtype;
  int32_t group_max_dq;
  int32_t group_max_dkdv;
  float* dv_f32;
  float* lse_c;
} dta_attn_bwd_args;

enum { DTA_BWD_PRE = 1, DTA_BWD_DQ = 2, DTA_BWD_DKDV = 4 };

int dta_attn_bwd(const dta_attn_bwd_args* a, void* stream);
size_t dta_attn_bwd_workspace_bytes(int32_t B, int32_t T, int32_t H, int32_t n_terms,
                                    int32_t head_size);
size_t dta_attn_bwd_dcoef_partial_bytes(int32_t B, int32_t T, int32_t H, int32_t n_terms);
int dta_attn_bwd_dkdv_groups(int32_t dtype, int32_t head_size, int32_t n_terms, int32_t dv, int32_t group_max_dkdv);

typedef struct dta_ln_args {
  int32_t dtype;
  int64_t rows, C;
  float eps, out_scale;
  const void* x; int64_t x_stride;
  void* y; int64_t y_stride;
  const float* w; const float* b;
  float* mean; float* rstd;
  const void* dy; int64_t dy_stride;
  void* dx; int64_t dx_stride;
  float* dw; float* db;
  float* partial;
  int32_t io_dtype;
  const void* res; int64_t res_stride;
  float* xo; int64_t xo_stride;
  const float* dres; int64_t dres_stride;
  void* dx16; int64_t dx16_stride;
} dta_ln_args;

int dta_ln_fwd(const dta_ln_args* a, void* stream);
int dta_ln_bwd(const dta_ln_args* a, void* stream);
size_t dta_ln_bwd_workspace_bytes(int64_t rows, int64_t C);

typedef struct dta_rope_args {
  int32_t dtype;
  int32_t B, T, H, n_terms, head_size;
  int32_t inverse, src_f32;
  dta_tensor src, dst;
  const float* freqs;
} dta_rope_args;

int dta_rope(const dta_rope_args* a, void* stream);

typedef struct dta_attn_decode_args {
  int32_t dtype;
  int32_t B, H, n_terms, head_size, dv;
  int32_t length;
  int32_t t_cap;
  float scale;
  dta_tensor q, k_cache, v_cache, o;
  const float* coef;
  float* workspace;
  const int32_t* length_dev;
} dta_attn_decode_args;
int dta_attn_decode(const dta_attn_decode_args* a, void* stream);
size_t dta_attn_decode_workspace_bytes(int32_t B, int32_t H, int32_t n_terms, int32_t head_size, int32_t dv,
                                       int32_t t_cap);

typedef struct dta_attn_decode_ragged_args {
  int32_t dtype;
  int32_t B, H, n_terms, head_size, dv;
  int32_t length;
  int32_t t_cap;
  float scale;
  dta_tensor q, k_cache, v_cache, o;
  const float* coef;
  float* workspace;
  const int32_t* lengths_dev;
} dta_attn_decode_ragged_args;
int dta_attn_decode_ragged(const dta_attn_decode_ragged_args* a, void* stream);

typedef struct dta_attn_extend_args {
  int32_t dtype;
  int32_t B, H, n_terms, head_size, dv;
  int32_t Tq;
  int32_t pos;
  int32_t t_cap;
  float scale;
  dta_tensor q, k_cache, v_cache, o;
  const float* coef;
} dta_attn_extend_args;
int dta_attn_extend(const dta_attn_extend_args* a, void* stream);
int dta_extend_supported(int32_t dtype, int32_t head_size, int32_t n_terms, int32_t dv);

typedef struct dta_attn_extend_ragged_args {
  int32_t dtype;
  int32_t B, H, n_terms, head_size, dv;
  int32_t Tq;
  int32_t t_cap;
  float scale;
  dta_tensor q, k_cache, v_cache, o;
  const float* coef;
  const int32_t* pos_dev;
  const int32_t* count_dev;
} dta_attn_extend_ragged_args;
int dta_attn_extend_ragged(const dta_attn_extend_ragged_args* a, void* stream);

typedef struct dta_attn_decode_paged_args {
  int32_t dtype;
  int32_t B, H, n_terms, head_size, dv;
  int32_t length;
  int32_t t_cap;
  float scale;
  dta_tensor q, k_pool, v_pool, o;
  const float* coef;
  float* workspace;
  const int32_t* lengths_dev;
  int32_t page_size, max_pages, n_pages;
  const int32_t* block_table_dev;
} dta_attn_decode_paged_args;
int dta_attn_decode_paged(const dta_attn_decode_paged_args* a, void* stream);

typedef struct dta_attn_extend_paged_args {
  int32_t dtype;
  int32_t B, H, n_terms, head_size, dv;
  int32_t Tq;
  int32_t t_cap;
  float scale;
  dta_tensor q, k_pool, v_pool, o;
  const float* coef;
  const int32_t* pos_dev;
  const int32_t* count_dev;
  int32_t page_size, max_pages, n_pages;
  const int32_t* block_table_dev;
} dta_attn_extend_paged_args;
int dta_attn_extend_paged(const dta_attn_extend_paged_args* a, void* stream);

typedef struct dta_attn_decode_paged_fp8_args {
  int32_t dtype;
  int32_t B, H, n_terms, head_size, dv;
  int32_t length;
  int32_t t_cap;
  float scale;
  dta_tensor q, k_pool, v_pool, o;
  const float* coef;
  float* workspace;
  const int32_t* lengths_dev;
  int32_t page_size, max_pages, n_pages;
  const int32_t* block_table_dev;
  const float* scale_pool_dev;
  int64_t scale_page_stride;
} dta_attn_decode_paged_fp8_args;
int dta_attn_decode_paged_fp8(const dta_attn_decode_paged_fp8_args* a, void* stream);

typedef struct dta_kv_quant_rows_args {
  int32_t dtype;
  int32_t B, Tn, H, n_terms, head_size, dv;
  int32_t page_size, n_pages;
  dta_tensor k_new, v_new;
  dta_tensor k_pool, v_pool;
  float* scale_pool_dev;
  int64_t scale_page_stride;
  const int32_t* slot_dev;
} dta_kv_quant_rows_args;
int dta_kv_quant_rows(const dta_kv_quant_rows_args* a, void* stream);

typedef struct dta_attn_extend_paged_fp8_args {
  int32_t dtype;
  int32_t B, H, n_terms, head_size, dv;
  int32_t Tq;
  int32_t t_cap;
  float scale;
  dta_tensor q, k_pool, v_pool, o;
  const float* coef;
  const int32_t* pos_dev;
  const int32_t* count_dev;
  int32_t page_size, max_pages, n_pages;
  const int32_t* block_table_dev;
  const float* scale_pool_dev;
  int64_t scale_page_stride;
} dta_attn_extend_paged_fp8_args;
int dta_attn_extend_paged_fp8(const dta_attn_extend_paged_fp8_args* a, void* stream);
int dta_extend_fp8_supported(int32_t dtype, int32_t head_size, int32_t n_terms, int32_t dv);

typedef struct {
  int32_t dtype;
  int64_t rows, n;
  const void* a; int64_t a_stride;
  const void* b; int64_t b_stride;
  void* out; int64_t out_stride;
  const void* dout; int64_t dout_stride;
  void* da; int64_t da_stride;
  void* db; int64_t db_stride;
  float* dbias; float* dbias_work;
} dta_swiglu_args;
int dta_swiglu_fwd(const dta_swiglu_args* a, void* stream);
int dta_swiglu_bwd(const dta_swiglu_args* a, void* stream);
size_t dta_swiglu_bwd_workspace_bytes(int64_t rows, int64_t n);

int dta_accumulate_f32(int32_t dtype, int64_t n, const void* src, float* dst, void* stream);

int dta_cast_f32(int32_t dtype, int32_t B, int32_t T, int32_t H, int32_t n_terms,
                 int32_t head_size, const float* src, dta_tensor dst, void* stream);

const char* dta_error_string(int code);
int dta_abi_version(void);
int dta_supported(int32_t dtype, int32_t head_size, int32_t n_terms, int32_t dv);

#ifdef __cplusplus
}
#endif
#endif
```

Before: 557.6 TFLOP/s.

## Pack per-row lse and delta into interleaved 32-row blocks for dK/dV ring

The dQ pre-pass now writes coefficient-folded LSE and delta values into one packed buffer, laid out as 32-row blocks that interleave all N branches. The dK/dV kernel can then stage both row vectors for a tile with a single 64-lane DMA piece instead of several separate pieces. Ownership of that piece rotates across waves per tile to spread the load. This is meant to cut the number of row-vector loads and the per-tile staging overhead in the backward ring, at the cost of a new workspace layout, an extra API path and more complex wait counting.

```diff
diff --git a/differential_transformer_replication_amd/_lib.py b/differential_transformer_replication_amd/_lib.py
--- a/differential_transformer_replication_amd/_lib.py
+++ b/differential_transformer_replication_amd/_lib.py
@@ -24,9 +24,11 @@
            "dta_attn_decode_ragged", "dta_attn_extend_ragged",
            "dta_attn_decode_paged", "dta_attn_extend_paged",
            "dta_attn_decode_paged_fp8", "dta_kv_quant_rows",
-           "dta_attn_extend_paged_fp8", "dta_extend_fp8_supported")
+           "dta_attn_extend_paged_fp8", "dta_extend_fp8_supported",
+           "dta_attn_bwd_packed", "dta_attn_bwd_row_pack_bytes", "dta_attn_bwd_packs")
 FP8_EXPORTS = ("dta_attn_decode_paged_fp8", "dta_kv_quant_rows")
 FP8_EXTEND_EXPORTS = ("dta_attn_extend_paged_fp8", "dta_extend_fp8_supported")
+ROW_PACK_EXPORTS = ("dta_attn_bwd_packed", "dta_attn_bwd_row_pack_bytes", "dta_attn_bwd_packs")
 
 
 class DtaTensor(ctypes.Structure):
@@ -205,6 +207,13 @@
             lib.dta_attn_extend_paged_fp8.argtypes = [P(ExtendPagedFp8Args), ctypes.c_void_p]
             lib.dta_extend_fp8_supported.argtypes = [ctypes.c_int32] * 4
             lib.dta_attn_extend_paged_fp8.restype = lib.dta_extend_fp8_supported.restype = ctypes.c_int
+        if row_pack_symbols(lib):
+            lib.dta_attn_bwd_packed.argtypes = [P(AttnBwdArgs), ctypes.c_void_p, ctypes.c_void_p]
+            lib.dta_attn_bwd_packed.restype = ctypes.c_int
+            lib.dta_attn_bwd_row_pack_bytes.argtypes = [ctypes.c_int32] * 4
+            lib.dta_attn_bwd_row_pack_bytes.restype = ctypes.c_size_t
+            lib.dta_attn_bwd_packs.argtypes = [P(AttnBwdArgs)]
+            lib.dta_attn_bwd_packs.restype = ctypes.c_int
         if lib.dta_abi_version() != ABI_VERSION:
             raise RuntimeError(f"libdiffattn ABI {lib.dta_abi_version()} != expected {ABI_VERSION}")
         _lib = lib
@@ -217,6 +226,10 @@
 
 def fp8_extend_symbols(lib) -> bool:
     return all(hasattr(lib, name) for name in FP8_EXTEND_EXPORTS)
+
+
+def row_pack_symbols(lib) -> bool:
+    return all(hasattr(lib, name) for name in ROW_PACK_EXPORTS)
 
 
 def check(rc: int) -> None:
diff --git a/differential_transformer_replication_amd/csrc/attn_bf16.hip b/differential_transformer_replication_amd/csrc/attn_bf16.hip
--- a/differential_transformer_replication_amd/csrc/attn_bf16.hip
+++ b/differential_transformer_replication_amd/csrc/attn_bf16.hip
@@ -5,4 +5,5 @@
 int launch_attn_dq_bf16(const BwdParams& p, hipStream_t st) { return dispatch_dq<__bf16, false>(p, st); }
 int launch_attn_dkdv_bf16(const BwdParams& p, hipStream_t st) { return dispatch_dkdv<__bf16, false>(p, st); }
 bool attn_native_bf16(int hs, int n, int dv) { return native_t<__bf16>(hs, n, dv); }
+bool attn_dkdv_pack_ok_bf16(const BwdParams& p) { return dkdv_pack_ok_t<__bf16>(p); }
 }
diff --git a/differential_transformer_replication_amd/csrc/attn_f16.hip b/differential_transformer_replication_amd/csrc/attn_f16.hip
--- a/differential_transformer_replication_amd/csrc/attn_f16.hip
+++ b/differential_transformer_replication_amd/csrc/attn_f16.hip
@@ -5,4 +5,5 @@
 int launch_attn_dq_f16(const BwdParams& p, hipStream_t st) { return dispatch_dq<_Float16, false>(p, st); }
 int launch_attn_dkdv_f16(const BwdParams& p, hipStream_t st) { return dispatch_dkdv<_Float16, false>(p, st); }
 bool attn_native_f16(int hs, int n, int dv) { return native_t<_Float16>(hs, n, dv); }
+bool attn_dkdv_pack_ok_f16(const BwdParams& p) { return dkdv_pack_ok_t<_Float16>(p); }
 }
diff --git a/differential_transformer_replication_amd/csrc/attn_kernels.h b/differential_transformer_replication_amd/csrc/attn_kernels.h
--- a/differential_transformer_replication_amd/csrc/attn_kernels.h
+++ b/differential_transformer_replication_amd/csrc/attn_kernels.h
@@ -1187,6 +1187,12 @@
   float dhead = 0.f;
   const int64_t rs = (((int64_t)0 * p.B + b) * p.H + hh) * T + qrow;
   const int64_t bstride = (int64_t)p.B * p.H * T;
+  constexpr bool CANPACK = !DROP && dq_packs((int)sizeof(E), HS, N);
+  float* rcrow = nullptr;
+  if constexpr (CANPACK) {
+    if (p.rowc && hf == 0 && qrow < (T + 31) / 32 * 32)
+      rcrow = p.rowc + ((((int64_t)b * p.H + hh) * ((T + 31) / 32) + (qrow >> 5)) * (2 * N) << 5) + (qrow & 31);
+  }
 #pragma unroll
   for (int s = 0; s < NSV; ++s)
     df[s] = rowok ? O::load_global(gdo + (int64_t)qrow * p.dout.st + s * KS + hf * O::KH) : O::zero();
@@ -1206,7 +1212,8 @@
       }
     }
     lse[i] = rowok ? p.lse[rs + i * bstride] : 0.f;
-    if (p.lsec && rowok && hf == 0) p.lsec[rs + i * bstride] = lse[i] + __builtin_log2f(fabsf(coef[i]));
+    if (rcrow) rcrow[i * 32] = rowok ? lse[i] + __builtin_log2f(fabsf(coef[i])) : 0.f;
+    else if (p.lsec && rowok && hf == 0) p.lsec[rs + i * bstride] = lse[i] + __builtin_log2f(fabsf(coef[i]));
     float d = 0.f;
     if (rowok) {
 #pragma unroll
@@ -1226,7 +1233,8 @@
     del[i] = d;
     const bool kstart = i == 0 || ((p.kstarts >> i) & 1);
     if (kstart) dhead = d;
-    if (rowok && hf == 0) p.delta[rs + i * bstride] = DROP ? d : (kstart ? -d : dhead - d);
+    if (rcrow) rcrow[(N + i) * 32] = rowok ? (kstart ? -d : dhead - d) : 0.f;
+    else if (rowok && hf == 0) p.delta[rs + i * bstride] = DROP ? d : (kstart ? -d : dhead - d);
     float w = (rowok && hf == 0) ? d : 0.f;
 #pragma unroll
     for (int o = 32; o > 0; o >>= 1) w += __shfl_xor(w, o, 64);
@@ -1523,7 +1531,7 @@
       }
 }
 
-template <class E, int HS, int N, int DV, int NW, bool DELTA, int BQ_ = 32, bool ROWS = true>
+template <class E, int HS, int N, int DV, int NW, bool DELTA, int BQ_ = 32, bool ROWS = true, bool PACK = false>
 struct TileRing {
   static constexpr int ES = (int)sizeof(E), BQ = BQ_;
   static constexpr int NP = (N * BQ + 63) / 64 * 64;
@@ -1532,11 +1540,34 @@
   static constexpr int OFF_D = N * QB, OFF_L = OFF_D + DB, OFF_G = OFF_L + NP * 4;
   static constexpr int SB = ROWS ? OFF_G + NP * 4 : OFF_L;
   static constexpr int PQ = N * QB / 1024, PD = DB / 1024, PL = NP / 64;
-  static constexpr int NPC = PQ + PD + (ROWS ? (DELTA ? 2 : 1) * PL : 0);
+  static constexpr int NPC = PQ + PD + (ROWS ? (PACK ? 1 : (DELTA ? 2 : 1) * PL) : 0);
   static constexpr int MYP = (NPC + NW - 1) / NW;
   static constexpr bool ok = ES == 2 && HS >= 32 && QB % 1024 == 0 && DB % 1024 == 0;
-
-  __device__ static int pieces(int wave) { return NPC / NW + (wave < NPC % NW ? 1 : 0); }
+  static constexpr int UR = (PQ + PD) / NW, WR = (PQ + PD) % NW, PLN = (DELTA ? 16 : 8) * N;
+  static constexpr bool ROT = PACK && WR == 0;
+  static constexpr bool pack_ok = ok && ROWS && BQ == 32 && N <= 4;
+  static_assert(!PACK || pack_ok, "packed row constants: one piece of at most 64 lanes");
+
+  __device__ static int pieces(int wave, int tt = 0) {
+    if constexpr (ROT) return UR + (tt % NW == wave ? 1 : 0);
+    else return NPC / NW + (wave < NPC % NW ? 1 : 0);
+  }
+  template <int CMAX>
+  __device__ static int pieces_of(int wave, int tt0, int c) {
+    if constexpr (ROT) {
+      int n = c * UR;
+#pragma unroll
+      for (int d = 0; d < CMAX; ++d) n += (d < c && (tt0 + d) % NW == wave) ? 1 : 0;
+      return n;
+    } else {
+      return c * pieces(wave);
+    }
+  }
+  __device__ static uint32_t offp(const BwdParams& p, int lane) {
+    const int c = min(lane >> 3, (DELTA ? 2 : 1) * N - 1);
+    const int col = c < N ? p.br0 + c : p.cst + p.br0 + (c - N);
+    return (uint32_t)(col * 128 + (lane & 7) * 16);
+  }
 
   __device__ static uint32_t offq(const BwdParams& p, int j, int lane) {
     using QI = Img<E, HSP>;
@@ -1565,11 +1596,13 @@
       const int j = u * NW + wave;
       if constexpr ((u + 1) * NW <= PQ) off[u] = offq(p, j, lane);
       else if constexpr (u * NW >= PQ && (u + 1) * NW <= PQ + PD) off[u] = offd(p, j, lane);
+      else if constexpr (PACK) off[u] = j < PQ ? offq(p, j, lane) : (j < PQ + PD ? offd(p, j, lane) : offp(p, lane));
       else off[u] = j < PQ ? offq(p, j, lane) : (j < PQ + PD ? offd(p, j, lane) : (j < NPC ? offr(j, lane, bstride) : 0u));
     });
   }
   __device__ static void issue_pre(const BwdParams& p, const E* gq, const E* gdo, const float* lse, const float* delta,
-                                   int64_t bstride, int q0, int T, char* st0, int wave, const uint32_t (&off)[MYP]) {
+                                   int64_t bstride, int q0, int T, char* st0, int wave, const uint32_t (&off)[MYP],
+                                   int tt = 0, int lane = 0) {
     const int rows = T - q0;
     const E* bq = gq + (int64_t)q0 * p.q.st;
     const E* bd = gdo + (int64_t)q0 * p.dout.st;
@@ -1582,6 +1615,13 @@
         buf_lds16(bq, nq, st0 + j * 1024, off[u]);
       } else if constexpr (u * NW >= PQ && (u + 1) * NW <= PQ + PD) {
         buf_lds16(bd, nd, st0 + OFF_D + (j - PQ) * 1024, off[u]);
+      } else if constexpr (PACK) {
+        if (j < PQ) buf_lds16(bq, nq, st0 + j * 1024, off[u]);
+        else if (j < PQ + PD) buf_lds16(bd, nd, st0 + OFF_D + (j - PQ) * 1024, off[u]);
+        else if (ROT ? tt % NW == wave : j == PQ + PD) {
+          const float* blk = lse + (int64_t)(q0 >> 5) * (2 * p.cst * 32);
+          if (PLN == 64 || lane < PLN) buf_lds16(blk, (uint32_t)(2 * p.cst * 128), st0 + OFF_L, off[u]);
+        }
       } else {
         if (j < PQ) buf_lds16(bq, nq, st0 + j * 1024, off[u]);
         else if (j < PQ + PD) buf_lds16(bd, nd, st0 + OFF_D + (j - PQ) * 1024, off[u]);
@@ -1592,10 +1632,11 @@
   }
 };
 
-inline bool ring_layout_ok(const BwdParams& p, int es) {
+inline bool ring_layout_ok(const BwdParams& p, int es, bool packed) {
   return dma_rows_ok(p.T, p.q.st, p.q.si, p.N, p.HS, es) && dma_rows_ok(p.T, p.dout.st, 0, 1, p.DV, es) &&
-         dma_rowvecs_ok(p.N, p.B, p.H, p.T);
-}
+         (packed ? dma_rowpack_ok(p.cst) : dma_rowvecs_ok(p.N, p.B, p.H, p.T));
+}
+inline bool ring_layout_ok(const BwdParams& p, int es) { return ring_layout_ok(p, es, p.rowc != nullptr); }
 
 
 template <class E, int HS, int N, int DV, int NW, bool PR = false, bool GRX = false>
@@ -1636,7 +1677,7 @@
 };
 
 template <class E, int HS, int N, int DV, int NW, bool DK, bool DVV, bool SRD, bool DROP, bool PR, bool GRX,
-          bool CFOLD = false>
+          bool CFOLD = false, bool PACK = false>
 __global__ __launch_bounds__(NW * 64, (NW >= 8 || PR ? 2 : 1))
 void attn_dkdv_kernel(BwdParams p) {
   using O = Ops<E>;
@@ -1660,7 +1701,8 @@
   float* Lb = reinterpret_cast<float*>(Db + NS * CF::nD);
   float* Gb = Lb + NS * NP;
   constexpr bool GR = CF::GR;
-  using RG = TileRing<E, HS, N, DV, NW, DK, BQ, !GR>;
+  static_assert(!PACK || (CFOLD && SRD), "PACK: the folded plans with descriptor staging");
+  using RG = TileRing<E, HS, N, DV, NW, DK, BQ, !GR, PACK>;
   char* ringb = reinterpret_cast<char*>(Qb);
   static_assert(!SRD || (RG::ok && RG::SB * NS <= CF::bytes - CF::nK * (int)sizeof(E) && RG::HSP == HSP &&
                           RG::DVP == DVP), "ring layout");
@@ -1706,8 +1748,11 @@
 
   uint32_t roff[SRD ? RG::MYP : 1];
   if constexpr (SRD) RG::offsets(p, bstride, wave, lane, roff);
-  auto stage_q = [&](int q0, int buf) {
-    if constexpr (SRD) {
+  auto stage_q = [&](int q0, int buf, int tt) {
+    if constexpr (PACK) {
+      const float* rcb = p.rowc + ((int64_t)b * p.H + hh) * ((T + 31) / 32) * (2 * p.cst * 32);
+      RG::issue_pre(p, gq, gdo, rcb, nullptr, bstride, q0, T, ringb + buf * RG::SB, wave, roff, tt, lane);
+    } else if constexpr (SRD) {
       RG::issue_pre(p, gq, gdo, lsep + rowvec, p.delta + rowvec, bstride, q0, T, ringb + buf * RG::SB, wave, roff);
     } else {
 #pragma unroll
@@ -1736,9 +1781,13 @@
   const int tile_pieces = SRD ? RG::pieces(wave)
                               : N * stage_pieces<E, HSP, BQ, HS, NW>(wave) + stage_pieces<E, DVP, BQ, DV, NW>(wave) +
                                     rows_pieces<N, BQ, NW>(wave) * (DK ? 2 : 1);
+  auto pieces_of = [&](int tt0, int c) {
+    if constexpr (PACK) return RG::template pieces_of<(NS > 2 ? NS - 2 : 1)>(wave, tt0, c);
+    else return tile_pieces * c;
+  };
   for (int j = 0; j < NS - 1; ++j)
-    if (j < ntiles) stage_q(kb0 + j * BQ, j);
-  wait_vm(tile_pieces * max(0, min(NS - 1, ntiles) - 1));
+    if (j < ntiles) stage_q(kb0 + j * BQ, j, j);
+  wait_vm(pieces_of(1, max(0, min(NS - 1, ntiles) - 1)));
   lds_barrier();
   scale_lds<E, NTHR>(Ks, CF::nK, p.sl2, tid);
   lds_barrier();
@@ -1766,14 +1815,14 @@
     krow = kw0 + c32;
     const int buf = t % NS;
     const int q0 = kb0 + t * BQ;
-    if (t + NS - 1 < ntiles) stage_q(q0 + (NS - 1) * BQ, (t + NS - 1) % NS);
+    if (t + NS - 1 < ntiles) stage_q(q0 + (NS - 1) * BQ, (t + NS - 1) % NS, t + NS - 1);
     st.lap<0>();
     if (wave_keys && q0 + 31 >= kw0) {
       const char* sg = ringb + buf * RG::SB;
       const E* Qc = SRD ? reinterpret_cast<const E*>(sg) : Qb + buf * N * BQ * HSP;
       const E* Dc = SRD ? reinterpret_cast<const E*>(sg + RG::OFF_D) : Db + buf * CF::nD;
       const float* Lc = SRD ? reinterpret_cast<const float*>(sg + RG::OFF_L) : Lb + buf * NP;
-      const float* Gc = SRD ? reinterpret_cast<const float*>(sg + RG::OFF_G) : Gb + buf * NP;
+      const float* Gc = PACK ? Lc + N * BQ : SRD ? reinterpret_cast<const float*>(sg + RG::OFF_G) : Gb + buf * NP;
       auto rows4 = [&](const float* ring, const float* glb, int i, int g) -> f32x4 {
         if constexpr (GR) {
           const float* v = glb + rowvec + i * bstride;
@@ -1939,7 +1988,7 @@
       }
     }
     st.lap<1>();
-    wait_vm(tile_pieces * max(0, min(NS - 2, ntiles - 2 - t)));
+    wait_vm(pieces_of(t + 2, max(0, min(NS - 2, ntiles - 2 - t))));
     st.lap<2>();
     lds_barrier();
     st.lap<3>();
@@ -2198,6 +2247,15 @@
 }
 
 template <class E, int HS, int N, int DV_, bool DROP>
+constexpr bool dkdv_can_pack() {
+  using PL = Plan<E, HS, N, DV_>;
+  using KW = DkdvWaves<E, HS, N, PL::DV, DROP>;
+  constexpr bool GR = KW::gr;
+  using CF = DkdvCfg<E, HS, N, PL::DV, KW::v, KW::pair && !GR, GR>;
+  return sizeof(E) == 2 && !DROP && !GR && TileRing<E, HS, N, PL::DV, KW::v, true, CF::BQ, !GR>::pack_ok;
+}
+
+template <class E, int HS, int N, int DV_, bool DROP>
 int launch_dkdv_t(const BwdParams& p, hipStream_t st) {
   using PL = Plan<E, HS, N, DV_>;
   using KW = DkdvWaves<E, HS, N, PL::DV, DROP>;
@@ -2213,16 +2271,20 @@
                          (sizeof(E) == 2 && NW == 4 && !PR && N * HSB / 2 + DV / 2 <= 288);
   constexpr bool CAN_FOLD = sizeof(E) == 2 && !DROP && !GR;
   auto run = [&](auto DKV, auto DVVV, auto SRDV) -> int {
-    auto launch = [&](auto CFV) -> int {
+    auto launch = [&](auto CFV, auto PKV) -> int {
       auto kern = attn_dkdv_kernel<E, HS, N, DV, NW, decltype(DKV)::value, decltype(DVVV)::value,
-                                   decltype(SRDV)::value, DROP, PR, GR, decltype(CFV)::value>;
+                                   decltype(SRDV)::value, DROP, PR, GR, decltype(CFV)::value, decltype(PKV)::value>;
       if (int e = set_smem(kern, bytes)) return e;
       hipLaunchKernelGGL(kern, grid, block, bytes, st, p);
       return 0;
     };
+    if (p.rowc) {
+      if constexpr (dkdv_can_pack<E, HS, N, DV_, DROP>() && decltype(SRDV)::value) return launch(std::true_type{}, std::true_type{});
+      else return -2;
+    }
     if constexpr (CAN_FOLD)
-      if (p.lsec) return launch(std::true_type{});
-    return launch(std::false_type{});
+      if (p.lsec) return launch(std::true_type{}, std::false_type{});
+    return launch(std::false_type{}, std::false_type{});
   };
   auto go = [&](auto SRDV) -> int {
     if constexpr (FUSED) {
@@ -2311,4 +2373,16 @@
   return -2;
 }
 
-}
+template <class E>
+bool dkdv_pack_ok_t(const BwdParams& p) {
+#define DTA_P(HS_, N_, DV_) \
+  if (p.HS == HS_ && p.N == N_ && p.DV == DV_) { \
+    if constexpr (Plan<E, HS_, N_, DV_>::ok) { \
+      if constexpr (dkdv_can_pack<E, HS_, N_, DV_, false>()) return ring_layout_ok(p, (int)sizeof(E), true); } \
+    return false; }
+  DTA_FOR_CONFIGS(DTA_P)
+#undef DTA_P
+  return false;
+}
+
+}
diff --git a/differential_transformer_replication_amd/csrc/capi.hip b/differential_transformer_replication_amd/csrc/capi.hip
--- a/differential_transformer_replication_amd/csrc/capi.hip
+++ b/differential_transformer_replication_amd/csrc/capi.hip
@@ -23,6 +23,17 @@
 bool attn_native_bf16(int, int, int);
 bool attn_native_f16(int, int, int);
 bool attn_native_f32(int, int, int);
+bool attn_dkdv_pack_ok_bf16(const BwdParams&);
+bool attn_dkdv_pack_ok_f16(const BwdParams&);
+
+bool attn_dkdv_pack_ok(int dtype, const BwdParams& p) {
+  if (p.drop_thr) return false;
+  switch (dtype) {
+    case DTA_BF16: return attn_dkdv_pack_ok_bf16(p);
+    case DTA_F16: return attn_dkdv_pack_ok_f16(p);
+  }
+  return false;
+}
 
 int launch_attn_fwd(int dtype, const FwdParams& p, hipStream_t st) {
   if (p.drop_thr) switch (dtype) {
@@ -233,7 +244,45 @@
   return delta + dq;
 }
 
-int dta_attn_bwd(const dta_attn_bwd_args* a, void* stream) {
+size_t dta_attn_bwd_row_pack_bytes(int32_t B, int32_t T, int32_t H, int32_t n_terms) {
+  return (size_t)B * H * ((T + 31) / 32) * 2 * n_terms * 32 * 4;
+}
+
+static int attn_bwd(const dta_attn_bwd_args* a, float* row_pack, void* stream);
+
+static bool bwd_packs(const dta_attn_bwd_args* a, uint32_t drop_thr) {
+  const int N = a->n_terms, hs = a->head_size;
+  if (a->dtype == DTA_F32 || drop_thr || a->group_max_dq < 0 || a->group_max_dkdv < 0) return false;
+  const int kcap = a->group_max_dkdv ? a->group_max_dkdv : bwd_group_cap(a->dtype, hs, N, true);
+  const int qcap = N > 64 ? kcap : (a->group_max_dq ? a->group_max_dq : bwd_group_cap(a->dtype, hs, N, false));
+  if (!dq_packs(2, hs, N) || branch_group(a->dtype, hs, N, a->dv, qcap) != N) return false;
+  BwdParams q{};
+  q.q = t5(a->q); q.dout = t5(a->dout);
+  q.B = a->B; q.T = a->T; q.H = a->H; q.HS = hs; q.DV = a->dv; q.cst = N;
+  for (int g0 = 0, ng; g0 < N; g0 += ng) {
+    ng = branch_group(a->dtype, hs, N - g0, a->dv, kcap);
+    q.N = ng; q.br0 = g0;
+    if (!attn_dkdv_pack_ok(a->dtype, q)) return false;
+  }
+  return true;
+}
+
+int dta_attn_bwd_packs(const dta_attn_bwd_args* a) {
+  if (!a || !ok_dims(a->dtype, a->B, a->T, a->H, a->n_terms, a->head_size, a->dv)) return 0;
+  if ((int64_t)a->B * a->T == 0 || !(a->dropout_p == 0.f)) return 0;
+  if (!attn_supported(a->dtype, a->head_size, a->n_terms, a->dv)) return 0;
+  return bwd_packs(a, 0) ? 1 : 0;
+}
+
+int dta_attn_bwd(const dta_attn_bwd_args* a, void* stream) { return attn_bwd(a, nullptr, stream); }
+
+int dta_attn_bwd_packed(const dta_attn_bwd_args* a, float* row_pack, void* stream) {
+  const bool empty = a && (int64_t)a->B * a->T == 0;
+  if (!empty && !aligned_ptr(row_pack)) return DTA_ERR_INVALID;
+  return attn_bwd(a, empty ? nullptr : row_pack, stream);
+}
+
+static int attn_bwd(const dta_attn_bwd_args* a, float* row_pack, void* stream) {
   if (!a) return DTA_ERR_INVALID;
   if (!ok_dims(a->dtype, a->B, a->T, a->H, a->n_terms, a->head_size, a->dv)) return DTA_ERR_INVALID;
   BwdParams p{};
@@ -293,6 +342,7 @@
   const bool rebase = qcap != kcap && !p.drop_thr;
   const uint64_t qstarts = rebase ? group_starts(a->dtype, p.HS, p.N, p.DV, qcap) : 0;
   const uint64_t kstarts = rebase ? group_starts(a->dtype, p.HS, p.N, p.DV, kcap) : 0;
+  if (row_pack && bwd_packs(a, p.drop_thr)) { p.rowc = row_pack; p.lsec = nullptr; }
   if (stages & DTA_BWD_DQ) {
     const bool direct = qstarts != kstarts && branch_group(a->dtype, p.HS, p.N, p.DV, qcap) == p.N;
     for (int g0 = 0, ng; g0 < p.N; g0 += ng) {
diff --git a/differential_transformer_replication_amd/csrc/dta_internal.h b/differential_transformer_replication_amd/csrc/dta_internal.h
--- a/differential_transformer_replication_amd/csrc/dta_internal.h
+++ b/differential_transformer_replication_amd/csrc/dta_internal.h
@@ -50,7 +50,13 @@
   int ob16;
   float* lsec;
   uint64_t kstarts;
+  float* rowc;
 };
+
+bool attn_dkdv_pack_ok(int dtype, const BwdParams& p);
+constexpr bool dq_packs(int esize, int hs, int n) {
+  return esize == 2 && !(hs >= 128 && n >= 3) && !(hs >= 192 && n >= 2);
+}
 
 int launch_attn_fwd(int dtype, const FwdParams& p, hipStream_t st);
 int launch_attn_fwd_drop(int dtype, const FwdParams& p, hipStream_t st);
diff --git a/differential_transformer_replication_amd/csrc/layout_checks.h b/differential_transformer_replication_amd/csrc/layout_checks.h
--- a/differential_transformer_replication_amd/csrc/layout_checks.h
+++ b/differential_transformer_replication_amd/csrc/layout_checks.h
@@ -18,4 +18,8 @@
   return n * B * H * T <= lim;
 }
 
+inline bool dma_rowpack_ok(int64_t n) {
+  return n <= 0 || n <= ((1ll << 31) - 1) / 256;
 }
+
+}
diff --git a/differential_transformer_replication_amd/ops.py b/differential_transformer_replication_amd/ops.py
--- a/differential_transformer_replication_amd/ops.py
+++ b/differential_transformer_replication_amd/ops.py
@@ -90,6 +90,7 @@
 
 _DV_F32_WORKSPACE = [True]
 _LSE_C_WORKSPACE = [True]
+_ROW_PACK_WORKSPACE = [True]
 
 _BWD_GROUP_MAX = [0, 0]
 
@@ -164,30 +165,37 @@
         dqkv = torch.empty_like(qkv)
         dq, dk, dvv = split_packed(dqkv, H, N, hs, dv)
         dcoef = torch.empty(H, N, device=dev, dtype=torch.float32)
-        delta = torch.empty(N, B, H, T, device=dev, dtype=torch.float32)
         dcp = torch.empty(lib.dta_attn_bwd_dcoef_partial_bytes(B, T, H, N) // 4, device=dev, dtype=torch.float32)
         dv32 = None
         caps = ctx.caps
         if dt != _lib.DTA_F32 and _DV_F32_WORKSPACE[0] and lib.dta_attn_bwd_dkdv_groups(dt, hs, N, dv, caps[1]) > 1:
             dv32 = torch.empty(B, T, H, dv, device=dev, dtype=torch.float32)
-        lsec = (torch.empty(N, B, H, T, device=dev, dtype=torch.float32)
-                if dt != _lib.DTA_F32 and ctx.drop[0] == 0.0 and _LSE_C_WORKSPACE[0] else None)
         obr_t = _lib.DtaTensor(obr.data_ptr(), *obr.stride()[1:4], obr.stride(0))
         a = _lib.AttnBwdArgs(dt, B, T, H, N, hs, dv, scale, ctx.drop[0],
                              _lib.tensor5(q), _lib.tensor5(k), _lib.tensor5(v), obr_t,
                              lse.data_ptr(), coef.data_ptr(), _lib.tensor5(do),
                              _lib.tensor5(dq), _lib.tensor5(dk), _lib.tensor5(dvv),
-                             dcoef.data_ptr(), delta.data_ptr(), None, _lib.BWD_PRE,
+                             dcoef.data_ptr(), None, None, _lib.BWD_PRE,
                              freqs.data_ptr() if freqs is not None else None, dcp.data_ptr(), ctx.drop[1],
                              _lib.dtype_code(obr.dtype), *caps,
-                             dv32.data_ptr() if dv32 is not None else None,
-                             lsec.data_ptr() if lsec is not None else None)
+                             dv32.data_ptr() if dv32 is not None else None, None)
+        fold = dt != _lib.DTA_F32 and ctx.drop[0] == 0.0 and _LSE_C_WORKSPACE[0]
+        packs = (fold and _ROW_PACK_WORKSPACE[0] and _lib.row_pack_symbols(lib)
+                 and lib.dta_attn_bwd_packs(a) == 1)
+        delta = torch.empty(lib.dta_attn_bwd_row_pack_bytes(B, T, H, N) // 4 if packs else N * B * H * T,
+                            device=dev, dtype=torch.float32)
+        lsec = torch.empty(N, B, H, T, device=dev, dtype=torch.float32) if fold and not packs else None
+        a.delta = delta.data_ptr()
+        a.lse_c = lsec.data_ptr() if lsec is not None else None
+        bwd = lib.dta_attn_bwd
+        if packs:
+            bwd = lambda args, st: lib.dta_attn_bwd_packed(args, delta.data_ptr(), st)
         a.stages = _lib.BWD_DQ
         with TIMER.region("attn_bwd_dq"):
-            _lib.check(lib.dta_attn_bwd(a, stream))
+            _lib.check(bwd(a, stream))
         a.stages = _lib.BWD_DKDV
         with TIMER.region("attn_bwd_dkdv"):
-            _lib.check(lib.dta_attn_bwd(a, stream))
+            _lib.check(bwd(a, stream))
         return dqkv, dcoef, None, None, None, None, None, None, None, None
 
 
diff --git a/include/diffattn.h b/include/diffattn.h
--- a/include/diffattn.h
+++ b/include/diffattn.h
@@ -74,6 +74,10 @@
                                     int32_t head_size);
 size_t dta_attn_bwd_dcoef_partial_bytes(int32_t B, int32_t T, int32_t H, int32_t n_terms);
 int dta_attn_bwd_dkdv_groups(int32_t dtype, int32_t head_size, int32_t n_terms, int32_t dv, int32_t group_max_dkdv);
+
+int dta_attn_bwd_packed(const dta_attn_bwd_args* a, float* row_pack, void* stream);
+size_t dta_attn_bwd_row_pack_bytes(int32_t B, int32_t T, int32_t H, int32_t n_terms);
+int dta_attn_bwd_packs(const dta_attn_bwd_args* a);
 
 typedef struct dta_ln_args {
   int32_t dtype;
```

New measurement: 558.1 TFLOP/s, median of 2. No clear change (+0.1%).
